# Avokadoen/tdt4230_project_raytracing

Hardware: AMD Instinct MI355X
Metric: Mray-samples/sec at 1080p/64spp/depth-8 (higher is better)
Workload: dtype f32; 1 GPU; 1920x1080, 64 spp, max_bounce 8, 64^3 octree terrain+spheres (BASELINE configs[1] scene at the metric's 64 spp); written_pixels=2027520, spp=64, passes=1, max_bounce=8, octree_max_depth=6, octree_cells=4209, scene_bytes=269868, partition=32x32 work-groups dealt round-robin over 1 rank(s)

## Files before the change

### include/tdt_rt.h

```cpp
#ifndef TDT_RT_H
#define TDT_RT_H

#include <stddef.h>
#include <stdint.h>

#ifdef __cplusplus
extern "C" {
#endif

typedef struct tdt_ctx tdt_ctx;
typedef struct tdt_compute tdt_compute;
typedef struct tdt_buffer tdt_buffer;
typedef struct tdt_image tdt_image;

enum {
  TDT_OK = 0,
  TDT_ERR_NO_DEVICE = 1,
  TDT_ERR_HIP = 2,
  TDT_ERR_INVALID_ENUM = 0x0500,
  TDT_ERR_INVALID_VALUE = 0x0501,
  TDT_ERR_INVALID_OPERATION = 0x0502,
  TDT_ERR_VARIABLE_NOT_FOUND = 3,
  TDT_ERR_INCOMPLETE = 4
};
// ... 183 lines not shown
#ifdef __cplusplus
static_assert(sizeof(tdt_mesh) == 40, "tdt_mesh is 40 bytes");
#else
_Static_assert(sizeof(tdt_mesh) == 40, "tdt_mesh is 40 bytes");
#endif
int tdt_voxelize_triangles(tdt_ctx *ctx, const tdt_mesh *mesh, int depth, int32_t *voxels_xyzm, size_t capacity, size_t *n_voxels);
int tdt_octree_edit_triangles(tdt_ctx *ctx, int op, const tdt_mesh *mesh, uint32_t *n_cells);

typedef struct tdt_fill {
  int32_t connectivity;
  int32_t material;
} tdt_fill;
#ifdef __cplusplus
static_assert(sizeof(tdt_fill) == 8, "tdt_fill is 8 bytes");
#else
_Static_assert(sizeof(tdt_fill) == 8, "tdt_fill is 8 bytes");
#endif
int tdt_octree_extract_enclosed(tdt_ctx *ctx, const tdt_fill *fill, const tdt_region *regions, size_t n_regions, int32_t *voxels_xyzm,
                                size_t capacity, size_t *n_voxels);
int tdt_octree_fill_enclosed(tdt_ctx *ctx, const tdt_fill *fill, const tdt_region *regions, size_t n_regions, uint32_t *n_cells);
int tdt_voxelize_triangles_solid(tdt_ctx *ctx, const tdt_mesh *mesh, int depth, const tdt_fill *fill, int32_t *voxels_xyzm, size_t capacity,
                                 size_t *n_voxels);
int tdt_octree_edit_triangles_solid(tdt_ctx *ctx, int op, const tdt_mesh *mesh, const tdt_fill *fill, uint32_t *n_cells);
int tdt_debug_fill_passes(const tdt_ctx *ctx);

typedef struct tdt_surface {
  int32_t merge;
  int32_t by_material;
} tdt_surface;
typedef struct tdt_quad {
  int32_t face;
  int32_t material;
  int32_t origin[3];
  int32_t size[2];
  int32_t pad;
} tdt_quad;
#ifdef __cplusplus
static_assert(sizeof(tdt_surface) == 8, "tdt_surface is 8 bytes");
static_assert(sizeof(tdt_quad) == 32, "tdt_quad is 32 bytes");
#else
_Static_assert(sizeof(tdt_surface) == 8, "tdt_surface is 8 bytes");
_Static_assert(sizeof(tdt_quad) == 32, "tdt_quad is 32 bytes");
#endif
int tdt_octree_extract_surface(tdt_ctx *ctx, const tdt_surface *opt, const tdt_region *regions, size_t n_regions, tdt_quad *quads,
                               size_t capacity, size_t *n_quads);

#define TDT_ROUND_DOMAIN_CAP (1u << 28)
typedef struct tdt_round {
  int32_t op;
  int32_t radius2;
  int32_t material;
  int32_t border;
} tdt_round;
#ifdef __cplusplus
static_assert(sizeof(tdt_round) == 16, "tdt_round is 16 bytes");
#else
_Static_assert(sizeof(tdt_round) == 16, "tdt_round is 16 bytes");
#endif
int tdt_octree_morph_round(tdt_ctx *ctx, const tdt_round *r, const tdt_region *regions, size_t n_regions, uint32_t *n_cells);
int tdt_octree_extract_morph_round(tdt_ctx *ctx, const tdt_round *r, const tdt_region *regions, size_t n_regions, int32_t *voxels_xyzm,
                                   size_t capacity, size_t *n_voxels);
int tdt_octree_distance_field(tdt_ctx *ctx, const int32_t lo[3], const int32_t hi[3], int32_t max_d2, int32_t border, int32_t *field,
                              int32_t *nearest_xyz, size_t capacity, size_t *n_voxels);

#define TDT_XFORM_ONE 65536
typedef struct tdt_xform {
  int64_t t[3];
  int32_t a[9];
  int32_t material;
  int32_t dst_lo[3], dst_hi[3];
  int32_t pad[2];
} tdt_xform;
#ifdef __cplusplus
static_assert(sizeof(tdt_xform) == 96, "tdt_xform is 96 bytes");
#else
_Static_assert(sizeof(tdt_xform) == 96, "tdt_xform is 96 bytes");
#endif
int tdt_octree_extract_transform(tdt_ctx *ctx, const tdt_xform *xf, const tdt_region *regions, size_t n_regions, int32_t *voxels_xyzm,
                                 size_t capacity, size_t *n_voxels);
int tdt_octree_transform(tdt_ctx *ctx, const tdt_xform *xf, int op, const tdt_region *regions, size_t n_regions, uint32_t *n_cells);
int tdt_debug_xform_bricks(const tdt_ctx *ctx, uint32_t out[2]);

int tdt_debug_last_variant(const tdt_ctx *ctx, int out[6]);
int tdt_debug_trace_variants(int *rows, int capacity, int *count);
int tdt_debug_stats(tdt_ctx *ctx, uint64_t *out, int n_words, int reset);
int tdt_debug_counters(tdt_ctx *ctx, uint64_t out[32]);
int tdt_debug_wave_ends(tdt_ctx *ctx, uint64_t *out, int n);
int tdt_debug_pixel_log(tdt_ctx *ctx, uint32_t *out, size_t n_u32);
int tdt_selftest(tdt_ctx *ctx, int which, uint64_t *mismatches);
int tdt_selftest_index(tdt_ctx *ctx, int32_t cell_count, float inv_cell_count, uint32_t n_cells, int shift, uint64_t *mismatches,
                       int *shape_ok);

#ifdef __cplusplus
}
#endif
#endif
```

### tdt4230_project_raytracing_amd/build.py

```python
import os
import shutil
import subprocess

_HERE = os.path.dirname(os.path.abspath(__file__))
ROOT = os.path.dirname(_HERE)
CSRC = os.path.join(_HERE, "csrc")
INCLUDE = os.path.join(ROOT, "include")

HIPCC = os.environ.get("HIPCC") or shutil.which("hipcc") or "/opt/rocm/bin/hipcc"

HIP_FLAGS = ["--offload-arch=gfx950", "-O3", "-std=c++17", "-fPIC", "-shared", "-ffp-contract=off",
             "-fhip-fp32-correctly-rounded-divide-sqrt", "-fno-fast-math", "-Wall", "-Wextra",
             "-fno-slp-vectorize"]
HOST_FLAGS = ["-O2", "-std=c++17", "-fPIC", "-shared", "-Wall", "-Wextra", "-ffp-contract=off"]


def _newer(out, srcs):
    if not os.path.exists(out):
        return True
    t = os.path.getmtime(out)
    return any(os.path.getmtime(s) > t for s in srcs)


def _run(cmd):
    r = subprocess.run(cmd, capture_output=True, text=True)
    if r.returncode != 0:
        raise RuntimeError("build failed: " + " ".join(cmd) + "\n" + r.stdout + r.stderr)
    return r.stdout + r.stderr


def build_host(force=False):
    out = os.path.join(_HERE, "libtdthost.so")
    srcs = [os.path.join(CSRC, "host_scene.cpp"), os.path.join(CSRC, "host_view.cpp"), os.path.join(CSRC, "host_mesh.cpp"),
            os.path.join(CSRC, "host_xform.cpp"), os.path.join(INCLUDE, "tdt_host.h"), os.path.join(INCLUDE, "tdt_rt.h"), os.path.abspath(__file__)]
    if force or _newer(out, srcs):
        _run(["g++"] + HOST_FLAGS + ["-I", INCLUDE] + srcs[:4] + ["-o", out, "-lz"])
    return out


DEVICE_UNITS = ("tdt_rt.hip", "tdt_multi.hip", "tdt_build.hip", "tdt_edit.hip", "tdt_query.hip", "tdt_compact.hip",
                "tdt_region.hip", "tdt_connect.hip", "tdt_morph.hip", "tdt_mesh.hip", "tdt_fill.hip", "tdt_surface.hip",
                "tdt_distance.hip", "tdt_bitvol.hip", "tdt_xform.hip")
DEVICE_HEADERS = ("trace_device.hpp", "trace_params.h", "tdt_internal.hpp", "device_scan.hpp", "region_device.hpp", "bitvol_device.hpp")


def build_device(force=False, extra_flags=(), out=None):
    out = out or os.path.join(_HERE, "libtdtrt.so")
    hdrs = [os.path.join(CSRC, f) for f in DEVICE_HEADERS] + [os.path.join(INCLUDE, "tdt_rt.h"), os.path.abspath(__file__)]
    srcs = [os.path.join(CSRC, f) for f in DEVICE_UNITS]
    if not (force or extra_flags or _newer(out, srcs + hdrs)):
        return out
    objdir = os.path.join(CSRC, "obj" + ("_" + str(abs(hash(tuple(extra_flags))) % 100000) if extra_flags else ""))
    os.makedirs(objdir, exist_ok=True)
    compile_flags = [f for f in HIP_FLAGS if f != "-shared"] + list(extra_flags)
    jobs = []
    for src in srcs:
        obj = os.path.join(objdir, os.path.basename(src) + ".o")
        if force or extra_flags or _newer(obj, [src] + hdrs):
            jobs.append((subprocess.Popen([HIPCC] + compile_flags + ["-I", INCLUDE, "-I", CSRC, "-c", src, "-o", obj],
                                          stdout=subprocess.PIPE, stderr=subprocess.STDOUT, text=True), src))
    for p, src in jobs:
        log, _ = p.communicate()
        if p.returncode != 0:
            raise RuntimeError("build failed: " + src + "\n" + log)
    objs = [os.path.join(objdir, os.path.basename(src) + ".o") for src in srcs]
    _run([HIPCC, "--offload-arch=gfx950", "-shared", "-fPIC"] + objs + ["-o", out, "-ldl"])
    return out


def build_demo(force=False):
    out = os.path.join(_HERE, "tdt_demo")
    srcs = [os.path.join(CSRC, "demo_main.cpp"), os.path.join(INCLUDE, "renderer.hpp"), os.path.join(INCLUDE, "tdt_rt.h"),
            os.path.join(INCLUDE, "tdt_host.h"), os.path.abspath(__file__)]
    if force or _newer(out, srcs):
        rocm_lib = os.path.join(os.path.dirname(os.path.dirname(os.path.realpath(HIPCC))), "lib")
        _run(["g++", "-O2", "-std=c++17", "-Wall", "-Wextra", "-I", INCLUDE, srcs[0], "-o", out, "-L", _HERE, "-ltdtrt", "-ltdthost",
              "-Wl,-rpath,$ORIGIN", "-Wl,-rpath-link," + rocm_lib])
    return out


def build_selftest(force=False):
    out = os.path.join(_HERE, "libtdtprims_selftest.so")
    src = os.path.join(CSRC, "prims_selftest.hip")
    deps = [src, os.path.join(CSRC, "device_scan.hpp"), os.path.join(CSRC, "tdt_internal.hpp"),
            os.path.join(INCLUDE, "tdt_rt.h"), os.path.abspath(__file__)]
    if force or _newer(out, deps):
        _run([HIPCC] + HIP_FLAGS + ["-I", INCLUDE, "-I", CSRC, src, "-o", out, "-L", _HERE, "-ltdtrt", "-Wl,-rpath,$ORIGIN"])
    return out


def build_all(force=False):
    return build_host(force), build_device(force), build_demo(force), build_selftest(force)
```

### tdt4230_project_raytracing_amd/csrc/tdt_rt.hip

```cpp
#include <hip/hip_runtime.h>

#include <atomic>
#include <cstdio>
#include <cstdlib>
#include <cstring>
#include <initializer_list>
#include <new>
#include <string>
#include <vector>

#include "tdt_rt.h"
#include "trace_device.hpp"
#include "trace_params.h"

#ifndef TDT_BLOCK
#define TDT_BLOCK 1024
#define TDT_BLOCKS_PER_CU 1
#endif
namespace tdt {

TDT_DEV void decode_pixel(const TraceParams &P, int k, uint32_t p, int &x, int &y, size_t &pix, bool &inside) {
  const int t = P.part_rank + k * P.part_world;
  int gx, gy;
  if (P.tiles_x_magic) { gy = (int)__umulhi((uint32_t)t, P.tiles_x_magic); gx = t - gy * P.tiles_x; }
  else { gx = t % P.tiles_x; gy = t / P.tiles_x; }
  const int tile = (int)(p >> 6), w = (int)(p & 63);
  const int lx = (tile & 3) * 8 + (w & 7), ly = (tile >> 2) * 8 + (w >> 3);
  x = gx * 32 + lx;
  y = gy * 32 + ly;
  pix = P.compact ? ((size_t)k * 1024 + (size_t)(ly * 32 + lx)) : ((size_t)y * (size_t)P.image_width + (size_t)x);
  inside = x < P.cover_w && y < P.cover_h;
}

TDT_DEV bool pixel_of_thread(const TraceParams &P, int &x, int &y, size_t &pix) {
  const int k = blockIdx.x >> 2, sub = blockIdx.x & 3;
  bool inside;
  decode_pixel(P, k, (uint32_t)(sub * 256 + threadIdx.x), x, y, pix, inside);
  return inside;
}

TDT_DEV uint32_t wave_sum(uint32_t v) {
  for (int o = 32; o > 0; o >>= 1) v += __shfl_xor(v, o, 64);
  return v;
}


enum : int { ST_DONE = -1, ST_TRAVERSE = 0, ST_HIT = 1, ST_END = 2, ST_FETCH = 3, ST_PRIMARY = 4, ST_NEWRAY = 5 };

template <bool AS_MASKS> struct HitOwed;
template <> struct HitOwed<true> {
  bool use_leaf = false, leaf_rec = false;
  TDT_DEV void set(bool later_step, bool cube_ok) { use_leaf = later_step; leaf_rec = later_step && cube_ok; }
  TDT_DEV bool leaf_site() const { return use_leaf; }
  TDT_DEV bool new_record() const { return leaf_rec; }
};
template <> struct HitOwed<false> {
  uint32_t bits = 0u;
  TDT_DEV void set(bool later_step, bool cube_ok) { bits = later_step ? (cube_ok ? 3u : 1u) : 0u; }
  TDT_DEV bool leaf_site() const { return (bits & 1u) != 0u; }
  TDT_DEV bool new_record() const { return (bits & 2u) != 0u; }
};

enum : int { STAT_TRAV_PASS = 0, STAT_TRAV_LANES, STAT_INSIDE_LANES, STAT_ALIVE_LANES, STAT_EVENT_PASS, STAT_EVENT_LANES, STAT_HIT_PASS, STAT_HIT_LANES,
             STAT_LAMB_PASS, STAT_LAMB_LANES, STAT_METAL_PASS, STAT_METAL_LANES, STAT_DIEL_PASS, STAT_DIEL_LANES, STAT_END_PASS, STAT_END_LANES,
             STAT_PIXEL_END_PASS, STAT_PIXEL_END_LANES, STAT_FETCH_PASS, STAT_FETCH_LANES, STAT_PRIMARY_PASS, STAT_PRIMARY_LANES,
             STAT_NEWRAY_PASS, STAT_NEWRAY_LANES, STAT_GATE_WAIT_LANES, STAT_DRAINED_TRAV_PASS, STAT_DRAINED_EVENT_PASS, STAT_LOOP_PASS, STAT_WAVE_TICKS, STAT_WAVES,
             STAT_T_FIRST, STAT_T_LAST, STAT_COUNT = 32 };
#ifdef TDT_STATS
TDT_DEV void stat_add(uint32_t *row, int i, unsigned long long mask) {
  const unsigned long long m = __ballot(1);
  if (mask != 0ull && (threadIdx.x & 63) == (uint32_t)__builtin_ctzll(m)) { row[i] += 1u; row[i + 1] += (uint32_t)__popcll(mask); }
}
#define TDT_ST(i, mask) stat_add(s_stat_row, (i), (mask))
#define TDT_ST1(i, v) do { const unsigned long long m_ = __ballot(1); if ((threadIdx.x & 63) == (uint32_t)__builtin_ctzll(m_)) s_stat_row[i] += (uint32_t)(v); } while (0)
#else
#define TDT_ST(i, mask) do {} while (0)
#define TDT_ST1(i, v) do {} while (0)
#endif

template <bool COUNT, int FORM, int DEPTH = 0, bool RESIDENT = false, bool SAFEV = false, bool FULL = false, bool UNIT = false, bool BRICK = false>
__global__ __launch_bounds__(TDT_BLOCK) void trace_kernel(const TraceParams P) {
  constexpr bool POW2 = FORM != FORM_LITERAL;
  constexpr bool kSlim2 = DEPTH > 0;
#ifdef TDT_THRESHOLD_EVERY
  constexpr uint32_t kThresholdEvery = kSlim2 ? TDT_THRESHOLD_EVERY : 1u;
#else
  constexpr uint32_t kThresholdEvery = kSlim2 ? 8u : 1u;
#endif
  constexpr bool kSharedRand = !BRICK;
  constexpr bool kColdArgs = BRICK;
#ifdef TDT_NO_STUCK_CUT
  constexpr bool kStuckCut = false;
#else
  constexpr bool kStuckCut = BRICK && !COUNT;
#endif
#ifdef TDT_NO_SHARED_NORM
  constexpr bool kSharedNorm = false;
#else
  constexpr bool kSharedNorm = kSlim2;
#endif
  __shared__ __attribute__((aligned(16))) uint16_t s_nodes[(BRICK ? kBrickLdsCells : kLdsCells) * 8 + 8];
  for (uint32_t i = threadIdx.x * 8u; i < P.lds_nodes; i += (uint32_t)TDT_BLOCK * 8u)
    *reinterpret_cast<uint4 *>(&s_nodes[i]) = *reinterpret_cast<const uint4 *>(&P.packed[i]);
  if (threadIdx.x < 16 && P.lds_nodes + threadIdx.x < ((P.lds_nodes + 7u) & ~7u) + 8u)
    s_nodes[P.lds_nodes + threadIdx.x] = (uint16_t)((RESIDENT && POW2) ? 0u : kPackedEscape);
  constexpr bool kPlanes = FULL && !COUNT && kFullEntryForm == kFullPlanes;
  __shared__ __attribute__((aligned(8))) float2 s_planes[kPlanes ? PlaneTable::kEntries : 1];
  if constexpr (kPlanes) build_plane_table<DEPTH, UNIT>(s_planes, P.scale, P.min_x, P.min_y, P.min_z);
  __syncthreads();
  constexpr bool TABLE = FORM == FORM_TABLE;
  static_assert(!TABLE || (SAFEV && !BRICK && !FULL), "per-cell thresholds: the resident walk, or the jump table's bands of a tree outside the LDS table");
  constexpr uint32_t kThrCells = !TABLE ? 0u : (RESIDENT ? kLdsCells : kThrTopCells);
  __shared__ __attribute__((aligned(8))) float2 s_thr[kThrCells + 1];
  __shared__ uint32_t s_band;
  if (TABLE) {
    for (uint32_t i = threadIdx.x; i <= kThrCells; i += (uint32_t)TDT_BLOCK)
      s_thr[i] = i < P.thr_cells ? reinterpret_cast<const float2 *>(P.thr)[i] : make_float2(2.0f, 2.0f);
    __syncthreads();
  }
  constexpr int GL = top_grid_levels(RESIDENT, TABLE);
  constexpr bool kUseGrid = !FULL && !BRICK && !COUNT && POW2 && SAFEV && DEPTH >= GL;
  __shared__ typename Grid<GL>::Entry s_grid[kUseGrid ? Grid<GL>::kEntries : 1];
  __shared__ int s_grid_ok;
  if (kUseGrid) build_top_grid<GL, TABLE>(s_nodes, P.lds_nodes, DEPTH, s_grid, &s_grid_ok, s_thr, P.thr_cells, P.thr_f0max, &s_band);
  __shared__ __attribute__((aligned(16))) uint32_t s_grid32[BRICK ? (1 << 15) : 4];
  if (BRICK) {
    for (uint32_t i = threadIdx.x * 4u; i < (1u << 15); i += (uint32_t)TDT_BLOCK * 4u)
      *reinterpret_cast<uint4 *>(&s_grid32[i]) = *reinterpret_cast<const uint4 *>(&P.brick_grid[i]);
    __syncthreads();
  }
  NodeSource ns;
  ns.lds = s_nodes; ns.lds_nodes = P.lds_nodes; ns.lds_cells = (P.lds_nodes + 7u) >> 3;
  ns.grid = s_grid; ns.grid_ok = kUseGrid ? (__builtin_amdgcn_readfirstlane(s_grid_ok) != 0) : false;
  ns.grid_band = FULL ? Grid<5>::kBand : (ns.grid_ok ? (TABLE && kUseGrid ? __uint_as_float((uint32_t)__builtin_amdgcn_readfirstlane((int)s_band)) : Grid<GL>::kBand) : 2.0f);
  ns.thr = s_thr; ns.thr_f0max = P.thr_f0max;
  ns.full = P.full_grid;
  if constexpr (kPlanes) ns.planes = s_planes;
  ns.grid32 = s_grid32; ns.bricks = P.bricks;
  if (BRICK) {
    uint32_t lo, hi;
    asm volatile("v_mov_b32 %0, %2\n\tv_mov_b32 %1, %3" : "=v"(lo), "=v"(hi) : "s"((uint32_t)(uintptr_t)P.bricks), "s"((uint32_t)((uintptr_t)P.bricks >> 32)));
    ns.bricks = reinterpret_cast<const void *>(((uintptr_t)hi << 32) | (uintptr_t)lo);
  }
  ns.cells = __builtin_amdgcn_make_buffer_rsrc((void *)P.cells, 0, (int)((P.cells_dwords >> 1) << 3), 0x00020000);
  typedef const __attribute__((address_space(4))) TraceParams *KArg;
  const KArg Pk = (KArg)__builtin_amdgcn_kernarg_segment_ptr();
  MatSource ms_regs;
  if (!kColdArgs) ms_regs = material_source(P);
#ifdef TDT_STATS
  __shared__ uint32_t s_stats[(TDT_BLOCK / 64) * STAT_COUNT];
  uint32_t *const s_stat_row = &s_stats[(threadIdx.x >> 6) * STAT_COUNT];
  if ((threadIdx.x & 63) < STAT_COUNT) s_stat_row[threadIdx.x & 63] = 0u;
  const unsigned long long stat_t0 = __builtin_amdgcn_s_memrealtime();
  bool stat_drained = false;
#endif
  const uint32_t total_slots = (uint32_t)P.owned_tiles * 1024u;
  if (blockIdx.x == 0 && threadIdx.x == 0 && P.queue_next) *P.queue_next = 0u;

  const float inf = __builtin_inff();
#ifdef TDT_STATS
  uint32_t stat_pix_t0 = 0u;
#endif
  unsigned long long pixel_rt0 = 0ull; bool wave_drained = false; uint32_t lane_S = 0, lane_E = 0, pass_no = 0, pixel_pass0 = 0, evpass_no = 0, pixel_evpass0 = 0;
  const unsigned long long wave_t0 = COUNT ? __builtin_amdgcn_s_memrealtime() : 0ull;
  if (COUNT && (threadIdx.x & 63) == 0) atomicCAS(&P.counters[23], 0ull, wave_t0);
  Counters cnt = {};
  uint32_t n_pixels = 0;
  constexpr int kMemo = BRICK ? kBrickMemoLevels : kMemoLevels;
  NodeMemo<kMemo> memo;
#pragma unroll
  for (int l = 0; l < kMemo; l++) { memo.key[l] = 0x3FFFFFFFu; memo.val[l] = 0u; }

  int state = ST_FETCH;
  int x = 0, y = 0; size_t pix = 0;
  uint32_t pixel_slot = 0;
  const bool exact_draw = P.plan != nullptr && __builtin_amdgcn_readfirstlane((int)P.plan[0]) != 0;
  uint32_t buf_slot = 0xFFFFFFFFu, buf_next = 0u, buf_count = 0u;
  int s = 0, loop_count = 0;
  Ray r = {0.f, 0.f, 0.f, 0.f, 0.f, 1.f};
  float ix = 0.f, iy = 0.f, iz = 0.f;
  float ar = 1.f, ag = 1.f, ab = 1.f;
  float sr = 0.f, sg = 0.f, sb = 0.f;
  float t_stride = 0.f, t_octree_max = 0.f, inv_pow_depth = 0.5f;
  int it = 0;
  HitOwed<DEPTH == 0> owed;
  uint32_t hit_index = 0;
  float leaf_box_x = 0.f, leaf_box_y = 0.f, leaf_box_z = 0.f;
  Carry pc;
  pc.root = {0.f, 0.f, 0.f, 0.f, 0.f, 0.f, false}; pc.leaf = pc.root; pc.root_t = 0.f;
  const int s_end = P.spp_begin + P.spp_count;

  uint32_t w_steps = 0, w_rays = 0, lane_work = 0;
  uint32_t ev_no = 0;
  int threshold = P.event_threshold > 0 ? P.event_threshold : 24;

  unsigned long long tacc[7] = {0, 0, 0, 0, 0, 0, 0}, tlast = COUNT ? __builtin_amdgcn_s_memtime() : 0ull;
#define TDT_TICK(i) do { if (COUNT) { const unsigned long long n_ = __builtin_amdgcn_s_memtime(); tacc[i] += n_ - tlast; tlast = n_; } } while (0)
  float vmin_x, vmin_y, vmin_z;
  if (DEPTH == 0) { vmin_x = P.min_x; vmin_y = P.min_y; vmin_z = P.min_z; }
  else asm volatile("v_mov_b32 %0, %3\n\tv_mov_b32 %1, %4\n\tv_mov_b32 %2, %5" : "=v"(vmin_x), "=v"(vmin_y), "=v"(vmin_z) : "s"(P.min_x), "s"(P.min_y), "s"(P.min_z));
  if constexpr (kPlanes) { ns.vmin_x = vmin_x; ns.vmin_y = vmin_y; ns.vmin_z = vmin_z; }
  unsigned long long k_trav = 0ull, k_event = ~0ull;
  int th_now = threshold;
  for (;;) {
    if (COUNT) pass_no++;
    TDT_ST1(STAT_LOOP_PASS, 1);
    TDT_MARK(traversal);
    {
      const bool trav = __builtin_amdgcn_inverse_ballot_w64(k_trav);
      const unsigned long long k_trav0 = k_trav;
      if (COUNT && trav) { lane_S++; cnt.trav_slots += slot64(); cnt.trav_active++; }
      const bool go = trav && (it < P.max_iter) && (t_stride < t_octree_max);
      const float adv = POW2 ? 0.0001f * (inv_pow_depth + 0.1f) : f_max(0.0001f * (inv_pow_depth + 0.1f), 0.000001f);
      const float tt = t_stride + adv;
      const float wx = tt * r.dx + r.ox, wy = tt * r.dy + r.oy, wz = tt * r.dz + r.oz;
      const float lx = UNIT ? (wx + -vmin_x) : (wx + -vmin_x) * P.inv_scale, ly = UNIT ? (wy + -vmin_y) : (wy + -vmin_y) * P.inv_scale,
                  lz = UNIT ? (wz + -vmin_z) : (wz + -vmin_z) * P.inv_scale;
      bool in_box;
      if (POW2) {
        constexpr bool kNoNegZero = UNIT && kSlim2;
        const uint32_t ux = __float_as_uint(kNoNegZero ? lx : lx + 0.0f), uy = __float_as_uint(kNoNegZero ? ly : ly + 0.0f), uz = __float_as_uint(kNoNegZero ? lz : lz + 0.0f);
        const uint32_t um = ux > uy ? ux : uy;
        in_box = (um > uz ? um : uz) < 0x3F800000u;
      } else {
        const float ex = f_fract(lx) + -lx, ey = f_fract(ly) + -ly, ez = f_fract(lz) + -lz;
        in_box = !((__builtin_fabsf(ez) + __builtin_fabsf(ey)) != -__builtin_fabsf(ex));
      }
      const bool inside = go && in_box;
      TDT_ST(STAT_TRAV_PASS, __ballot(trav)); TDT_ST1(STAT_INSIDE_LANES, __popcll(__ballot(inside))); TDT_ST1(STAT_ALIVE_LANES, __popcll(__ballot(state != ST_DONE)));
#ifdef TDT_STATS
      TDT_ST1(STAT_DRAINED_TRAV_PASS, stat_drained ? 1 : 0);
#endif
      if (inside) {
        float ugx, ugy, ugz; uint32_t value;
        if (COUNT) cnt.iterations++;
        const float ipd_in = inv_pow_depth;
        CellPlanes cp;
        bool leaf;
        if constexpr (kPlanes) leaf = tree_lookup_pow2<COUNT, kMemo, DEPTH, RESIDENT, SAFEV, FULL, BRICK, TABLE, UNIT>(P, ns, lx, ly, lz, inv_pow_depth, ugx, ugy, ugz, value, memo, cnt, &cp);
        else leaf = POW2 ? tree_lookup_pow2<COUNT, kMemo, DEPTH, RESIDENT, SAFEV, FULL, BRICK, TABLE>(P, ns, lx, ly, lz, inv_pow_depth, ugx, ugy, ugz, value, memo, cnt)
                         : tree_lookup<COUNT>(P, ns, lx, ly, lz, inv_pow_depth, ugx, ugy, ugz, value, cnt);
        TDT_MARK(traversal_b);
        float t_enter, t_exit, cs, cx = 0.f, cy = 0.f, cz = 0.f;
        if constexpr (kPlanes) {
          leaf_box_x = cp.lox; leaf_box_y = cp.loy; leaf_box_z = cp.loz; hit_index = value;
          cube_slabs_planes(r, ix, iy, iz, cp.lox, cp.loy, cp.loz, cp.hix, cp.hiy, cp.hiz, t_stride, t_octree_max, t_enter, t_exit);
          cs = UNIT ? inv_pow_depth : P.scale * inv_pow_depth;
        } else {
          if (!kSlim2) lane_work += kCostStep + (127u - (__float_as_uint(inv_pow_depth) >> 23));
          const float bx = (UNIT ? ugx : ugx * P.scale) + vmin_x, by = (UNIT ? ugy : ugy * P.scale) + vmin_y, bz = (UNIT ? ugz : ugz * P.scale) + vmin_z;
          const float cs0 = UNIT ? inv_pow_depth : P.scale * inv_pow_depth;
          const float pad = leaf ? -0.0f : -0.00001f;
          if (kSlim2) { leaf_box_x = bx + pad; leaf_box_y = by + pad; leaf_box_z = bz + pad; hit_index = value; }
          cx = kSlim2 ? leaf_box_x : bx + pad; cy = kSlim2 ? leaf_box_y : by + pad; cz = kSlim2 ? leaf_box_z : bz + pad;
          cs = leaf ? cs0 : cs0 + 0.00002f;
          cube_slabs(r, ix, iy, iz, cx, cy, cz, cs, t_stride, t_octree_max, t_enter, t_exit);
        }
        const bool cube_ok = !(t_exit < t_enter);
        if (leaf) {
          if (!kSlim2) { leaf_box_x = cx; leaf_box_y = cy; leaf_box_z = cz; hit_index = value; }
          inv_pow_depth = cs; t_stride = t_enter;
          owed.set(it > 0, cube_ok);
          state = ST_HIT;
        } else {
          const float ts_new = cube_ok ? t_exit : t_octree_max;
          if (kStuckCut) {
            const bool stuck = __float_as_uint(ts_new) == __float_as_uint(t_stride) && __float_as_uint(inv_pow_depth) == __float_as_uint(ipd_in);
            t_stride = stuck ? t_octree_max : ts_new;
          } else t_stride = ts_new;
          it++;
        }
      }
      state = (trav && !inside) ? ST_END : state;
      k_trav &= __ballot(state == ST_TRAVERSE);
      k_event = ~k_trav & (k_event | k_trav0);
    }

    TDT_TICK(0);
    TDT_MARK(gate);
    const unsigned long long m_trav = k_trav, m_event = k_event;
    if (m_trav == 0ull && m_event == 0ull) break;
    w_steps += (uint32_t)__popcll(m_trav);
    TDT_ST1(STAT_GATE_WAIT_LANES, __popcll(m_event));
    if ((int)__popcll(m_event) < th_now && m_trav != 0ull) { TDT_TICK(1); continue; }
    TDT_TICK(1);
    TDT_ST(STAT_EVENT_PASS, m_event); TDT_ST(STAT_HIT_PASS, __ballot(state == ST_HIT));
#ifdef TDT_STATS
    TDT_ST1(STAT_DRAINED_EVENT_PASS, stat_drained ? 1 : 0);
#endif

    TDT_MARK(hit_prologue);
    if (COUNT) evpass_no++;
    if (COUNT) { cnt.event_slots += slot64(); cnt.event_active += (state > ST_TRAVERSE); }
    if (kSlim2) lane_work += (state == ST_HIT || state == ST_END) ? kCostEvent + kCostRayStep * ((uint32_t)it + 1u) : ((state > ST_TRAVERSE) ? kCostEvent : 0u);
    else lane_work += (state > ST_TRAVERSE) ? kCostEvent : 0u;
    if (COUNT) lane_E += (state > ST_TRAVERSE) ? 1u : 0u;
    if (state == ST_HIT) {
      if (COUNT) { cnt.scatter_slots += slot64(); cnt.scatter_active++; }
      MatSource ms;
      if (kColdArgs) {
        KArg pk = Pk; asm volatile("" : "+s"(pk));
        ms.materials = table_rsrc(pk->materials, pk->materials_dwords); ms.albedos = table_rsrc(pk->albedos, pk->albedos_dwords);
        ms.metal = table_rsrc(pk->metal, pk->metal_dwords); ms.dielectric = table_rsrc(pk->dielectric, pk->dielectric_dwords);
      } else ms = ms_regs;
      const MatRef mat = material_fetch(ms, hit_index);
      TDT_ST(STAT_LAMB_PASS, __ballot(mat.type == 0u)); TDT_ST(STAT_METAL_PASS, __ballot(mat.type == 1u)); TDT_ST(STAT_DIEL_PASS, __ballot(mat.type == 2u));
      if (owed.new_record()) { cube_hit_record(r, t_stride, leaf_box_x, leaf_box_y, leaf_box_z, inv_pow_depth, pc.leaf); if (COUNT) cnt.leaf_records++; }
      loop_count += 1;
      const HitTmp &src = owed.leaf_site() ? pc.leaf : pc.root;
      Hit h;
      h.px = src.px; h.py = src.py; h.pz = src.pz; h.nx = src.nx; h.ny = src.ny; h.nz = src.nz; h.ff = src.ff;
      h.index = hit_index;
      Ray nr; float tr, tg, tb;
      const bool scattered = scatter<COUNT, kSharedRand, kSharedNorm>(ms, r, h, mat, nr, tr, tg, tb, cnt);
      TDT_MARK(hit_epilogue);
      if (scattered) {
        ar = ar * tr; ag = ag * tg; ab = ab * tb;
        r = nr;
        state = loop_count < P.max_bounce ? ST_NEWRAY : ST_END;
      } else {
        state = ST_END;
      }
    }
    TDT_TICK(2);
    TDT_MARK(end_of_path);
    TDT_ST(STAT_END_PASS, __ballot(state == ST_END));
    if (state == ST_END) {
      float cr, cg, cb;
      if (loop_count > 0) { cr = ar; cg = ag; cb = ab; }
      else {
        const float yp = r.dy + 1.0f;
        const float w = 1.0f + -(0.5f * yp);
        cr = w + 0.25f * yp; cg = w + 0.35f * yp; cb = 1.0f;
      }
      sr = sr + cr; sg = sg + cg; sb = sb + cb;
      s++;
      if (s < s_end) state = ST_PRIMARY;
      else {
        TDT_MARK(pixel_end);
        TDT_ST(STAT_PIXEL_END_PASS, __ballot(1));
        float4 *dst = reinterpret_cast<float4 *>(P.image) + pix;
        if (P.accumulate) {
          *dst = make_float4(sr, sg, sb, 0.f);
          if (P.carry && !P.carry_final) {
            float4 *c = reinterpret_cast<float4 *>(P.carry) + pix * 4;
            c[0] = make_float4(pc.root.nx, pc.root.ny, pc.root.nz, pc.root.px);
            c[1] = make_float4(pc.root.py, pc.root.pz, pc.root.ff ? 1.f : 0.f, pc.root_t);
            c[2] = make_float4(pc.leaf.nx, pc.leaf.ny, pc.leaf.nz, pc.leaf.px);
            c[3] = make_float4(pc.leaf.py, pc.leaf.pz, pc.leaf.ff ? 1.f : 0.f, 0.f);
          }
        } else {
          const float n = (float)P.samples_per_pixel;
          float4 o;
          o.x = f_min(f_max(__builtin_sqrtf(sr / n), 0.f), 1.f);
          o.y = f_min(f_max(__builtin_sqrtf(sg / n), 0.f), 1.f);
          o.z = f_min(f_max(__builtin_sqrtf(sb / n), 0.f), 1.f);
          o.w = 1.0f;
          *dst = o;
        }
#ifdef TDT_STATS
        if (P.stats && P.pixel_log) {
          uint32_t *L = P.pixel_log + (size_t)pixel_slot * 8;
          L[0] = lane_work; L[3] = stat_pix_t0; L[4] = (uint32_t)__builtin_amdgcn_s_memrealtime(); L[5] = blockIdx.x * 16 + (threadIdx.x >> 6); L[7] = (uint32_t)threshold;
        }
#endif
        if (COUNT && P.pixel_log) {
          uint32_t *L = P.pixel_log + (size_t)pixel_slot * 8;
          L[0] = lane_S; L[1] = lane_E; L[2] = pass_no - pixel_pass0; L[3] = (uint32_t)(pixel_rt0 - P.counters[23]);
          L[4] = (uint32_t)(__builtin_amdgcn_s_memrealtime() - P.counters[23]); L[5] = blockIdx.x * 16 + (threadIdx.x >> 6); L[6] = evpass_no - pixel_evpass0; L[7] = (uint32_t)threshold;
        }
        if (COUNT) {
          const unsigned long long d = (__builtin_amdgcn_s_memrealtime() - pixel_rt0) / 10000ull;
          atomicAdd(&P.counters[32 + 16384 + (wave_drained ? 128 : 0) + (d > 127ull ? 127ull : d)], 1ull);
        }
        if (P.slot_cost) P.slot_cost[pixel_slot] = lane_work | 1u;
        state = ST_FETCH;
      }
    }
    TDT_TICK(3);
    TDT_MARK(fetch);
    {
      bool want = state == ST_FETCH;
      unsigned long long m = __ballot(want);
      TDT_ST(STAT_FETCH_PASS, m);
      while (m != 0ull) {
        if (buf_next >= buf_count) {
          const uint32_t chunk = exact_draw ? (uint32_t)__popcll(m) : 64u;
          uint32_t base = 0;
          if ((threadIdx.x & 63) == 0) base = atomicAdd(P.queue, chunk);
          base = (uint32_t)__builtin_amdgcn_readfirstlane((int)base);
          const uint32_t bq = base + (threadIdx.x & 63u);
          buf_slot = ((threadIdx.x & 63u) < chunk && bq < total_slots) ? (P.slot_order ? P.slot_order[bq] : bq) : 0xFFFFFFFFu;
          buf_next = 0u; buf_count = chunk;
          if (COUNT && base + chunk > total_slots) wave_drained = true;
#ifdef TDT_STATS
          if (base + chunk > total_slots && !stat_drained) { stat_drained = true; if (P.stats && (threadIdx.x & 63) == 0) atomicMin(&P.stats[STAT_COUNT], __builtin_amdgcn_s_memrealtime()); }
#endif
        }
        const uint32_t rank = (uint32_t)__popcll(m & ((1ull << (threadIdx.x & 63)) - 1ull));
        const uint32_t avail = buf_count - buf_next;
        const uint32_t got = (uint32_t)__shfl((int)buf_slot, (int)((buf_next + rank) & 63u), 64);
        const bool served = want && rank < avail;
        buf_next += (uint32_t)__popcll(m) < avail ? (uint32_t)__popcll(m) : avail;
        m = __ballot(want && !served);
        if (served) {
          want = false;
          const uint32_t q = got;
          if (q == 0xFFFFFFFFu) { state = ST_DONE; if (COUNT) atomicMin(&P.counters[22], __builtin_amdgcn_s_memrealtime()); }
          else {
#ifdef TDT_STATS
            stat_pix_t0 = (uint32_t)__builtin_amdgcn_s_memrealtime();
#endif
            if (COUNT) { pixel_rt0 = __builtin_amdgcn_s_memrealtime(); lane_S = 0; lane_E = 0; pixel_pass0 = pass_no; pixel_evpass0 = evpass_no; }
            bool inside;
            pixel_slot = q;
            decode_pixel(P, (int)(pixel_slot >> 10), pixel_slot & 1023u, x, y, pix, inside);
            lane_work = 0u;
            if (inside) {
              n_pixels++;
              sr = 0.f; sg = 0.f; sb = 0.f; s = P.spp_begin;
              pc.root = {0.f, 0.f, 0.f, 0.f, 0.f, 0.f, false}; pc.leaf = pc.root; pc.root_t = 0.f;
              if (P.accumulate && P.spp_begin != 0) {
                const float4 acc = *(reinterpret_cast<const float4 *>(P.image) + pix);
                sr = acc.x; sg = acc.y; sb = acc.z;
                if (P.carry) {
                  const float4 *c = reinterpret_cast<const float4 *>(P.carry) + pix * 4;
                  const float4 c0 = c[0], c1 = c[1], c2 = c[2], c3 = c[3];
                  pc.root = {c0.x, c0.y, c0.z, c0.w, c1.x, c1.y, c1.z != 0.f}; pc.root_t = c1.w;
                  pc.leaf = {c2.x, c2.y, c2.z, c2.w, c3.x, c3.y, c3.z != 0.f};
                }
              }
              if (s < s_end) state = ST_PRIMARY;
              else if (!P.accumulate) {
                const float n = (float)P.samples_per_pixel;
                const float v0 = f_min(f_max(__builtin_sqrtf(0.f / n), 0.f), 1.f);
                *(reinterpret_cast<float4 *>(P.image) + pix) = make_float4(v0, v0, v0, 1.0f);
              }
            }
          }
        }
      }
    }
    TDT_TICK(4);
    TDT_MARK(primary);
    TDT_ST(STAT_PRIMARY_PASS, __ballot(state == ST_PRIMARY));
    if (state == ST_PRIMARY) {
      r = primary_ray(P, x, y, s);
      loop_count = 0; ar = 1.f; ag = 1.f; ab = 1.f;
      state = ST_NEWRAY;
    }
    TDT_MARK(threshold);
    w_rays += (uint32_t)__popcll(__ballot(state == ST_NEWRAY));
    if (P.event_threshold <= 0 && (ev_no++ & (kThresholdEvery - 1u)) == 0u) {
      if (w_rays > kEventWindow) { w_steps >>= 1; w_rays >>= 1; }
      const float est = 64.0f * __builtin_amdgcn_rcpf(0.5f + __builtin_amdgcn_sqrtf(P.event_k * (float)w_steps * __builtin_amdgcn_rcpf((float)w_rays + 1.0f)));
      const int th = (int)__builtin_fminf(est, P.event_clamp);
      threshold = w_rays < 256u ? 24 : (th < 2 ? 2 : th);
    }
    TDT_TICK(5);
    TDT_MARK(newray);
    TDT_ST(STAT_NEWRAY_PASS, __ballot(state == ST_NEWRAY));
    if (state == ST_NEWRAY) {
      if (!(loop_count < P.max_bounce)) state = ST_END;
      else {
        if (COUNT) cnt.octree_hit_calls++;
        q_rcp3(r.dx, r.dy, r.dz, ix, iy, iz);
        const float lx = (P.min_x + -r.ox) * ix, ly = (P.min_y + -r.oy) * iy, lz = (P.min_z + -r.oz) * iz;
        const float ux = ((P.min_x + P.scale) + -r.ox) * ix, uy = ((P.min_y + P.scale) + -r.oy) * iy,
                    uz = ((P.min_z + P.scale) + -r.oz) * iz;
        const float mnx = hw_min(lx, ux), mny = hw_min(ly, uy), mnz = hw_min(lz, uz);
        const float mxx = hw_max(lx, ux), mxy = hw_max(ly, uy), mxz = hw_max(lz, uz);
        const float t_enter = hw_max(hw_max(hw_max(mnx, 0.0003f), mny), mnz);
        const float t_exit = hw_min(hw_min(hw_min(mxx, inf), mxy), mxz);
        t_octree_max = inf;
        if (t_exit >= t_enter) {
          cube_hit_record(r, t_enter, P.min_x, P.min_y, P.min_z, P.scale, pc.root);
          pc.root_t = t_enter;
          t_octree_max = t_exit;
        }
        t_stride = pc.root_t;
        inv_pow_depth = 0.5f;
        it = 0;
        state = ST_TRAVERSE;
      }
    }
    TDT_TICK(6);
    k_trav = __ballot(state == ST_TRAVERSE); k_event = __ballot(state > ST_TRAVERSE);
    { const int n_alive = __popcll(k_trav | k_event); th_now = n_alive == 64 ? threshold : ((threshold * n_alive) >> 6) + 1; }
    TDT_MARK(loop_tail);
  }
  TDT_MARK(after_loop);
#undef TDT_TICK
#ifdef TDT_STATS
  if (P.stats) {
    const unsigned long long stat_t1 = __builtin_amdgcn_s_memrealtime();
    const uint32_t lane = threadIdx.x & 63u;
    if (lane < (uint32_t)STAT_WAVE_TICKS) { const uint32_t v = s_stat_row[lane]; if (v) atomicAdd(&P.stats[lane], (unsigned long long)v); }
    if (lane == 0) { atomicAdd(&P.stats[STAT_WAVE_TICKS], stat_t1 - stat_t0); atomicAdd(&P.stats[STAT_WAVES], 1ull);
                     atomicMin(&P.stats[STAT_T_FIRST], stat_t0); atomicMax(&P.stats[STAT_T_LAST], stat_t1);
                     const uint32_t w = blockIdx.x * (TDT_BLOCK / 64) + (threadIdx.x >> 6);
                     if (w < 8192u) P.stats[STAT_COUNT + 1 + w] = stat_t1; }
  }
#endif

  if (COUNT) {
    if ((threadIdx.x & 63) == 0) {
      const unsigned long long t_end = __builtin_amdgcn_s_memrealtime();
      atomicMin(&P.counters[18], wave_t0); atomicMax(&P.counters[19], t_end);
      atomicAdd(&P.counters[20], t_end - wave_t0); atomicAdd(&P.counters[21], 1ull);
      P.counters[32 + blockIdx.x * (TDT_BLOCK / 64) + (threadIdx.x >> 6)] = t_end;
    }
    if ((threadIdx.x & 63) == 0) for (int i = 0; i < 7; i++) atomicAdd(&P.counters[24 + i], tacc[i]);
    uint32_t v[18] = {n_pixels, cnt.octree_hit_calls, cnt.iterations, cnt.node_loads,
                      cnt.lambertian, cnt.metal, cnt.dielectric, cnt.unknown,
                      cnt.trav_slots, cnt.trav_active, cnt.level_slots, cnt.level_active, cnt.event_slots, cnt.event_active,
                      cnt.scatter_slots, cnt.scatter_active, cnt.memo_miss, cnt.leaf_records};
    for (int i = 0; i < 18; i++) {
      uint32_t tot = wave_sum(v[i]);
      if ((threadIdx.x & 63) == 0 && tot) atomicAdd(&P.counters[i], (unsigned long long)tot);
    }
  }
}

__global__ __launch_bounds__(256) void resolve_kernel(const TraceParams P) {
  int x, y; size_t pix;
  if (!pixel_of_thread(P, x, y, pix)) return;
  float4 *dst = reinterpret_cast<float4 *>(P.image) + pix;
  float4 a = *dst;
  if (P.carry_final && a.w != 0.f) return;
  const float n = (float)P.total_spp;
  float4 o;
  o.x = f_min(f_max(__builtin_sqrtf(a.x / n), 0.f), 1.f);
  o.y = f_min(f_max(__builtin_sqrtf(a.y / n), 0.f), 1.f);
  o.z = f_min(f_max(__builtin_sqrtf(a.z / n), 0.f), 1.f);
  o.w = 1.0f;
  *dst = o;
}

__global__ __launch_bounds__(256) void miss_prepass_kernel(const TraceParams P, uint8_t *__restrict__ done) {
  int x, y; size_t pix;
  const bool covered = pixel_of_thread(P, x, y, pix);
  const size_t slot = (size_t)(blockIdx.x >> 2) * 1024u + (size_t)((blockIdx.x & 3) * 256 + threadIdx.x);
  bool all_miss = covered;
  float sr = 0.f, sg = 0.f, sb = 0.f;
  const float inf = __builtin_inff();
  for (int s = 0; s < P.samples_per_pixel && __ballot(all_miss) != 0ull; s++) {
    const Ray r = primary_ray(P, x, y, s);
    float ix, iy, iz;
    q_rcp3(r.dx, r.dy, r.dz, ix, iy, iz);
    const float lx = (P.min_x + -r.ox) * ix, ly = (P.min_y + -r.oy) * iy, lz = (P.min_z + -r.oz) * iz;
    const float ux = ((P.min_x + P.scale) + -r.ox) * ix, uy = ((P.min_y + P.scale) + -r.oy) * iy, uz = ((P.min_z + P.scale) + -r.oz) * iz;
    const float mnx = hw_min(lx, ux), mny = hw_min(ly, uy), mnz = hw_min(lz, uz);
    const float mxx = hw_max(lx, ux), mxy = hw_max(ly, uy), mxz = hw_max(lz, uz);
    const float t_enter = hw_max(hw_max(hw_max(mnx, 0.0003f), mny), mnz);
    const float t_exit = hw_min(hw_min(hw_min(mxx, inf), mxy), mxz);
    const bool root_hit = t_exit >= t_enter;
    const float adv = f_max(0.0001f * (0.5f + 0.1f), 0.000001f);
    const float tt = 0.f + adv;
    const float wx = tt * r.dx + r.ox, wy = tt * r.dy + r.oy, wz = tt * r.dz + r.oz;
    const float px = (wx + -P.min_x) * P.inv_scale, py = (wy + -P.min_y) * P.inv_scale, pz = (wz + -P.min_z) * P.inv_scale;
    const float ex = f_fract(px) + -px, ey = f_fract(py) + -py, ez = f_fract(pz) + -pz;
    const bool in_box = !((__builtin_fabsf(ez) + __builtin_fabsf(ey)) != -__builtin_fabsf(ex));
    const bool steps_in = (0 < P.max_iter) && (0.f < inf) && in_box;
    if (root_hit || steps_in) all_miss = false;
    const float yp = r.dy + 1.0f;
    const float w = 1.0f + -(0.5f * yp);
    sr = sr + (w + 0.25f * yp); sg = sg + (w + 0.35f * yp); sb = sb + 1.0f;
  }
  if (covered && all_miss) {
    const float n = (float)P.samples_per_pixel;
    float4 o;
    o.x = f_min(f_max(__builtin_sqrtf(sr / n), 0.f), 1.f);
    o.y = f_min(f_max(__builtin_sqrtf(sg / n), 0.f), 1.f);
    o.z = f_min(f_max(__builtin_sqrtf(sb / n), 0.f), 1.f);
    o.w = 1.0f;
    *(reinterpret_cast<float4 *>(P.image) + pix) = o;
  }
  done[slot] = (!covered || all_miss) ? 1u : 0u;
}

constexpr uint32_t kFilterChunk = 4096;
TDT_DEV uint32_t filter_rank(bool live, uint32_t *s_wave, uint32_t &block_total) {
  const unsigned long long m = __ballot(live);
  const uint32_t lane = threadIdx.x & 63u, wave = threadIdx.x >> 6;
  if (lane == 0) s_wave[wave] = (uint32_t)__popcll(m);
  __syncthreads();
  uint32_t before = 0, total = 0;
  for (uint32_t w = 0; w < 16u; w++) { const uint32_t c = s_wave[w]; before += w < wave ? c : 0u; total += c; }
  __syncthreads();
  block_total = total;
  return before + (uint32_t)__popcll(m & ((1ull << lane) - 1ull));
}
__global__ __launch_bounds__(1024) void filter_count_kernel(const uint32_t *__restrict__ order, const uint8_t *__restrict__ done, uint32_t n, uint32_t *__restrict__ counts) {
// ... 479 lines not shown
  const float4 c = image[(size_t)y * w + x];
  auto u8 = [](float v) -> uint32_t {
    const float t = !(v > 0.0f) ? 0.0f : (v > 1.0f ? 1.0f : v);
    return (uint32_t)__builtin_rintf(t * 255.0f);
  };
  out[(size_t)(top_down ? h - 1 - y : y) * w + x] = u8(c.x) | (u8(c.y) << 8) | (u8(c.z) << 16) | (u8(c.w) << 24);
}

__global__ __launch_bounds__(256) void assemble_kernel(const float4 *__restrict__ tiles, float4 *__restrict__ image,
                                                       int image_width, int cover_w, int cover_h, int tiles_x,
                                                       int world, int tiles_per_rank) {
  const int x = blockIdx.x * 64 + (threadIdx.x & 63);
  const int y = blockIdx.y * 4 + (threadIdx.x >> 6);
  if (x >= cover_w || y >= cover_h) return;
  const int t = (y >> 5) * tiles_x + (x >> 5);
  const int rank = t % world, k = t / world;
  const size_t src = ((size_t)rank * tiles_per_rank + k) * 1024 + (size_t)((y & 31) * 32 + (x & 31));
  image[(size_t)y * image_width + x] = tiles[src];
}

}

#include "tdt_internal.hpp"

namespace {
thread_local std::string g_create_err;
}

namespace tdt {
int fail(tdt_ctx *ctx, int code, const std::string &msg) {
  if (ctx) ctx->err = msg; else g_create_err = msg;
  return code;
}
int hip_fail(tdt_ctx *ctx, hipError_t e, const char *what) {
  return fail(ctx, TDT_ERR_HIP, std::string(what) + ": " + hipGetErrorString(e));
}
}
using tdt::fail; using tdt::hip_fail; using tdt::erase_from; using tdt::Cover; using tdt::Tiles; using tdt::cover_of; using tdt::tiles_of;

Cover tdt::cover_of(const tdt_compute *c, int width, int height) {
  Cover k;
  k.groups_x = width / 32 < 1 ? 1 : width / 32;
  k.groups_y = height / 32 < 1 ? 1 : height / 32;
  long cw = (long)k.groups_x * 32, ch = (long)k.groups_y * 32;
  k.cover_w = (int)(cw < c->image_width ? cw : c->image_width);
  k.cover_h = (int)(ch < c->image_height ? ch : c->image_height);
  if (k.cover_w < 0) k.cover_w = 0;
  if (k.cover_h < 0) k.cover_h = 0;
  return k;
}
Tiles tdt::tiles_of(const tdt_compute *c, const Cover &k) {
  Tiles t;
  t.tiles_x = (k.cover_w + 31) / 32; t.tiles_y = (k.cover_h + 31) / 32;
  t.total = t.tiles_x * t.tiles_y;
  t.owned = t.total > c->part_rank ? (t.total - c->part_rank + c->part_world - 1) / c->part_world : 0;
  return t;
}
namespace {
int64_t owned_pixels(const tdt_compute *c, const Cover &k) {
  Tiles t = tiles_of(c, k);
  int64_t n = 0;
  for (int i = 0; i < t.owned; i++) {
    int id = c->part_rank + i * c->part_world;
    int gx = id % t.tiles_x, gy = id / t.tiles_x;
    int w = k.cover_w - gx * 32, h = k.cover_h - gy * 32;
    n += (int64_t)(w > 32 ? 32 : w) * (h > 32 ? 32 : h);
  }
  return n;
}

void make_sig(const tdt_ctx *ctx, const tdt_compute *c, const Cover &k, const tdt_image *img, CostSig *sig) {
  std::memset(sig, 0, sizeof *sig);
  std::memcpy(sig->cam_i, &c->image_width, sizeof sig->cam_i);
  std::memcpy(sig->cam_f, c->horizontal, sizeof sig->cam_f);
  sig->part[0] = c->part_rank; sig->part[1] = c->part_world;
  std::memcpy(sig->octree_f, ctx->ssbo[TDT_SLOT_OCTREE_FLOATS]->shadow, sizeof sig->octree_f);
  std::memcpy(sig->octree_i, ctx->ssbo[TDT_SLOT_OCTREE_INTS]->shadow, sizeof sig->octree_i);
  sig->cover[0] = k.cover_w; sig->cover[1] = k.cover_h; sig->image[0] = img->w; sig->image[1] = img->h;
  for (int sl = 0; sl < kNumSlots; sl++)
    if (ctx->ssbo[sl]) { sig->slot[sl].buffer = ctx->ssbo[sl]; sig->slot[sl].version = ctx->ssbo[sl]->version; }
}

using TraceFn = void (*)(const TraceParams);
struct TraceVariant { int form, depth; bool resident, full, brick, unit; TraceFn fn; };
#define TDT_V1(FORM, D, R, F, B, U) {tdt::FORM, D, R, F, B, U, tdt::trace_kernel<false, tdt::FORM, D, R, true, F, U, B>}
#define TDT_V(FORM, D, R, F, B) TDT_V1(FORM, D, R, F, B, false), TDT_V1(FORM, D, R, F, B, true)
const TraceVariant kTraceVariants[] = {
  TDT_V(FORM_POW2, 6, false, false, true), TDT_V(FORM_POW2, 7, false, false, true), TDT_V(FORM_POW2, 8, false, false, true),
  TDT_V(FORM_POW2, 9, false, false, true), TDT_V(FORM_POW2, 10, false, false, true),
  TDT_V(FORM_POW2, 6, false, false, false), TDT_V(FORM_POW2, 7, false, false, false), TDT_V(FORM_POW2, 8, false, false, false),
  TDT_V(FORM_POW2, 9, false, false, false), TDT_V(FORM_POW2, 10, false, false, false),
  TDT_V(FORM_POW2, 5, true, true, false), TDT_V(FORM_POW2, 6, true, true, false),
  TDT_V(FORM_POW2, 3, true, false, false), TDT_V(FORM_POW2, 4, true, false, false), TDT_V(FORM_POW2, 5, true, false, false),
  TDT_V(FORM_POW2, 6, true, false, false), TDT_V(FORM_POW2, 7, true, false, false), TDT_V(FORM_POW2, 8, true, false, false),
  TDT_V(FORM_POW2, 9, true, false, false), TDT_V(FORM_POW2, 10, true, false, false),
  TDT_V(FORM_TABLE, 3, true, false, false), TDT_V(FORM_TABLE, 4, true, false, false), TDT_V(FORM_TABLE, 5, true, false, false),
  TDT_V(FORM_TABLE, 6, true, false, false), TDT_V(FORM_TABLE, 7, true, false, false), TDT_V(FORM_TABLE, 8, true, false, false),
  TDT_V(FORM_TABLE, 9, true, false, false), TDT_V(FORM_TABLE, 10, true, false, false),
  TDT_V(FORM_TABLE, 6, false, false, false), TDT_V(FORM_TABLE, 7, false, false, false), TDT_V(FORM_TABLE, 8, false, false, false),
  TDT_V(FORM_TABLE, 9, false, false, false), TDT_V(FORM_TABLE, 10, false, false, false),
};
#undef TDT_V
#undef TDT_V1
TraceFn find_variant(int form, int depth, bool resident, bool full, bool brick, bool unit) {
  for (const TraceVariant &v : kTraceVariants)
    if (v.form == form && v.depth == depth && v.resident == resident && v.full == full && v.brick == brick && v.unit == unit) return v.fn;
  return nullptr;
}

}

int tdt::octree_uniforms(tdt_ctx *ctx, TraceParams &P) {
  if (ctx->ssbo[TDT_SLOT_OCTREE_FLOATS]->bytes < 28 || ctx->ssbo[TDT_SLOT_OCTREE_INTS]->bytes < 12)
    return fail(ctx, TDT_ERR_INVALID_VALUE, "octree uniform buffers are too small (need 28 / 12 bytes)");
  float of[7]; int32_t oi[3];
  std::memcpy(of, ctx->ssbo[TDT_SLOT_OCTREE_FLOATS]->shadow, sizeof of);
  std::memcpy(oi, ctx->ssbo[TDT_SLOT_OCTREE_INTS]->shadow, sizeof oi);
  P.min_x = of[0]; P.min_y = of[1]; P.min_z = of[2]; P.scale = of[4]; P.inv_scale = of[5]; P.inv_cell_count = of[6];
  P.max_depth = oi[0]; P.max_iter = oi[1]; P.cell_count = oi[2];
  return TDT_OK;
}

namespace {
bool env_set(const char *name) { return getenv(name) != nullptr; }
bool env_one(const char *name) { const char *v = getenv(name); return v && v[0] == '1'; }
float env_float(const char *name, float otherwise) { const char *v = getenv(name); return v ? (float)atof(v) : otherwise; }
int env_int(const char *name, int lo, int hi, int otherwise) {
  const char *v = getenv(name);
  return v && atoi(v) >= lo && atoi(v) <= hi ? atoi(v) : otherwise;
}
constexpr int kAnyLo = -2147483647 - 1, kAnyHi = 2147483647;
}

struct tdt::TraceState {
  tdt::DeviceScratch mem;
  struct Switches {
    bool no_cost_order = env_one("TDT_NO_COST_ORDER");
    int force_smooth = env_int("TDT_ORDER_SMOOTH", kAnyLo, kAnyHi, -1);
    bool no_cost_accum = env_set("TDT_NO_COST_ACCUM");
    bool no_two_phase = env_set("TDT_NO_TWO_PHASE");
    bool no_prepass = env_set("TDT_NO_PREPASS");
    bool no_order_reuse = env_set("TDT_NO_ORDER_REUSE");
    bool no_full = env_set("TDT_NO_FULL_GRID");
    bool no_table_form = env_set("TDT_NO_TABLE_FORM");
    bool no_bricks = env_set("TDT_NO_BRICKS");
    float max_share = env_float("TDT_MAX_SHARE", 1.0f);
    float order_blend = env_float("TDT_ORDER_BLEND", 0.5f);
    int two_phase_min_spp = env_int("TDT_TWO_PHASE_MIN_SPP", 2, kAnyHi, 16);
    int probe_div = env_int("TDT_PROBE_DIV", 2, 64, 16);
    bool force_generic = env_one("TDT_FORCE_GENERIC");
    bool no_specialise = env_one("TDT_NO_SPECIALISE");
    int event_threshold = env_int("TDT_EVENT_THRESHOLD", kAnyLo, kAnyHi, 0);
    float event_k = env_float("TDT_EVENT_K", 0.0f);
    int event_clamp = env_int("TDT_EVENT_CLAMP", 2, 64, 40);
  } env;
  struct Queue {
    unsigned int *heads = nullptr; unsigned parity = 0;
  } queue;
  struct CostOrder {
    uint32_t *slot_cost = nullptr, *slot_acc = nullptr, *slot_order = nullptr;
    uint32_t *hist = nullptr; unsigned parity = 0;
    uint32_t tile_capacity = 0, cost_tiles = 0;
    uint32_t cost_dispatches = 0;
    uint32_t acc_samples = 0, last_launch_samples = 0;
    int cost_range[2] = {0, 0}; bool order_exact = false;
    CostSig cost_sig = {};
  } order;
  struct MissPrepass {
    uint8_t *slot_done = nullptr; uint32_t *slot_live = nullptr, *filter_counts = nullptr; uint32_t capacity = 0;
  } miss;
  struct TableKey {
    const tdt_buffer *buffer = nullptr; unsigned long long version = 0; int depth = 0;
    bool operator==(const TableKey &o) const { return buffer == o.buffer && version == o.version && depth == o.depth; }
  };
  struct ThresholdKey {
    int32_t cell_count = 0; uint32_t ic_bits = 0, n = 0;
    bool operator==(const ThresholdKey &o) const { return cell_count == o.cell_count && ic_bits == o.ic_bits && n == o.n; }
  };
  struct Tables {
    uint16_t *packed = nullptr; TableKey packed_key;
    uint32_t *scan = nullptr;
    uint32_t max_parent_value = 0xFFFFFFFFu, max_any_value = 0xFFFFFFFFu, live_nodes = 0xFFFFFFFFu;
    float *thr = nullptr; ThresholdKey thr_key; float thr_f0max = 0.0f; bool thr_ok = false;
    FullGridEntry *full_grid = nullptr; TableKey full_key; bool full_ok = false;
    uint32_t *brick_grid = nullptr; uint16_t *bricks = nullptr; size_t bricks_bytes = 0; TableKey brick_key; bool brick_ok = false;
  } tables;
  float *frame_carry = nullptr; size_t frame_carry_bytes = 0;
  bool phase_timing = false; hipEvent_t phase_ev[4] = {}; int phase_n = 0;
  uint32_t *present = nullptr; size_t present_bytes = 0;
  uint32_t *pixel_log = nullptr; size_t pixel_log_u32 = 0;
  unsigned long long *stats = nullptr;
  int last_variant[6] = {};

  ~TraceState() { if (phase_timing) for (auto &e : phase_ev) (void)hipEventDestroy(e); }
  template <class T> hipError_t alloc(T *&p, size_t n) { p = mem.get<T>(n); return p ? hipSuccess : hipErrorOutOfMemory; }
  struct Array {
    void **p; size_t bytes;
    template <class T> Array(T *&ptr, size_t count) : p(reinterpret_cast<void **>(&ptr)), bytes(count * sizeof(T)) {}
  };
  template <class C> hipError_t grow(C &capacity, C need, std::initializer_list<Array> arrays) {
    if (capacity >= need) return hipSuccess;
    capacity = 0;
    for (const Array &a : arrays) { mem.drop(*a.p); *a.p = nullptr; }
    for (const Array &a : arrays)
      if (!(*a.p = mem.get<unsigned char>(a.bytes))) {
        for (const Array &b : arrays) { mem.drop(*b.p); *b.p = nullptr; }
        return hipErrorOutOfMemory;
      }
    capacity = need;
    return hipSuccess;
  }
};

namespace {
using tdt::TraceState;

struct LaunchRequest {
  enum Kind { kRender = 0, kAccumulate = 1, kResolve = 2, kMissPrepass = 3 } kind = kRender;
  int spp_begin = 0, spp_count = 0, total_spp = 0;
  void *carry = nullptr; bool carry_final = false;
  bool probe = false;
  bool prepass_ran = false;
  unsigned long long *counts_out = nullptr;
};

int bind_params(const tdt_compute *c, int width, int height, const LaunchRequest &rq, TraceParams &P, Cover &k, Tiles &t) {
  tdt_ctx *ctx = c->ctx;
  const TraceState::Switches &env = ctx->trace->env;
  static const int required[] = {TDT_SLOT_CELLS, TDT_SLOT_MATERIALS, TDT_SLOT_ALBEDOS, TDT_SLOT_METAL,
                                 TDT_SLOT_DIELECTRIC, TDT_SLOT_OCTREE_FLOATS, TDT_SLOT_OCTREE_INTS};
  for (int s : required)
    if (!ctx->ssbo[s]) return fail(ctx, TDT_ERR_INCOMPLETE, "no buffer bound to shader-storage slot " + std::to_string(s));
  if (!ctx->image0) return fail(ctx, TDT_ERR_INCOMPLETE, "no image bound to unit 0");
  const tdt_image *img = ctx->image0;

  std::memset(&P, 0, sizeof P);
  if (int rc = tdt::octree_uniforms(ctx, P)) return rc;
  P.image_width = c->image_width; P.image_height = c->image_height;
  for (int i = 0; i < 3; i++) {
    P.hor[i] = c->horizontal[i]; P.ver[i] = c->vertical[i]; P.llc[i] = c->lower_left_corner[i]; P.org[i] = c->origin[i];
  }
  P.samples_per_pixel = c->samples_per_pixel; P.max_bounce = c->max_bounce;
  auto dwords = [](const tdt_buffer *b) { size_t d = b->bytes >> 2; return (uint32_t)(d > 0xFFFFFFFFull ? 0xFFFFFFFFull : d); };
  P.cells = (const uint32_t *)ctx->ssbo[TDT_SLOT_CELLS]->dev; P.cells_dwords = dwords(ctx->ssbo[TDT_SLOT_CELLS]);
  P.materials = (const uint32_t *)ctx->ssbo[TDT_SLOT_MATERIALS]->dev; P.materials_dwords = dwords(ctx->ssbo[TDT_SLOT_MATERIALS]);
  P.albedos = (const uint32_t *)ctx->ssbo[TDT_SLOT_ALBEDOS]->dev; P.albedos_dwords = dwords(ctx->ssbo[TDT_SLOT_ALBEDOS]);
  P.metal = (const uint32_t *)ctx->ssbo[TDT_SLOT_METAL]->dev; P.metal_dwords = dwords(ctx->ssbo[TDT_SLOT_METAL]);
  P.dielectric = (const uint32_t *)ctx->ssbo[TDT_SLOT_DIELECTRIC]->dev; P.dielectric_dwords = dwords(ctx->ssbo[TDT_SLOT_DIELECTRIC]);
  P.image = img->dev; P.carry = (float *)rq.carry;
  P.carry_final = (rq.kind == LaunchRequest::kResolve ? rq.prepass_ran : rq.carry_final) ? 1 : 0;
  k = cover_of(c, width, height);
  t = tiles_of(c, k);
  P.cover_w = k.cover_w; P.cover_h = k.cover_h;
  P.tiles_x = t.tiles_x > 0 ? t.tiles_x : 1; P.owned_tiles = t.owned;
  P.tiles_x_magic = ((unsigned long long)(t.total > 0 ? t.total : 1) * (unsigned long long)P.tiles_x < (1ull << 32) && P.tiles_x > 1)
                        ? (uint32_t)((1ull << 32) / (unsigned long long)P.tiles_x) + 1u : 0u;
  P.part_rank = c->part_rank; P.part_world = c->part_world;
  if (img->w == c->image_width && img->h == c->image_height) P.compact = 0;
  else if (img->w == 32 && img->h >= 32 * t.owned && (img->h % 32) == 0) P.compact = 1;
  else return fail(ctx, TDT_ERR_INVALID_OPERATION,
                   "bound image is neither camera.image_width x image_height nor a 32 x 32*tiles tile buffer");
  P.spp_begin = rq.spp_begin; P.spp_count = rq.spp_count; P.mode = rq.kind; P.total_spp = rq.total_spp;
  P.accumulate = rq.kind == LaunchRequest::kAccumulate ? 1 : 0;
  P.event_threshold = env.event_threshold;
  P.event_clamp = (float)env.event_clamp;
  {
    const float mib = (float)ctx->ssbo[TDT_SLOT_CELLS]->bytes / 1048576.0f;
    const float r = 0.07f * mib;
    P.event_k = env.event_k > 0.0f ? env.event_k : (r < 0.10f ? 0.10f : (r > 0.35f ? 0.35f : r));
    { static const char *ks = getenv("TDT_EVENT_K_SCALE"); if (ks && atof(ks) > 0.0) P.event_k *= (float)atof(ks); }
  }
  TDT_HIP(ctx, hipSetDevice(ctx->device));
  if (ctx->ssbo[TDT_SLOT_CELLS]->bytes > 0xFFFFFFF8ull)
    return fail(ctx, TDT_ERR_INVALID_VALUE, "cells buffer larger than 4 GiB is not addressable by the shader's 32-bit offsets");
  return TDT_OK;
// ... 1 lines not shown

int launch_miss_prepass(tdt_ctx *ctx, TraceState &S, int owned, const TraceParams &P) {
  if (owned <= 0) return TDT_OK;
  const size_t n = (size_t)owned * 1024;
  TDT_HIP(ctx, S.grow(S.miss.capacity, (uint32_t)owned, {{S.miss.slot_done, n}, {S.miss.slot_live, n},
                                                         {S.miss.filter_counts, (n + tdt::kFilterChunk - 1) / tdt::kFilterChunk + 1}}));
  hipLaunchKernelGGL(tdt::miss_prepass_kernel, dim3((unsigned)owned * 4u), dim3(256), 0, ctx->stream, P, S.miss.slot_done);
  TDT_HIP(ctx, hipGetLastError());
  return TDT_OK;
}

int launch_resolve(tdt_ctx *ctx, int owned, const TraceParams &P) {
  if (owned <= 0) return TDT_OK;
  hipLaunchKernelGGL(tdt::resolve_kernel, dim3((unsigned)owned * 4u, 1, 1), dim3(256, 1, 1), 0, ctx->stream, P);
  TDT_HIP(ctx, hipGetLastError());
  return TDT_OK;
}

int begin_instrumented(tdt_ctx *ctx, TraceState &S, const LaunchRequest &rq, int owned, TraceParams &P) {
  bool logged = rq.counts_out != nullptr;
#ifdef TDT_STATS
  P.stats = !rq.counts_out && !(rq.probe && getenv("TDT_STATS_SKIP_PROBE")) ? S.stats : nullptr;
  logged = logged || P.stats;
#endif
  if (rq.counts_out) {
    if (!ctx->counters) TDT_HIP(ctx, hipMalloc((void **)&ctx->counters, (32 + 16384 + 256) * sizeof(unsigned long long)));
    TDT_HIP(ctx, hipMemsetAsync(ctx->counters, 0, 32 * sizeof(unsigned long long), ctx->stream));
    TDT_HIP(ctx, hipMemsetAsync(ctx->counters + 18, 0xFF, sizeof(unsigned long long), ctx->stream));
    TDT_HIP(ctx, hipMemsetAsync(ctx->counters + 22, 0xFF, sizeof(unsigned long long), ctx->stream));
    TDT_HIP(ctx, hipMemsetAsync(ctx->counters + 32 + 16384, 0, 256 * sizeof(unsigned long long), ctx->stream));
    P.counters = ctx->counters;
  }
  if (logged && getenv("TDT_PIXEL_LOG")) {
    const size_t need = (size_t)owned * 1024 * 8;
    TDT_HIP(ctx, S.grow(S.pixel_log_u32, need, {{S.pixel_log, need}}));
    TDT_HIP(ctx, hipMemsetAsync(S.pixel_log, 0, need * 4, ctx->stream));
    P.pixel_log = S.pixel_log;
  }
  return TDT_OK;
}

int bind_queue(tdt_ctx *ctx, TraceState::Queue &Q, tdt::DeviceScratch &mem, TraceParams &P) {
  if (!Q.heads) {
    unsigned int *heads = mem.get<unsigned int>(2);
    if (!heads) return hip_fail(ctx, hipErrorOutOfMemory, "pixel-queue heads");
    const hipError_t e = hipMemsetAsync(heads, 0, 2 * sizeof(unsigned int), ctx->stream);
    if (e != hipSuccess) { mem.drop(heads); return hip_fail(ctx, e, "pixel-queue heads"); }
    Q.heads = heads; Q.parity = 0;
  }
  P.queue = Q.heads + Q.parity; P.queue_next = Q.heads + (Q.parity ^ 1u);
  return TDT_OK;
}

int refresh_packed(tdt_ctx *ctx, TraceState &S, TraceParams &P) {
  TraceState::Tables &T = S.tables;
  const tdt_buffer *cb = ctx->ssbo[TDT_SLOT_CELLS];
  const uint32_t buf_nodes = P.cells_dwords >> 1;
  if (!T.packed) TDT_HIP(ctx, S.alloc(T.packed, (size_t)tdt::kLdsCells * 8));
  P.lds_nodes = buf_nodes < tdt::kLdsCells * 8u ? (buf_nodes & ~7u) : tdt::kLdsCells * 8u;
  const TraceState::TableKey key{cb, cb->version, 0};
  if (!(T.packed_key == key)) {
    if (!T.scan) TDT_HIP(ctx, S.alloc(T.scan, 4));
    TDT_HIP(ctx, hipMemsetAsync(T.scan, 0, 4 * sizeof(uint32_t), ctx->stream));
    if (P.lds_nodes)
      hipLaunchKernelGGL(tdt::pack_cells_kernel, dim3((P.lds_nodes + 255) / 256), dim3(256), 0, ctx->stream,
                         P.cells, P.cells_dwords, T.packed, P.lds_nodes);
    if (buf_nodes) {
      unsigned nb = (buf_nodes + 255) / 256; if (nb > 4096) nb = 4096;
      hipLaunchKernelGGL(tdt::scan_cells_kernel, dim3(nb), dim3(256), 0, ctx->stream, P.cells, buf_nodes, T.scan);
    }
    TDT_HIP(ctx, hipGetLastError());
    uint32_t res[3] = {0, 0, 0};
    TDT_HIP(ctx, hipMemcpyAsync(res, T.scan, sizeof res, hipMemcpyDeviceToHost, ctx->stream));
    TDT_HIP(ctx, hipStreamSynchronize(ctx->stream));
    T.max_parent_value = res[0]; T.max_any_value = res[1]; T.live_nodes = res[2];
    T.packed_key = key;
  }
  P.packed = T.packed;
  return TDT_OK;
}

struct HandOut { const uint32_t *slot_order = nullptr, *plan = nullptr; uint32_t *slot_cost = nullptr; };

int plan_order(tdt_ctx *ctx, TraceState &S, const CostSig &sig, const LaunchRequest &rq, int owned, HandOut &out) {
  TraceState::CostOrder &O = S.order;
  const TraceState::Switches &env = S.env;
  const size_t n = (size_t)owned * 1024;
  if (O.tile_capacity < (uint32_t)owned) { O.cost_tiles = 0; O.order_exact = false; }
  TDT_HIP(ctx, S.grow(O.tile_capacity, (uint32_t)owned, {{O.slot_cost, n}, {O.slot_order, n}, {O.slot_acc, n}}));
  if (!O.hist) {
    TDT_HIP(ctx, S.alloc(O.hist, 2048 + 4 + 512));
    TDT_HIP(ctx, hipMemsetAsync(O.hist, 0, (2048 + 4 + 512) * sizeof(uint32_t), ctx->stream));
    O.parity = 0;
  }
  out.slot_cost = O.slot_cost;
  const bool same_sig = std::memcmp(&sig, &O.cost_sig, sizeof sig) == 0;
  const bool same_launch = O.cost_tiles == (uint32_t)owned && same_sig &&
                           O.cost_range[0] == rq.spp_begin && O.cost_range[1] == rq.spp_count && env.force_smooth < 0;
  if (same_launch && O.order_exact && !env.no_order_reuse) {
    out.slot_order = O.slot_order; out.plan = O.hist + 2048; out.slot_cost = nullptr;
  } else if (O.cost_tiles == (uint32_t)owned) {
    if (O.order_exact) {
      TDT_HIP(ctx, hipMemcpyAsync(O.slot_cost, O.slot_acc, n * sizeof(uint32_t), hipMemcpyDeviceToDevice, ctx->stream));
      O.order_exact = false;
    }
    const int smooth = env.force_smooth >= 0 ? env.force_smooth : (same_sig ? 0 : 1);
    const bool keep_costs = !smooth && !env.no_cost_accum && O.cost_dispatches < 256;
    O.cost_dispatches = keep_costs ? O.cost_dispatches + 1 : 0;
    O.acc_samples = (keep_costs ? O.acc_samples : 0u) + O.last_launch_samples;
    const float blend = (!smooth && O.acc_samples < 16u) ? env.order_blend : 0.0f;
    if (smooth) O.acc_samples = 0;
    const uint32_t n_slots = (uint32_t)owned * 1024u, n_chunks = (n_slots + tdt::kOrderChunk - 1) / tdt::kOrderChunk;
    const uint32_t og = tdt::kOrderBits;
    uint32_t *hist = O.hist + 1024u * O.parity, *hist_next = O.hist + 1024u * (O.parity ^ 1u), *plan = O.hist + 2048;
    const uint32_t lanes = (uint32_t)ctx->num_cus * TDT_BLOCKS_PER_CU * TDT_BLOCK;
    hipLaunchKernelGGL(tdt::order_hist_kernel, dim3(n_chunks), dim3(1024), 0, ctx->stream, O.slot_cost, O.slot_acc, n_slots, hist, og, smooth, keep_costs ? 1 : 0, blend);
    hipLaunchKernelGGL(tdt::order_plan_kernel, dim3(1), dim3(512), 0, ctx->stream, hist, og, lanes, env.max_share, plan, smooth, hist_next, plan + 4);
    hipLaunchKernelGGL(tdt::order_scatter_kernel, dim3(n_chunks), dim3(1024), 0, ctx->stream, O.slot_cost, O.slot_acc, n_slots,
                       plan + 4, hist + 512, O.slot_order, og, smooth, blend);
    const hipError_t e = hipGetLastError();
    if (e != hipSuccess) {
      (void)hipMemsetAsync(O.hist, 0, (2048 + 4 + 512) * sizeof(uint32_t), ctx->stream);
      O.cost_tiles = 0; O.order_exact = false; O.parity = 0;
      return hip_fail(ctx, e, "cost-order sort");
    }
    O.parity ^= 1u;
    out.slot_order = O.slot_order; out.plan = plan;
    O.order_exact = same_launch && !smooth && blend == 0.0f;
  } else {
    TDT_HIP(ctx, hipMemsetAsync(O.slot_cost, 0, n * sizeof(uint32_t), ctx->stream));
    TDT_HIP(ctx, hipMemsetAsync(O.slot_acc, 0, n * sizeof(uint32_t), ctx->stream));
    O.cost_dispatches = 0; O.acc_samples = 0; O.order_exact = false;
  }
  if (out.slot_cost) {
    O.last_launch_samples = (uint32_t)(rq.spp_count > 0 ? rq.spp_count : 0);
    O.cost_sig = sig; O.cost_range[0] = rq.spp_begin; O.cost_range[1] = rq.spp_count;
    O.cost_tiles = (uint32_t)owned;
  }
  return TDT_OK;
}

int filter_done(tdt_ctx *ctx, const TraceState::MissPrepass &M, int owned, const uint32_t *&slot_order) {
  const uint32_t n_slots = (uint32_t)owned * 1024u, n_chunks = (n_slots + tdt::kFilterChunk - 1) / tdt::kFilterChunk;
  hipLaunchKernelGGL(tdt::filter_count_kernel, dim3(n_chunks), dim3(1024), 0, ctx->stream, slot_order, M.slot_done, n_slots, M.filter_counts);
  hipLaunchKernelGGL(tdt::filter_write_kernel, dim3(n_chunks), dim3(1024), 0, ctx->stream, slot_order, M.slot_done, n_slots, M.filter_counts, M.slot_live);
  TDT_HIP(ctx, hipGetLastError());
  slot_order = M.slot_live;
  return TDT_OK;
}

struct TreeForm { bool depth_ok, pow2, safev, resident, table_form = false, full = false, brick = false; };

TreeForm classify_tree(const TraceState &S, TraceParams &P) {
  const TraceState::Tables &T = S.tables;
  TreeForm f;
  const uint32_t cc = (uint32_t)P.cell_count;
  f.depth_ok = P.max_depth >= 0 && P.max_depth <= 30;
  f.pow2 = !S.env.force_generic && P.cell_count > 0 && (cc & (cc - 1)) == 0 && cc <= (1u << 22) &&
           P.inv_cell_count == 1.0f / (float)cc && f.depth_ok;
  f.safev = T.max_parent_value < (1u << 22);
  f.resident = (P.cells_dwords >> 1) > 0 && T.live_nodes <= P.lds_nodes && T.max_any_value <= tdt::kPackedMaxValue;
  if (f.resident && !S.env.no_specialise) P.lds_nodes = (T.live_nodes + 7u) & ~7u;
  return f;
}

int prepare_thresholds(tdt_ctx *ctx, TraceState &S, TreeForm &f, TraceParams &P) {
  TraceState::Tables &T = S.tables;
  if (f.pow2 || S.env.force_generic || S.env.no_specialise || S.env.no_table_form || !f.depth_ok || P.cell_count <= 0 || P.lds_nodes == 0) return TDT_OK;
  const uint32_t lds_cells = (P.lds_nodes + 7u) >> 3;
  const uint32_t n_thr = f.resident ? lds_cells : (lds_cells < tdt::kThrTopCells ? lds_cells : tdt::kThrTopCells);
  TraceState::ThresholdKey key{P.cell_count, 0, n_thr};
  std::memcpy(&key.ic_bits, &P.inv_cell_count, 4);
  if (!(T.thr_key == key)) {
    if (!T.thr) TDT_HIP(ctx, S.alloc(T.thr, ((size_t)tdt::kLdsCells + 1) * 2));
    uint32_t *aux = reinterpret_cast<uint32_t *>(T.thr + (size_t)tdt::kLdsCells * 2);
    TDT_HIP(ctx, hipMemsetAsync(aux, 0, 2 * sizeof(uint32_t), ctx->stream));
    hipLaunchKernelGGL(tdt::build_thresholds_kernel, dim3((n_thr + 255u) / 256u), dim3(256), 0, ctx->stream, P.inv_cell_count, P.cell_count, n_thr,
                       reinterpret_cast<float2 *>(T.thr), aux, (float4 *)nullptr);
    TDT_HIP(ctx, hipGetLastError());
    uint32_t res[2] = {1, 0};
    TDT_HIP(ctx, hipMemcpyAsync(res, aux, sizeof res, hipMemcpyDeviceToHost, ctx->stream));
    TDT_HIP(ctx, hipStreamSynchronize(ctx->stream));
    T.thr_key = key; T.thr_ok = res[0] == 0;
    std::memcpy(&T.thr_f0max, &res[1], 4);
  }
  f.table_form = T.thr_ok && (!f.resident || T.max_parent_value < n_thr);
  P.thr = T.thr; P.thr_cells = n_thr; P.thr_f0max = T.thr_f0max;
  return TDT_OK;
}

int prepare_full_grid(tdt_ctx *ctx, TraceState &S, TreeForm &f, TraceParams &P) {
  TraceState::Tables &T = S.tables;
  if (!f.pow2 || !f.safev || !f.resident || S.env.no_specialise || S.env.no_full || (P.max_depth != 5 && P.max_depth != 6)) return TDT_OK;
  const tdt_buffer *cb = ctx->ssbo[TDT_SLOT_CELLS];
  const TraceState::TableKey key{cb, cb->version, P.max_depth};
  if (!(T.full_key == key)) {
    const size_t entries = (size_t)1 << (3 * P.max_depth);
    if (!T.full_grid) TDT_HIP(ctx, S.alloc(T.full_grid, ((size_t)1 << 18) + 2));
    uint32_t *bad = reinterpret_cast<uint32_t *>(T.full_grid + ((size_t)1 << 18));
    TDT_HIP(ctx, hipMemsetAsync(bad, 0, sizeof(uint32_t), ctx->stream));
    hipLaunchKernelGGL(tdt::build_full_grid_kernel<tdt::kFullEntryForm>, dim3((unsigned)((entries + 255) / 256)), dim3(256), 0, ctx->stream, P.cells, P.cells_dwords, P.max_depth, T.full_grid, bad);
    TDT_HIP(ctx, hipGetLastError());
    uint32_t flag = 1;
    TDT_HIP(ctx, hipMemcpyAsync(&flag, bad, sizeof flag, hipMemcpyDeviceToHost, ctx->stream));
    TDT_HIP(ctx, hipStreamSynchronize(ctx->stream));
    T.full_key = key; T.full_ok = flag == 0;
  }
  f.full = T.full_ok;
  P.full_grid = T.full_grid;
  return TDT_OK;
}

int prepare_bricks(tdt_ctx *ctx, TraceState &S, TreeForm &f, TraceParams &P) {
  TraceState::Tables &T = S.tables;
  if (!f.pow2 || !f.safev || f.resident || S.env.no_specialise || S.env.no_bricks || P.max_depth < 6 || P.max_depth > 10) return TDT_OK;
  const tdt_buffer *cb = ctx->ssbo[TDT_SLOT_CELLS];
  const TraceState::TableKey key{cb, cb->version, P.max_depth};
  if (!(T.brick_key == key)) {
    const bool has_bricks = tdt::brick_levels(P.max_depth) != 0u;
    const size_t need = has_bricks ? ((size_t)1 << 15) * tdt::brick_entries(P.max_depth) * sizeof(uint16_t) : 0;
    if (!T.brick_grid) TDT_HIP(ctx, S.alloc(T.brick_grid, ((size_t)1 << 15) + 1));
    if (S.grow(T.bricks_bytes, need, {{T.bricks, need / sizeof(uint16_t)}}) != hipSuccess) {
      (void)hipGetLastError();
      S.env.no_bricks = true;
      return TDT_OK;
    }
    uint32_t *bad = T.brick_grid + ((size_t)1 << 15);
    TDT_HIP(ctx, hipMemsetAsync(bad, 0, sizeof(uint32_t), ctx->stream));
    switch (tdt::brick_levels(P.max_depth)) {
#define TDT_BUILD_BRICKS(B) case B: hipLaunchKernelGGL(tdt::build_bricks_kernel<B>, dim3(1u << 15), dim3(256), 0, ctx->stream, P.cells, P.cells_dwords, T.brick_grid, T.bricks, bad); break
      TDT_BUILD_BRICKS(1); TDT_BUILD_BRICKS(2); TDT_BUILD_BRICKS(3); TDT_BUILD_BRICKS(4);
      default: TDT_BUILD_BRICKS(0);
#undef TDT_BUILD_BRICKS
    }
    TDT_HIP(ctx, hipGetLastError());
    uint32_t flag = 1;
    TDT_HIP(ctx, hipMemcpyAsync(&flag, bad, sizeof flag, hipMemcpyDeviceToHost, ctx->stream));
    TDT_HIP(ctx, hipStreamSynchronize(ctx->stream));
    T.brick_key = key; T.brick_ok = flag == 0;
  }
  f.brick = T.brick_ok;
  if (f.brick) {
    P.brick_grid = T.brick_grid; P.bricks = T.bricks;
    if (P.lds_nodes > tdt::kBrickLdsCells * 8u) P.lds_nodes = tdt::kBrickLdsCells * 8u;
  }
  return TDT_OK;
}

int launch_trace(tdt_ctx *ctx, TraceState &S, const LaunchRequest &rq, const TreeForm &f, int owned, const TraceParams &P) {
  unsigned nblk = (unsigned)(((long)owned * 1024 + 1023) / 1024);
  if (nblk > (unsigned)ctx->num_cus * TDT_BLOCKS_PER_CU) nblk = (unsigned)ctx->num_cus * TDT_BLOCKS_PER_CU;
  const dim3 grid(nblk, 1, 1), block(TDT_BLOCK, 1, 1);
  bool launched = false;
  if (!rq.counts_out && (f.pow2 || f.table_form) && f.safev && !S.env.no_specialise) {
    const bool unit = P.scale == 1.0f && P.inv_scale == 1.0f && P.min_x != 0.0f && P.min_y != 0.0f && P.min_z != 0.0f && !rq.probe;
    const int form = f.pow2 ? tdt::FORM_POW2 : tdt::FORM_TABLE;
    TraceFn fn = nullptr;
    if (f.brick) fn = find_variant(form, P.max_depth, false, false, true, unit);
    if (!fn && f.full) fn = find_variant(form, P.max_depth, true, true, false, unit);
    if (!fn) fn = find_variant(form, P.max_depth, f.resident, false, false, unit);
    if (fn) {
      hipLaunchKernelGGL(fn, grid, block, 0, ctx->stream, P); launched = true;
      const int v[6] = {form, P.max_depth, (f.brick || !f.resident) ? 0 : 1, (!f.brick && f.full) ? 1 : 0, f.brick ? 1 : 0, unit ? 1 : 0};
      std::memcpy(S.last_variant, v, sizeof v);
    }
  }
  if (!launched) { const int v[6] = {f.pow2 ? tdt::FORM_POW2 : tdt::FORM_LITERAL, 0, 0, 0, 0, 0}; std::memcpy(S.last_variant, v, sizeof v); }
#define TDT_LAUNCH(C) do { if (f.pow2) hipLaunchKernelGGL((tdt::trace_kernel<C, tdt::FORM_POW2>), grid, block, 0, ctx->stream, P); \
                           else hipLaunchKernelGGL((tdt::trace_kernel<C, tdt::FORM_LITERAL>), grid, block, 0, ctx->stream, P); } while (0)
  if (!launched && rq.counts_out && getenv("TDT_COUNT_SPECIALISED") && f.pow2 && f.safev && f.resident && P.max_depth == 6) {
    hipLaunchKernelGGL((tdt::trace_kernel<true, tdt::FORM_POW2, 6, true, true>), grid, block, 0, ctx->stream, P); launched = true;
  }
  if (launched) {}
  else if (!rq.counts_out) TDT_LAUNCH(false);
  else TDT_LAUNCH(true);
#undef TDT_LAUNCH
  TDT_HIP(ctx, hipGetLastError());
  S.queue.parity ^= 1u;
  return TDT_OK;
}

int launch(tdt_compute *c, int width, int height, int depth, const LaunchRequest &rq) {
  (void)depth;
  tdt_ctx *ctx = c->ctx;
  TraceState &S = *ctx->trace;
  TraceParams P; Cover k; Tiles t;
  if (int rc = bind_params(c, width, height, rq, P, k, t)) return rc;
  if (rq.kind == LaunchRequest::kMissPrepass) return launch_miss_prepass(ctx, S, t.owned, P);
  if (rq.kind == LaunchRequest::kResolve) return launch_resolve(ctx, t.owned, P);
  if (int rc = begin_instrumented(ctx, S, rq, t.owned, P)) return rc;
  if (t.owned > 0) {
    if (int rc = bind_queue(ctx, S.queue, S.mem, P)) return rc;
    if (int rc = refresh_packed(ctx, S, P)) return rc;
    if (!S.env.no_cost_order) {
      CostSig sig; HandOut h;
      make_sig(ctx, c, k, ctx->image0, &sig);
      if (int rc = plan_order(ctx, S, sig, rq, t.owned, h)) return rc;
      P.slot_order = h.slot_order; P.plan = h.plan; P.slot_cost = h.slot_cost;
    }
    if (rq.prepass_ran && !rq.counts_out)
      if (int rc = filter_done(ctx, S.miss, t.owned, P.slot_order)) return rc;
    TreeForm f = classify_tree(S, P);
    if (!rq.counts_out) {
      if (int rc = prepare_thresholds(ctx, S, f, P)) return rc;
      if (int rc = prepare_full_grid(ctx, S, f, P)) return rc;
      if (int rc = prepare_bricks(ctx, S, f, P)) return rc;
    }
    if (int rc = launch_trace(ctx, S, rq, f, t.owned, P)) return rc;
  }
  if (rq.counts_out) {
    TDT_HIP(ctx, hipMemcpyAsync(rq.counts_out, ctx->counters, 8 * sizeof(unsigned long long), hipMemcpyDeviceToHost, ctx->stream));
    TDT_HIP(ctx, hipStreamSynchronize(ctx->stream));
  }
  return TDT_OK;
}

}

static unsigned long long next_buffer_version() {
  static std::atomic<unsigned long long> next_version{1};
  return next_version.fetch_add(1);
}

int tdt::adopt_device_buffer(tdt_ctx *ctx, void *dev, size_t bytes, tdt_buffer **out) {
  tdt_buffer *b = new (std::nothrow) tdt_buffer();
  if (!b) return fail(ctx, TDT_ERR_HIP, "out of host memory");
  b->ctx = ctx; b->bytes = bytes; b->dev = dev; b->version = next_buffer_version();
  const size_t head = bytes < sizeof b->shadow ? bytes : sizeof b->shadow;
  hipError_t e = hipSetDevice(ctx->device);
  if (e == hipSuccess && head) e = hipMemcpyAsync(b->shadow, dev, head, hipMemcpyDeviceToHost, ctx->stream);
  if (e == hipSuccess) e = hipStreamSynchronize(ctx->stream);
  if (e != hipSuccess) { delete b; return hip_fail(ctx, e, "adopt_device_buffer"); }
  ctx->buffers.push_back(b);
  *out = b;
  return TDT_OK;
}

extern "C" {

int tdt_ctx_create(int device_id, void *stream, tdt_ctx **out) {
  if (!out) return fail(nullptr, TDT_ERR_INVALID_VALUE, "null out pointer");
  *out = nullptr;
  int n = 0;
  hipError_t e = hipGetDeviceCount(&n);
  if (e != hipSuccess || n <= 0)
    return fail(nullptr, TDT_ERR_NO_DEVICE, std::string("no HIP device: ") + (e != hipSuccess ? hipGetErrorString(e) : "device count is 0"));
  if (device_id < 0 || device_id >= n) return fail(nullptr, TDT_ERR_INVALID_VALUE, "device id out of range");
  e = hipSetDevice(device_id);
  if (e != hipSuccess) return fail(nullptr, TDT_ERR_NO_DEVICE, std::string("hipSetDevice: ") + hipGetErrorString(e));
  tdt_ctx *ctx = new (std::nothrow) tdt_ctx();
  if (!ctx) return fail(nullptr, TDT_ERR_HIP, "out of host memory");
  ctx->device = device_id;
  ctx->trace = new (std::nothrow) tdt::TraceState();
  if (!ctx->trace) { delete ctx; return fail(nullptr, TDT_ERR_HIP, "out of host memory"); }
  { hipDeviceProp_t prop; ctx->num_cus = (hipGetDeviceProperties(&prop, device_id) == hipSuccess && prop.multiProcessorCount > 0) ? prop.multiProcessorCount : 256; }
  if (stream) { ctx->stream = (hipStream_t)stream; ctx->own_stream = false; }
  else {
    e = hipStreamCreateWithFlags(&ctx->stream, hipStreamNonBlocking);
    if (e != hipSuccess) { delete ctx->trace; delete ctx; return fail(nullptr, TDT_ERR_NO_DEVICE, std::string("hipStreamCreate: ") + hipGetErrorString(e)); }
    ctx->own_stream = true;
  }
  *out = ctx;
  return TDT_OK;
}

void tdt_ctx_destroy(tdt_ctx *ctx) {
  if (!ctx) return;
  if (ctx->multi) { tdt::multi_destroy(ctx); return; }
  (void)hipSetDevice(ctx->device);
  (void)hipStreamSynchronize(ctx->stream);
  for (tdt_compute *c : ctx->computes) delete c;
  for (tdt_buffer *b : ctx->buffers) { (void)hipFree(b->dev); delete b; }
  for (tdt_image *i : ctx->images) { if (i->owned) (void)hipFree(i->dev); delete i; }
  if (ctx->counters) (void)hipFree(ctx->counters);
  delete ctx->trace;
  tdt::edit_scratch_destroy(ctx);
  tdt::query_scratch_destroy(ctx);
  if (ctx->own_stream) (void)hipStreamDestroy(ctx->stream);
  delete ctx;
}

int tdt_finish(tdt_ctx *ctx) {
  if (!ctx) return TDT_ERR_INVALID_VALUE;
  if (ctx->multi) return tdt::multi_finish(ctx);
  TDT_HIP(ctx, hipSetDevice(ctx->device));
  TDT_HIP(ctx, hipStreamSynchronize(ctx->stream));
  return TDT_OK;
}

const char *tdt_last_error(const tdt_ctx *ctx) { return ctx ? ctx->err.c_str() : g_create_err.c_str(); }

// ... 343 lines not shown
int tdt_dispatch_resolve(tdt_compute *c, int width, int height, int depth, int total_spp) {
  if (!c) return TDT_ERR_INVALID_VALUE;
  if (c->kind != TDT_PROGRAM_RAYTRACER) return fail(c->ctx, TDT_ERR_INVALID_OPERATION, "not the raytracer program");
  if (c->ctx->multi) return tdt::multi_dispatch_resolve(c, width, height, depth, total_spp);
  LaunchRequest rq;
  rq.kind = LaunchRequest::kResolve; rq.total_spp = total_spp;
  return launch(c, width, height, depth, rq);
}

int64_t tdt_covered_pixels(const tdt_compute *c, int width, int height, int depth) {
  (void)depth;
  if (!c) return 0;
  return owned_pixels(c, cover_of(c, width, height));
}

int tdt_owned_tiles(const tdt_compute *c, int width, int height, int depth, int *tiles_x, int *tiles_total) {
  (void)depth;
  if (!c) return 0;
  Cover k = cover_of(c, width, height);
  Tiles t = tiles_of(c, k);
  if (tiles_x) *tiles_x = t.tiles_x;
  if (tiles_total) *tiles_total = t.total;
  return t.owned;
}

int tdt_dispatch_counted(tdt_compute *c, int width, int height, int depth, uint64_t counts[8]) {
  if (!c || !counts) return TDT_ERR_INVALID_VALUE;
  if (c->ctx->multi) return tdt::multi_dispatch_counted(c, width, height, depth, counts);
  if (c->kind != TDT_PROGRAM_RAYTRACER) return fail(c->ctx, TDT_ERR_INVALID_OPERATION, "not the raytracer program");
  static_assert(sizeof(unsigned long long) == sizeof(uint64_t), "");
  LaunchRequest rq;
  rq.spp_count = rq.total_spp = c->samples_per_pixel; rq.counts_out = reinterpret_cast<unsigned long long *>(counts);
  return launch(c, width, height, depth, rq);
}

int tdt_dispatch_counted_range(tdt_compute *c, int width, int height, int depth, int spp_begin, int spp_count, void *carry,
                               uint64_t counts[8]) {
  if (!c || !counts) return TDT_ERR_INVALID_VALUE;
  if (c->ctx->multi) return fail(c->ctx, TDT_ERR_INVALID_OPERATION, "progressive passes are a single-device feature (per-device carry memory)");
  if (c->kind != TDT_PROGRAM_RAYTRACER) return fail(c->ctx, TDT_ERR_INVALID_OPERATION, "not the raytracer program");
  if (spp_begin < 0 || spp_count < 0) return fail(c->ctx, TDT_ERR_INVALID_VALUE, "negative sample range");
  if (carry && ((uintptr_t)carry & 15) != 0) return fail(c->ctx, TDT_ERR_INVALID_VALUE, "carry memory must be 16-byte aligned");
  LaunchRequest rq;
  rq.kind = LaunchRequest::kAccumulate; rq.spp_begin = spp_begin; rq.spp_count = spp_count; rq.carry = carry;
  rq.counts_out = reinterpret_cast<unsigned long long *>(counts);
  return launch(c, width, height, depth, rq);
}

int tdt_forget_costs(tdt_ctx *ctx) {
  if (!ctx) return TDT_ERR_INVALID_VALUE;
  if (ctx->multi) return tdt::multi_forget_costs(ctx);
  tdt::TraceState::CostOrder &O = ctx->trace->order;
  O.cost_tiles = 0; O.cost_dispatches = 0; O.order_exact = false;
  return TDT_OK;
}

int tdt_debug_phase_timing(tdt_ctx *ctx, int enable, float ms[3]) {
  if (!ctx) return TDT_ERR_INVALID_VALUE;
  TDT_HIP(ctx, hipSetDevice(ctx->device));
  if (ms) ms[0] = ms[1] = ms[2] = 0.f;
  if (!ctx->trace) return TDT_OK;
  tdt::TraceState &S = *ctx->trace;
  if (ms && S.phase_timing && S.phase_n >= 2) {
    TDT_HIP(ctx, hipEventSynchronize(S.phase_ev[S.phase_n - 1]));
    for (int i = 0; i + 1 < S.phase_n; i++) TDT_HIP(ctx, hipEventElapsedTime(&ms[S.phase_n == 2 ? 1 : i], S.phase_ev[i], S.phase_ev[i + 1]));
  }
  if (enable && !S.phase_timing) {
    for (auto &e : S.phase_ev) TDT_HIP(ctx, hipEventCreate(&e));
    S.phase_timing = true; S.phase_n = 0;
  } else if (!enable && S.phase_timing) {
    for (auto &e : S.phase_ev) (void)hipEventDestroy(e);
    S.phase_timing = false; S.phase_n = 0;
  }
  return TDT_OK;
}

int tdt_debug_last_variant(const tdt_ctx *ctx, int out[6]) {
  if (!ctx || !out) return TDT_ERR_INVALID_VALUE;
  if (ctx->multi) ctx = tdt::multi_first_member(const_cast<tdt_ctx *>(ctx));
  std::memcpy(out, ctx->trace->last_variant, 6 * sizeof(int));
  return TDT_OK;
}

int tdt_debug_trace_variants(int *rows, int capacity, int *count) {
  if (!count || capacity < 0 || (capacity > 0 && !rows)) return TDT_ERR_INVALID_VALUE;
  int n = 0;
  for (const TraceVariant &v : kTraceVariants) {
    if (n < capacity) {
      const int r[6] = {v.form, v.depth, v.resident ? 1 : 0, v.full ? 1 : 0, v.brick ? 1 : 0, v.unit ? 1 : 0};
      std::memcpy(rows + 6 * n, r, sizeof r);
    }
    n++;
  }
  *count = n;
  return TDT_OK;
}

int tdt_debug_stats(tdt_ctx *ctx, uint64_t *out, int n_words, int reset) {
  if (!ctx) return TDT_ERR_INVALID_VALUE;
  if (ctx->multi) ctx = tdt::multi_first_member(ctx);
#ifdef TDT_STATS
  TDT_HIP(ctx, hipSetDevice(ctx->device));
  unsigned long long *&stats = ctx->trace->stats;
  const bool fresh = stats == nullptr;
  constexpr size_t kStatWords = tdt::STAT_COUNT + 1 + 8192;
  if (fresh) TDT_HIP(ctx, ctx->trace->alloc(stats, kStatWords));
  TDT_HIP(ctx, hipStreamSynchronize(ctx->stream));
  const size_t n_out = n_words > 0 ? ((size_t)n_words < kStatWords ? (size_t)n_words : kStatWords) : (size_t)tdt::STAT_COUNT;
  if (out && !fresh) TDT_HIP(ctx, hipMemcpy(out, stats, n_out * sizeof(uint64_t), hipMemcpyDeviceToHost));
  else if (out) std::memset(out, 0, n_out * sizeof(uint64_t));
  if (reset || fresh) {
    std::vector<unsigned long long> init(kStatWords, 0ull);
    init[tdt::STAT_T_FIRST] = ~0ull; init[tdt::STAT_COUNT] = ~0ull;
    TDT_HIP(ctx, hipMemcpy(stats, init.data(), kStatWords * sizeof(unsigned long long), hipMemcpyHostToDevice));
  }
  return TDT_OK;
#else
  (void)out; (void)n_words; (void)reset;
  return fail(ctx, TDT_ERR_INVALID_OPERATION, "pass statistics need a -DTDT_STATS build of the library (tools/loss_budget.py)");
#endif
}

int tdt_debug_counters(tdt_ctx *ctx, uint64_t out[32]) {
  if (!ctx || !out || !ctx->counters) return TDT_ERR_INVALID_VALUE;
  TDT_HIP(ctx, hipSetDevice(ctx->device));
  TDT_HIP(ctx, hipMemcpy(out, ctx->counters, 32 * sizeof(uint64_t), hipMemcpyDeviceToHost));
  return TDT_OK;
}
int tdt_debug_pixel_log(tdt_ctx *ctx, uint32_t *out, size_t n_u32) {
  if (!ctx || !out || !ctx->trace || !ctx->trace->pixel_log || n_u32 > ctx->trace->pixel_log_u32) return TDT_ERR_INVALID_VALUE;
  TDT_HIP(ctx, hipSetDevice(ctx->device));
  TDT_HIP(ctx, hipMemcpy(out, ctx->trace->pixel_log, n_u32 * 4, hipMemcpyDeviceToHost));
  return TDT_OK;
}
int tdt_debug_wave_ends(tdt_ctx *ctx, uint64_t *out, int n) {
  if (!ctx || !out || !ctx->counters || n < 0 || n > 16384 + 256) return TDT_ERR_INVALID_VALUE;
  TDT_HIP(ctx, hipSetDevice(ctx->device));
  TDT_HIP(ctx, hipMemcpy(out, ctx->counters + 32, (size_t)n * sizeof(uint64_t), hipMemcpyDeviceToHost));
  return TDT_OK;
}

static int selftest_full_grid(tdt_ctx *front, int which, uint64_t *mismatches) {
  tdt_ctx *ctx = front->multi ? tdt::multi_first_member(front) : front;
  TDT_HIP(front, hipSetDevice(ctx->device));
  TraceParams P;
  std::memset(&P, 0, sizeof P);
  const tdt_buffer *cb = ctx->ssbo[TDT_SLOT_CELLS];
  if (!cb) return tdt::fail(front, TDT_ERR_INCOMPLETE, "tdt_selftest 17: no cells buffer bound");
  if (int rc = tdt::octree_uniforms(ctx, P)) return rc;
  if (P.max_depth != 5 && P.max_depth != 6) return tdt::fail(front, TDT_ERR_INVALID_OPERATION, "tdt_selftest 17: max_depth must be 5 or 6");
  if (cb->bytes > 0xFFFFFFF8ull) return tdt::fail(front, TDT_ERR_INVALID_OPERATION, "tdt_selftest 17: cells buffer too large");
  const uint32_t *cells = (const uint32_t *)cb->dev;
  const uint32_t cells_dwords = (uint32_t)(cb->bytes >> 2), buf_nodes = cells_dwords >> 1;
  const uint32_t staged = buf_nodes < tdt::kLdsCells * 8u ? (buf_nodes & ~7u) : tdt::kLdsCells * 8u;
  const size_t entries = (size_t)1 << (3 * P.max_depth);
  tdt::DeviceScratch mem;
  FullGridEntry *grid = which == 17 ? mem.get<FullGridEntry>(entries) : nullptr;
  FullGridEntry64 *grid_planes = which == 18 ? mem.get<FullGridEntry64>(entries) : nullptr;
  uint16_t *grid16 = mem.get<uint16_t>(entries), *packed = mem.get<uint16_t>((size_t)tdt::kLdsCells * 8);
  unsigned long long *words = mem.get<unsigned long long>(4);
  if ((!grid && !grid_planes) || !grid16 || !packed || !words) return tdt::hip_fail(front, hipErrorOutOfMemory, "tdt_selftest 17");
  uint32_t *bad = reinterpret_cast<uint32_t *>(words + 1), *scan = reinterpret_cast<uint32_t *>(words + 2);
  TDT_HIP(front, hipMemsetAsync(words, 0, 4 * sizeof(unsigned long long), ctx->stream));
  if (staged) hipLaunchKernelGGL(tdt::pack_cells_kernel, dim3((staged + 255) / 256), dim3(256), 0, ctx->stream, cells, cells_dwords, packed, staged);
  if (buf_nodes) {
    unsigned nb = (buf_nodes + 255) / 256; if (nb > 4096) nb = 4096;
    hipLaunchKernelGGL(tdt::scan_cells_kernel, dim3(nb), dim3(256), 0, ctx->stream, cells, buf_nodes, scan);
  }
  const dim3 blocks((unsigned)((entries + 255) / 256));
  if (which == 17) hipLaunchKernelGGL(tdt::build_full_grid_kernel<tdt::kFullEntryForm>, blocks, dim3(256), 0, ctx->stream, cells, cells_dwords, P.max_depth, grid, bad);
// ... 81 lines not shown
```

### tdt4230_project_raytracing_amd/csrc/trace_device.hpp

```cpp
#pragma once
#include <hip/hip_runtime.h>
#include <stdint.h>

#include "trace_params.h"

namespace tdt {

#define TDT_DEV __device__ __forceinline__
#ifdef TDT_MARKERS
#define TDT_MARK(name) asm volatile("; TDT_MARK " #name)
#else
#define TDT_MARK(name) do {} while (0)
#endif

enum : int { FORM_LITERAL = 0, FORM_POW2 = 1, FORM_TABLE = 2 };

TDT_DEV float f_fract(float x) { return x - __builtin_floorf(x); }
TDT_DEV float f_fract_nonneg(float x) { return __builtin_amdgcn_fractf(x); }
TDT_DEV float f_rcp(float x) { return 1.0f / x; }
TDT_DEV float f_rsq(float x) { return 1.0f / __builtin_sqrtf(x); }

TDT_DEV bool exp_in_window(float x) {
  return ((__float_as_uint(x) & 0x7FFFFFFFu) - 0x0D800000u) < 0x65000000u;
}
// ... 49 lines not shown
TDT_DEV float hw_min(float a, float b) { return __builtin_fminf(a, b); }
TDT_DEV float hw_max(float a, float b) { return __builtin_fmaxf(a, b); }
TDT_DEV float b2f(bool b) { return b ? 1.0f : 0.0f; }
TDT_DEV int32_t f2i(float f) {
  return (f > -2147483904.0f && f < 2147483648.0f) ? (int32_t)f : (int32_t)0x80000000;
}

TDT_DEV void sincos_poly(float a, float &s_out, float &c_out) {
  float x = __builtin_fabsf(a);
  int32_t j = f2i(x * 1.27323954473516f);
  j = (j + 1) & ~1;
  float y = (float)j;
  x = __builtin_fmaf(y, -0.78515625f, x);
  x = __builtin_fmaf(y, -2.4187564849853515625e-4f, x);
  x = __builtin_fmaf(y, -3.77489497744594108e-8f, x);
  float z = x * x;
  float c = 2.443315711809948e-5f;
  c = __builtin_fmaf(c, z, -1.388731625493765e-3f);
  c = __builtin_fmaf(c, z, 4.166664568298827e-2f);
  c = c * z;
  c = c * z;
  c = __builtin_fmaf(-0.5f, z, c);
  c = c + 1.0f;
  float s = -1.9515295891e-4f;
  s = __builtin_fmaf(s, z, 8.3321608736e-3f);
  s = __builtin_fmaf(s, z, -1.6666654611e-1f);
  s = s * z;
  s = __builtin_fmaf(s, x, x);
  float rs = ((j & 2) == 0) ? s : c;
  bool neg_s = (((j & 4) != 0) != ((__float_as_uint(a) >> 31) != 0));
  s_out = neg_s ? -rs : rs;
  int32_t k = j - 2;
  float rc = ((k & 2) == 0) ? s : c;
  c_out = (((~k) & 4) != 0) ? -rc : rc;
}
TDT_DEV float sin_poly(float a) { float s, c; sincos_poly(a, s, c); return s; }

TDT_DEV float pow_poly(float x, float yy) {
  uint32_t u = __float_as_uint(x);
  float e = (float)((int32_t)((u >> 23) & 0xff) - 127);
  float m = __uint_as_float((u & 0x007fffffu) | 0x3f800000u);
  float t = pow_t(m);
  float z = t * t;
  float z2 = z * z;
  float even = __builtin_fmaf(z2, __builtin_fmaf(z2, 0.406718052498846252698f, 0.577440339438736392009f), 2.88539009343309178325f);
  float odd = __builtin_fmaf(z2, 0.403343858251329912514f, 0.961791550404184197881f);
  float p = __builtin_fmaf(odd, z, even);
  float l2 = __builtin_fmaf(t, p, e);
  float w = l2 * yy;
  w = f_min(f_max(w, -126.99999f), 128.0f);
  float i = __builtin_floorf(w);
  float f = w - i;
  float f2 = f * f;
  float ev = __builtin_fmaf(f2, __builtin_fmaf(f2, 0.00898934009049466391101f, 0.240153617044375388211f), 1.0f);
  float od = __builtin_fmaf(f2, __builtin_fmaf(f2, 0.00187757667519147912699f, 0.0558263180532956664775f), 0.693153073200168932794f);
  float q = __builtin_fmaf(od, f, ev);
  int32_t ii = f2i(i);
  return __uint_as_float((uint32_t)(ii + 127) << 23) * q;
}

TDT_DEV uint32_t ld_dw(const uint32_t *buf, uint32_t dwords, uint32_t byte_off) {
  uint32_t i = byte_off >> 2;
  return (i < dwords) ? buf[i] : 0u;
}

#ifndef TDT_LDS_CELLS
#define TDT_LDS_CELLS 5120
#endif
constexpr uint32_t kLdsCells = TDT_LDS_CELLS;
constexpr uint32_t kPackedEscape = 0xFFFFu;
constexpr uint32_t kPackedMaxValue = 0x3FFEu;

struct NodeSource {
  const uint16_t *lds;
  uint32_t lds_nodes;
  uint32_t lds_cells;
  const void *grid;
  bool grid_ok; float grid_band;
  const FullGridEntry *full;
  const float2 *planes; float vmin_x, vmin_y, vmin_z;
  const uint32_t *grid32; const void *bricks;
  const float2 *thr; float thr_f0max;
  __amdgpu_buffer_rsrc_t cells;
};

TDT_DEV uint32_t fetch_node(const NodeSource &ns, uint32_t idx, uint32_t &code) {
  idx &= 0x1FFFFFFFu;
  {
    const uint32_t n = ns.lds[idx < ns.lds_nodes ? idx : ns.lds_nodes];
    if (n != kPackedEscape) { code = n & 3u; return n >> 2; }
  }
  const auto n2 = __builtin_amdgcn_raw_buffer_load_b64(ns.cells, (int)(idx << 3), 0, 0);
  const uint32_t node_type = (uint32_t)n2[1];
  code = (node_type == 0u) ? 0u : (node_type == 2u ? 2u : 1u);
  return (uint32_t)n2[0];
}

struct Counters {
  uint32_t octree_hit_calls, iterations, node_loads, lambertian, metal, dielectric, unknown;
  uint32_t trav_slots, trav_active, level_slots, level_active, event_slots, event_active,
           scatter_slots, scatter_active, memo_miss, leaf_records;
};
TDT_DEV uint32_t slot64() {
  const unsigned long long m = __ballot(1);
  return ((threadIdx.x & 63) == (uint32_t)__builtin_ctzll(m)) ? 64u : 0u;
}

struct Ray { float ox, oy, oz, dx, dy, dz; };
struct HitTmp { float nx, ny, nz, px, py, pz; bool ff; };
struct Carry { HitTmp root; float root_t; HitTmp leaf; };
struct Hit { float px, py, pz, nx, ny, nz; bool ff; uint32_t index; };

TDT_DEV void cube_normal_literal(const Ray &r, float nx, float ny, float nz, HitTmp &h) {
  float ax = __builtin_fabsf(nx), ay = __builtin_fabsf(ny), az = __builtin_fabsf(nz);
  nx = nx * b2f(ax >= f_max(ay, az));
  ny = ny * b2f(f_max(ax, az) < ay);
  nz = nz * b2f(f_max(ax, ay) < az);
  float rs = q_rsq((nz * nz + ny * ny) + nx * nx);
  nx = nx * rs; ny = ny * rs; nz = nz * rs;
  bool ff = (r.dz * nz + r.dy * ny) < -(r.dx * nx);
  float flip = -2.0f * b2f(!ff) + 1.0f;
  nx = nx * flip; ny = ny * flip; nz = nz * flip;
  rs = q_rsq((nz * nz + ny * ny) + nx * nx);
  h.nx = nx * rs; h.ny = ny * rs; h.nz = nz * rs;
  h.ff = ff;
}
TDT_DEV bool cube_normal_fast_ok(float nx, float ny, float nz, bool &sx, bool &sy, bool &sz) {
  const float ax = __builtin_fabsf(nx), ay = __builtin_fabsf(ny), az = __builtin_fabsf(nz);
  sx = ax >= hw_max(ay, az); sy = hw_max(ax, az) < ay; sz = hw_max(ax, ay) < az;
  const float sum = (ax + ay) + az;
  return (sx || sy || sz) && (__float_as_uint(sum) - 0x27000000u) < (0x58000000u - 0x27000000u);
}
TDT_DEV void cube_normal_fast(const Ray &r, float nx, float ny, float nz, bool sx, bool sy, bool sz, HitTmp &h) {
  const uint32_t ex = (__float_as_uint(nx) & 0x80000000u) | (sx ? 0x3F800000u : 0u);
  const uint32_t ey = (__float_as_uint(ny) & 0x80000000u) | (sy ? 0x3F800000u : 0u);
  const uint32_t ez = (__float_as_uint(nz) & 0x80000000u) | (sz ? 0x3F800000u : 0u);
  const bool ff = (r.dz * __uint_as_float(ez) + r.dy * __uint_as_float(ey)) < -(r.dx * __uint_as_float(ex));
  const uint32_t fl = ff ? 0u : 0x80000000u;
  h.nx = __uint_as_float(ex ^ fl); h.ny = __uint_as_float(ey ^ fl); h.nz = __uint_as_float(ez ^ fl);
  h.ff = ff;
}
TDT_DEV void cube_hit_record(const Ray &r, float t, float cx, float cy, float cz, float size, HitTmp &h) {
  float px = t * r.dx + r.ox, py = t * r.dy + r.oy, pz = t * r.dz + r.oz;
  float radius = size * 0.5f;
  float nx = px + -(cx + radius), ny = py + -(cy + radius), nz = pz + -(cz + radius);
  h.px = px; h.py = py; h.pz = pz;
#ifdef TDT_LITERAL_NORMAL
  cube_normal_literal(r, nx, ny, nz, h);
#else
  bool sx, sy, sz;
  const bool ok = cube_normal_fast_ok(nx, ny, nz, sx, sy, sz);
  if (__builtin_expect(__ballot(!ok) != 0ull, 0)) cube_normal_literal(r, nx, ny, nz, h);
  else cube_normal_fast(r, nx, ny, nz, sx, sy, sz, h);
#endif
}

TDT_DEV void cube_slabs(const Ray &r, float ix, float iy, float iz, float cx, float cy, float cz, float size,
                        float t_min, float t_max, float &t_enter, float &t_exit) {
  float lx = (cx + -r.ox) * ix, ly = (cy + -r.oy) * iy, lz = (cz + -r.oz) * iz;
  float ux = ((cx + size) + -r.ox) * ix, uy = ((cy + size) + -r.oy) * iy, uz = ((cz + size) + -r.oz) * iz;
  float mnx = hw_min(lx, ux), mny = hw_min(ly, uy), mnz = hw_min(lz, uz);
  float mxx = hw_max(lx, ux), mxy = hw_max(ly, uy), mxz = hw_max(lz, uz);
  float e1, e3, x1, x3;
  asm("v_max_f32 %0, %1, %2" : "=v"(e1) : "v"(t_min), "v"(mnx));
  asm("v_max3_f32 %0, %1, %2, %3" : "=v"(e3) : "v"(e1), "v"(mny), "v"(mnz));
  asm("v_min_f32 %0, %1, %2" : "=v"(x1) : "v"(t_max), "v"(mxx));
  asm("v_min3_f32 %0, %1, %2, %3" : "=v"(x3) : "v"(x1), "v"(mxy), "v"(mxz));
  t_enter = e3; t_exit = x3;
}
TDT_DEV void cube_slabs_planes(const Ray &r, float ix, float iy, float iz, float cx, float cy, float cz, float hx, float hy, float hz,
                               float t_min, float t_max, float &t_enter, float &t_exit) {
  float lx = (cx + -r.ox) * ix, ly = (cy + -r.oy) * iy, lz = (cz + -r.oz) * iz;
  float ux = (hx + -r.ox) * ix, uy = (hy + -r.oy) * iy, uz = (hz + -r.oz) * iz;
  float mnx = hw_min(lx, ux), mny = hw_min(ly, uy), mnz = hw_min(lz, uz);
  float mxx = hw_max(lx, ux), mxy = hw_max(ly, uy), mxz = hw_max(lz, uz);
  float e1, e3, x1, x3;
  asm("v_max_f32 %0, %1, %2" : "=v"(e1) : "v"(t_min), "v"(mnx));
  asm("v_max3_f32 %0, %1, %2, %3" : "=v"(e3) : "v"(e1), "v"(mny), "v"(mnz));
  asm("v_min_f32 %0, %1, %2" : "=v"(x1) : "v"(t_max), "v"(mxx));
  asm("v_min3_f32 %0, %1, %2, %3" : "=v"(x3) : "v"(x1), "v"(mxy), "v"(mxz));
  t_enter = e3; t_exit = x3;
}

template <bool COUNT>
TDT_DEV bool tree_lookup(const TraceParams &P, const NodeSource &ns, float cx, float cy, float cz, float &inv_pow_depth,
                         float &gx, float &gy, float &gz, uint32_t &value, Counters &cnt) {
  float ipd = 1.0f, ux = 0.0f, uy = 0.0f, uz = 0.0f;
  uint32_t node_value = 0;
  bool is_leaf = false;
  const float two_cc = (float)(int32_t)((uint32_t)P.cell_count << 1);
  const float fdepth = (float)P.max_depth;
  for (float i = 0.0f; i < fdepth; i = i + 1.0f) {
    ipd = ipd * 0.5f;
    float fx = f_fract(cx), fy = f_fract(cy), fz = f_fract(cz);
    float rx = __builtin_rintf((((float)node_value + fx) * P.inv_cell_count) * two_cc + -0.5f);
    float ry = __builtin_rintf(fy * 2.0f + -0.5f);
    float rz = __builtin_rintf(fz * 2.0f + -0.5f);
    int32_t ix = f2i(rx), iy = f2i(ry), iz = f2i(rz);
    float tx = __builtin_truncf(rx), ty = __builtin_truncf(ry), tz = __builtin_truncf(rz);
    float bx = tx + -(2.0f * __builtin_floorf(tx / 2.0f));
    float by = ty + -(2.0f * __builtin_floorf(ty / 2.0f));
    float bz = tz + -(2.0f * __builtin_floorf(tz / 2.0f));
    ux = ux + bx * ipd; uy = uy + by * ipd; uz = uz + bz * ipd;
    uint32_t idx = (((uint32_t)ix << 1) + (uint32_t)iy);
    idx = (idx << 1) + (uint32_t)iz;
    uint32_t node_type;
    node_value = fetch_node(ns, idx, node_type);
    if (COUNT) cnt.node_loads++;
    if (node_type == 0u || node_type == 2u) { is_leaf = (node_type == 2u); break; }
    cx = cx * 2.0f; cy = cy * 2.0f; cz = cz * 2.0f;
  }
  inv_pow_depth = ipd; gx = ux; gy = uy; gz = uz; value = node_value;
  return is_leaf;
}

TDT_DEV int32_t x_index_literal(uint32_t v, float f, float inv_cell_count, float two_cc) {
  return f2i(__builtin_rintf((((float)v + f) * inv_cell_count) * two_cc + -0.5f));
}
TDT_DEV float x_threshold_need(float2 F, float f0max) {
  const float d1 = __builtin_fabsf(F.x - 0.5f), d2 = F.y <= 1.0f ? 1.0f - F.y : 0.0f;
  const float d = d1 > d2 ? d1 : d2;
  return d > f0max ? d : f0max;
}
TDT_DEV float4 x_thresholds(uint32_t v, float inv_cell_count, int32_t cell_count, uint32_t *bad) {
  const float two_cc = (float)(int32_t)((uint32_t)cell_count << 1);
  const int32_t base = (int32_t)(2u * v);
  const uint32_t kOne = 0x3F800000u;
  const int32_t g0 = x_index_literal(v, 0.0f, inv_cell_count, two_cc), g1 = x_index_literal(v, __uint_as_float(kOne - 1u), inv_cell_count, two_cc);
  if (v >= (1u << 22) || cell_count <= 0 || g0 < base - 1 || g0 > base || g1 < base + 1 || g1 > base + 2 || (v == 0u && g0 != 0)) {
    atomicOr(bad, 1u);
    return make_float4(2.0f, 2.0f, 0.0f, 0.0f);
  }
  auto first = [&](int32_t target) {
    uint32_t lo = 0u, hi = kOne;
    while (lo < hi) {
      const uint32_t mid = (lo + hi) >> 1;
      if (x_index_literal(v, __uint_as_float(mid), inv_cell_count, two_cc) >= target) hi = mid; else lo = mid + 1u;
    }
    return lo == kOne ? 2.0f : __uint_as_float(lo);
  };
  return make_float4(first(base + 1), first(base + 2), first(base), 0.0f);
}
template <int CL>
struct NodeMemo { uint32_t key[CL]; uint32_t val[CL]; };
constexpr int kNoProbeFrom = 6;
TDT_DEV uint32_t grid_v_bound(int level) { return level < 3 ? 128u : (level == 3 ? 1024u : 8192u); }
template <int GL> struct Grid;
template <> struct Grid<4> {
  static constexpr int kLevels = 4;
  static constexpr uint32_t kEntries = 1u << 12;
  static constexpr float kBand = 0x1.0p-12f;
  typedef uint32_t Entry;
  static TDT_DEV bool encode(uint32_t v, uint32_t m, uint32_t code, Entry &e) { e = (v << 5) | (m << 2) | code; return true; }
  static TDT_DEV void decode(uint32_t g, uint32_t &v, uint32_t &m, uint32_t &code) { code = g & 3u; m = (g >> 2) & 7u; v = g >> 5; }
};
template <> struct Grid<5> {
  static constexpr int kLevels = 5;
  static constexpr uint32_t kEntries = 1u << 15;
  static constexpr float kBand = 0x1.0p-11f;
  typedef uint16_t Entry;
  static TDT_DEV bool encode(uint32_t v, uint32_t m, uint32_t code, Entry &e) {
    if (code == 1u) { e = (Entry)((v << 2) | 1u); return v <= kPackedMaxValue && m == 5u; }
    e = (Entry)((v << 5) | (m << 2) | code);
    return v < 2048u;
  }
  static TDT_DEV void decode(uint32_t g, uint32_t &v, uint32_t &m, uint32_t &code) {
    code = g & 3u;
    const bool parent = code == 1u;
    m = parent ? 5u : (g >> 2) & 7u;
    v = parent ? g >> 2 : g >> 5;
  }
};
template <int GL, bool TABLE = false>
TDT_DEV void build_top_grid(const uint16_t *lds, uint32_t lds_nodes, int depth, typename Grid<GL>::Entry *grid, int *grid_ok,
                            const float2 *thr = nullptr, uint32_t thr_cells = 0u, float f0max = 0.0f, uint32_t *band_bits = nullptr) {
  constexpr int kGridLevels = GL;
  if (threadIdx.x == 0) { *grid_ok = depth >= kGridLevels ? 1 : 0; if (TABLE) *band_bits = 0u; }
  __syncthreads();
  if (depth >= kGridLevels) {
    for (uint32_t e = threadIdx.x; e < Grid<GL>::kEntries; e += blockDim.x) {
      const uint32_t xg = e >> (2 * kGridLevels), yg = (e >> kGridLevels) & ((1u << kGridLevels) - 1u), zg = e & ((1u << kGridLevels) - 1u);
      uint32_t v = 0, code = 1u, m = 0;
      bool ok = true;
      float need = 0.0f;
      for (int l = 1; l <= kGridLevels && code == 1u; l++) {
        const int sh = kGridLevels - l;
        if (TABLE) {
          if (v >= thr_cells) { ok = false; break; }
          const float n = x_threshold_need(thr[v], f0max) * (float)(2 << sh);
          need = n > need ? n : need;
        }
        const uint32_t idx = ((2u * v + ((xg >> sh) & 1u)) << 2) + (((yg >> sh) & 1u) << 1) + ((zg >> sh) & 1u);
        const uint32_t n = lds[idx < lds_nodes ? idx : lds_nodes];
        if (n == kPackedEscape) { ok = false; break; }
        v = n >> 2; code = n & 3u; m = (uint32_t)l;
        if (!TABLE && code == 1u && l < kGridLevels && v >= grid_v_bound(l)) ok = false;
      }
      if (code == 1u && m < (uint32_t)kGridLevels) ok = false;
      if (!Grid<GL>::encode(v, m, code, grid[e])) ok = false;
      if (!ok) atomicAnd(grid_ok, 0);
      if (TABLE) atomicMax(band_bits, __float_as_uint(need));
    }
  }
  __syncthreads();
}

constexpr uint32_t kCostStep = 3, kCostEvent = 64, kCostRayStep = 7;
constexpr uint32_t kEventWindow = 1024;
constexpr int kMemoLevels = 9;
constexpr int kBrickMemoLevels = 3;
__host__ __device__ constexpr int top_grid_levels(bool resident, bool table) { return (resident || table) ? 4 : 5; }
constexpr uint32_t kThrTopCells = 1024u;
constexpr int kMemoFirst = 3;

__host__ __device__ constexpr uint32_t brick_levels(int depth) { return depth >= 6 && depth <= 9 ? (uint32_t)(depth - 5) : 0u; }
__host__ __device__ constexpr uint32_t brick_entries(int depth) { uint32_t n = 1u; for (uint32_t j = 0; j < brick_levels(depth); j++) n *= 12u; return n; }
constexpr uint32_t kBrickLdsCells = 1024u;
TDT_DEV int brick_band_exp(int l, uint32_t v) { return (v == 0u ? -40 : (31 - (int)__builtin_clz(v)) + 5 - l - 23); }
TDT_DEV float brick_q(uint32_t e, float f) { const float V = __uint_as_float((127u + e) << 23); return (V + f) - V; }
constexpr int kFullEntryBits = TDT_FULL_ENTRY_BITS;
constexpr int kFullPlanes = 65;
constexpr int kFullEntryForm = TDT_FULL_ENTRY_PLANES ? kFullPlanes : kFullEntryBits;
template <int BITS> struct FullEntry;
template <> struct FullEntry<16> { typedef uint16_t Type; };
template <> struct FullEntry<32> { typedef uint32_t Type; };
template <> struct FullEntry<64> { typedef FullGridEntry64 Type; };
template <> struct FullEntry<kFullPlanes> { typedef FullGridEntry64 Type; };
// ... 7 lines not shown
    f = j >= kCells ? 1u : 0u; const uint32_t c = j - f * kCells + 2u;
    m = 31u - (uint32_t)__builtin_clz(c); k = c - (1u << m);
  }
};
template <bool UNIT>
TDT_DEV float2 slab_planes(float ug, float ipd, bool leaf, float scale, float vmin) {
  const float b = (UNIT ? ug : ug * scale) + vmin;
  const float lo = b + (leaf ? -0.0f : -0.00001f);
  const float cs0 = UNIT ? ipd : scale * ipd;
  const float cs = leaf ? cs0 : cs0 + 0.00002f;
  return make_float2(lo, lo + cs);
}
template <int DEPTH, bool UNIT>
TDT_DEV void build_plane_table(float2 *t, float scale, float min_x, float min_y, float min_z) {
  static_assert(DEPTH >= 1 && DEPTH <= 6, "PlaneTable::kCells");
  for (uint32_t i = threadIdx.x; i < PlaneTable::kEntries; i += blockDim.x) {
    uint32_t a, f, m, k;
    PlaneTable::cell(i, a, f, m, k);
    if (m > (uint32_t)DEPTH) continue;
    const float ipd = __uint_as_float((127u - m) << 23);
    t[i] = slab_planes<UNIT>((float)k * ipd, ipd, f != 0u, scale, a == 0u ? min_x : (a == 1u ? min_y : min_z));
  }
}
struct CellPlanes { float lox, loy, loz, hix, hiy, hiz; };
template <int BITS>
TDT_DEV bool full_entry_encode(uint32_t meta16, int depth, uint32_t xg, uint32_t yg, uint32_t zg, typename FullEntry<BITS>::Type &e) {
  if constexpr (BITS == 16) { e = (uint16_t)meta16; return true; }
  else if constexpr (BITS == kFullPlanes) {
    const uint32_t sh = (meta16 >> 2) & 7u, m = (uint32_t)depth - sh, f = (meta16 & 3u) == 2u ? 1u : 0u;
    if (depth > 6 || m < 1u) { e.w0 = meta16; e.w1 = 0u; return false; }
    e.w0 = (PlaneTable::index(0u, f, m, xg >> sh) << 19) | meta16;
    e.w1 = (PlaneTable::index(1u, f, m, yg >> sh) << 19) | (PlaneTable::index(2u, f, m, zg >> sh) << 3);
    return true;
  } else {
    const uint32_t sh = (meta16 >> 2) & 7u;
    const float ipd = __uint_as_float(((127u - (uint32_t)depth) << 23) + (sh << 23));
    const uint32_t cx = __float_as_uint((float)(xg >> sh) * ipd), cy = __float_as_uint((float)(yg >> sh) * ipd), cz = __float_as_uint((float)(zg >> sh) * ipd);
    if constexpr (BITS == 32) { e = (cx & 0xFFFF0000u) | meta16; return (cx & 0xFFFFu) == 0u; }
    else { e.w0 = (cx & 0xFFFF0000u) | meta16; e.w1 = (cy & 0xFFFF0000u) | (cz >> 16); return ((cx | cy | cz) & 0xFFFFu) == 0u; }
  }
}
template <int BITS, int DEPTH>
TDT_DEV bool full_entry_decode(const typename FullEntry<BITS>::Type &g, uint32_t xg, uint32_t Yi, uint32_t Zi, float &gx, float &gy, float &gz, float &ipd, uint32_t &value) {
  uint32_t meta;
  if constexpr (BITS == 64 || BITS == kFullPlanes) meta = g.w0; else meta = g;
  const uint32_t sh = (meta >> 2) & 7u;
  ipd = __uint_as_float(((127u - (uint32_t)DEPTH) << 23) + (sh << 23));
  if constexpr (BITS == kFullPlanes) {
    const uint32_t off[3] = {g.w0 >> 16, g.w1 >> 16, g.w1 & 0xFFFFu};
    float c[3];
    for (uint32_t a = 0; a < 3u; a++) {
      uint32_t ta, tf, tm, tk;
      PlaneTable::cell(off[a] >> 3, ta, tf, tm, tk);
      const bool ok = (off[a] & 7u) == 0u && (off[a] >> 3) < PlaneTable::kEntries && ta == a && tm == (uint32_t)DEPTH - sh && tf == ((meta & 3u) == 2u ? 1u : 0u);
      c[a] = ok ? (float)tk * ipd : __builtin_nanf("");
    }
    gx = c[0]; gy = c[1]; gz = c[2];
    value = (meta >> 5) & 0x7FFu;
  } else
  if constexpr (BITS == 16) {
    gx = (float)(xg >> sh) * ipd; gy = (float)(Yi >> sh) * ipd; gz = (float)(Zi >> sh) * ipd;
    value = meta >> 5;
  } else if constexpr (BITS == 32) {
    gx = __uint_as_float(meta & 0xFFFF0000u); gy = (float)(Yi >> sh) * ipd; gz = (float)(Zi >> sh) * ipd;
    value = (meta >> 5) & 0x7FFu;
  } else {
    gx = __uint_as_float(meta & 0xFFFF0000u); gy = __uint_as_float(g.w1 & 0xFFFF0000u); gz = __uint_as_float(g.w1 << 16);
    value = (meta >> 5) & 0x7FFu;
  }
  return (meta & 3u) == 2u;
}
template <int DEPTH>
TDT_DEV bool full_entry_planes(const FullGridEntry64 &g, const float2 *planes, CellPlanes &cp, float &ipd, uint32_t &value) {
  const char *base = reinterpret_cast<const char *>(planes);
  const float2 px = *reinterpret_cast<const float2 *>(base + (g.w0 >> 16));
  const float2 py = *reinterpret_cast<const float2 *>(base + (g.w1 >> 16));
  const float2 pz = *reinterpret_cast<const float2 *>(base + (g.w1 & 0xFFFFu));
  cp.lox = px.x; cp.hix = px.y; cp.loy = py.x; cp.hiy = py.y; cp.loz = pz.x; cp.hiz = pz.y;
  const uint32_t sh = (g.w0 >> 2) & 7u;
  ipd = __uint_as_float(((127u - (uint32_t)DEPTH) << 23) + (sh << 23));
  value = (g.w0 >> 5) & 0x7FFu;
  return (g.w0 & 3u) == 2u;
}
template <bool COUNT, int CL, int DEPTH, bool RESIDENT, bool SAFEV, bool FULL = false, bool BRICK = false, bool TABLE = false, bool UNIT = false>
TDT_DEV bool tree_lookup_pow2(const TraceParams &P, const NodeSource &ns, float fx, float fy, float fz, float &inv_pow_depth,
                              float &gx, float &gy, float &gz, uint32_t &value, NodeMemo<CL> &memo, Counters &cnt, CellPlanes *cp = nullptr) {
  static_assert(!TABLE || (SAFEV && !BRICK && !FULL), "per-cell thresholds: the resident walk, or (trees outside the LDS table) the jump table's bands only");
  constexpr bool PLANES = FULL && !COUNT && kFullEntryForm == kFullPlanes;
  const int depth = DEPTH > 0 ? DEPTH : P.max_depth;
  const float scale_d = __uint_as_float((uint32_t)(127 + depth) << 23);
  const float Yf = fy * scale_d, Zf = fz * scale_d;
  const float Yfl = __builtin_floorf(Yf), Zfl = __builtin_floorf(Zf);
  uint32_t Yi = (uint32_t)Yfl, Zi = (uint32_t)Zfl;
  if (__builtin_expect(__ballot((Yf == Yfl) | (Zf == Zfl)) != 0ull, 0)) {
    Yi = (Yf == Yfl) ? (Yi & (Yi - 1u)) : Yi;
    Zi = (Zf == Zfl) ? (Zi & (Zi - 1u)) : Zi;
  }
  uint32_t qx = 1u, v = 0, code = 1u;
  const float fx0 = fx;
  bool jumped = false;
  constexpr int kTableLevels = top_grid_levels(RESIDENT, TABLE);
  constexpr int kGridLevels = FULL ? DEPTH : kTableLevels;
  if constexpr (FULL && !COUNT) {
    const float tg = fx0 * (float)(1 << DEPTH);
    const bool safe = __builtin_fabsf(tg - __builtin_rintf(tg)) > ns.grid_band;
    if (__builtin_expect(__ballot(!safe) == 0ull, 1)) {
      const uint32_t xg = (uint32_t)tg;
      const FullGridEntry g = ns.full[(xg << (2 * DEPTH)) | (Yi << DEPTH) | Zi];
      if constexpr (PLANES) return full_entry_planes<DEPTH>(g, ns.planes, *cp, inv_pow_depth, value);
      else return full_entry_decode<kFullEntryBits, DEPTH>(g, xg, Yi, Zi, gx, gy, gz, inv_pow_depth, value);
    }
  } else if constexpr (BRICK && !COUNT) {
    static_assert(!BRICK || (DEPTH >= 6 && DEPTH <= 10 && !RESIDENT && SAFEV), "the 32-bit table: trees of depth 6-10 outside the LDS table");
    constexpr int BL = (int)brick_levels(DEPTH);
    const float tg = fx0 * 32.0f;
    const uint32_t xg = (uint32_t)tg;
    const uint32_t e = (xg << 10) | ((Yi >> (DEPTH - 5)) << 5) | (Zi >> (DEPTH - 5));
    const uint32_t g = ns.grid32[e];
    const float band = __uint_as_float((116u - (g >> 29)) << 23);
    if constexpr (BL == 0) {
      if (__builtin_expect(__ballot(!(__builtin_fabsf(tg - __builtin_rintf(tg)) > band)) == 0ull, 1)) {
        code = g & 3u;
        const bool parent = code == 1u;
        const uint32_t mg = parent ? 5u : (g >> 2) & 15u;
        v = parent ? (g >> 2) & 0x3FFFFFu : (g >> 6) & 0x7FFFFFu;
        qx = (1u << mg) | (xg >> (5u - mg));
        fx = f_fract_nonneg(tg);
        jumped = true;
      }
    } else
    if (__builtin_expect((__ballot(!(__builtin_fabsf(tg - __builtin_rintf(tg)) > band)) | __ballot((g & 0x7Fu) == 0x7Du)) == 0ull, 1)) {
      uint32_t ent = g & 0x1FFFFFFFu, xd = xg << BL;
      if ((g & 3u) == 1u) {
        uint32_t ci = 0u, xlow = 0u;
#pragma unroll
        for (int j = 0; j < BL; j++) {
          const float f = j == 0 ? f_fract_nonneg(tg) : f_fract_nonneg(fx0 * (float)(32 << j));
          const float q = brick_q((g >> (2 + 5 * j)) & 31u, f);
          const uint32_t a = q > 0.5f ? 1u : 0u, b = q == 1.0f ? 1u : 0u;
          ci = ci * 3u + a + b;
          xlow = (xlow << 1) | (a & ~b);
        }
        constexpr uint32_t kCombos = BL == 1 ? 3u : (BL == 2 ? 9u : (BL == 3 ? 27u : 81u)), kMask = (1u << BL) - 1u;
        const uint32_t bi = ((__umul24(e, kCombos) + ci) << (2 * BL)) | ((Yi & kMask) << BL) | (Zi & kMask);
        ent = static_cast<const uint16_t *>(ns.bricks)[bi];
        xd |= xlow;
      }
      const uint32_t sh = (ent >> 2) & 15u;
      const float ipd = __uint_as_float(((127u - (uint32_t)DEPTH) << 23) + (sh << 23));
      gx = (float)(xd >> sh) * ipd; gy = (float)(Yi >> sh) * ipd; gz = (float)(Zi >> sh) * ipd;
      inv_pow_depth = ipd;
      value = ent >> 6;
      return (ent & 3u) == 2u;
    }
  } else if constexpr (!COUNT && DEPTH >= kTableLevels) {
    const float tg = fx0 * (float)(1 << kGridLevels);
    const bool safe = __builtin_fabsf(tg - __builtin_rintf(tg)) > ns.grid_band;
    if (__builtin_expect(__ballot(!safe) == 0ull, 1)) {
      const uint32_t xg = (uint32_t)tg;
      const uint32_t g = static_cast<const typename Grid<kTableLevels>::Entry *>(ns.grid)[(xg << (2 * kGridLevels)) | ((Yi >> (depth - kGridLevels)) << kGridLevels) | (Zi >> (depth - kGridLevels))];
      uint32_t mg;
      Grid<kTableLevels>::decode(g, v, mg, code);
      qx = (1u << mg) | (xg >> ((uint32_t)kGridLevels - mg));
      fx = f_fract_nonneg(tg);
      jumped = true;
    }
  }
  auto level = [&](int l, uint32_t *mkey, uint32_t *mval) {
    const int sh = depth - l;
    const float fv = (float)v;
    if (COUNT) { cnt.level_slots += slot64(); cnt.level_active++; cnt.node_loads++; }
    if (RESIDENT && SAFEV) {
      const uint32_t cell = v < ns.lds_cells ? v : ns.lds_cells;
      const uint4 c = *reinterpret_cast<const uint4 *>(ns.lds + (cell << 3));
      bool a, b, low = false;
      if constexpr (TABLE) { const float2 F = ns.thr[cell]; a = fx >= F.x; b = fx >= F.y; low = fx < ns.thr_f0max; }
      else { const float q = (fv + fx) - fv; a = q > 0.5f; b = (q == 1.0f); }
      uint32_t bitx = (a && !b) ? 1u : 0u;
      const uint32_t yb = (Yi >> sh) & 1u, zb = (Zi >> sh) & 1u;
      const uint32_t lo = a ? c.z : c.x, hi = a ? c.w : c.y;
      uint32_t n = ((yb ? hi : lo) >> (zb << 4)) & 0xFFFFu;
      if (__builtin_expect(__ballot(b || low) != 0ull, 0)) {
        if (b || low) {
          uint32_t ix = 2u * v + 2u;
          if constexpr (TABLE) if (low) {
            ix = (uint32_t)x_index_literal(v, fx, P.inv_cell_count, (float)(int32_t)((uint32_t)P.cell_count << 1));
            bitx = ix & 1u;
          }
          const uint32_t idx = ((ix << 2) + (yb << 1) + zb) & 0x1FFFFFFFu;
          n = ns.lds[idx < ns.lds_nodes ? idx : ns.lds_nodes];
        }
      }
      qx = qx + qx + bitx;
      v = n >> 2; code = n & 3u;
      fx = f_fract_nonneg(fx0 * __uint_as_float((uint32_t)(127 + l) << 23));
      return;
    }
    uint32_t ix; uint32_t bitx;
    if constexpr (TABLE) {
      const float two_cc = (float)(int32_t)((uint32_t)P.cell_count << 1);
      const float rx = __builtin_rintf(((fv + fx) * P.inv_cell_count) * two_cc + -0.5f);
      ix = (uint32_t)f2i(rx);
      const float tx = __builtin_truncf(rx);
      bitx = ((tx + -(2.0f * __builtin_floorf(tx / 2.0f))) != 0.0f) ? 1u : 0u;
    } else
    if (SAFEV || __builtin_expect(__ballot(v >= (1u << 22)) == 0ull, 1)) {
      const float q = (fv + fx) - fv;
      const bool a = q > 0.5f, b = (q == 1.0f);
      ix = (v + v + (uint32_t)a) + (uint32_t)b;
      bitx = (a && !b) ? 1u : 0u;
    } else {
      const float two_cc = (float)(int32_t)((uint32_t)P.cell_count << 1);
      const float rx = __builtin_rintf(((fv + fx) * P.inv_cell_count) * two_cc + -0.5f);
      ix = (uint32_t)f2i(rx);
      const float tx = __builtin_truncf(rx);
      bitx = ((tx + -(2.0f * __builtin_floorf(tx / 2.0f))) != 0.0f) ? 1u : 0u;
      if (v < (1u << 22)) {
        const float q = (fv + fx) - fv;
        const uint32_t a = q > 0.5f ? 1u : 0u, b = (q == 1.0f) ? 1u : 0u;
        ix = 2u * v + a + b; bitx = a & ~b;
      }
    }
    qx = qx + qx + bitx;
    const uint32_t idx = ((ix << 2) + (((Yi >> sh) & 1u) << 1) + ((Zi >> sh) & 1u)) & 0x1FFFFFFFu;
    bool resident = false;
    if (RESIDENT || l < kNoProbeFrom) {
      const uint32_t li = idx < ns.lds_nodes ? idx : ns.lds_nodes;
      const uint32_t n = ns.lds[li];
      resident = RESIDENT || (n != kPackedEscape);
      v = n >> 2; code = n & 3u;
    }
    if (!resident) {
      if (mkey && (*mkey & 0x1FFFFFFFu) == idx) {
        v = *mval; code = *mkey >> 30;
      } else {
        if (COUNT) cnt.memo_miss++;
        const auto n2 = __builtin_amdgcn_raw_buffer_load_b64(ns.cells, (int)(idx << 3), 0, 0);
        const uint32_t node_type = (uint32_t)n2[1];
        code = (node_type == 0u) ? 0u : (node_type == 2u ? 2u : 1u);
        v = (uint32_t)n2[0];
        if (mkey) { *mkey = idx | (code << 30); *mval = v; }
      }
    }
    fx = f_fract_nonneg(fx0 * __uint_as_float((uint32_t)(127 + l) << 23));
  };
  constexpr int kFirstAfterJump = (kGridLevels > kMemoFirst ? kGridLevels : kMemoFirst) + 1;
  TDT_MARK(walk);
  if (!jumped) {
#pragma unroll
    for (int l = 1; l <= kMemoFirst; l++) {
      if (code == 1u && l <= depth) level(l, nullptr, nullptr);
    }
#pragma unroll
    for (int l = kMemoFirst + 1; l < kFirstAfterJump; l++) {
      if (code == 1u && l <= depth) {
        if (l - kMemoFirst - 1 < CL) level(l, &memo.key[l - kMemoFirst - 1 < CL ? l - kMemoFirst - 1 : 0], &memo.val[l - kMemoFirst - 1 < CL ? l - kMemoFirst - 1 : 0]);
        else level(l, nullptr, nullptr);
      }
    }
  }
#pragma unroll
  for (int l = kFirstAfterJump; l <= kMemoFirst + CL; l++) {
    if (code == 1u && l <= depth) level(l, &memo.key[l - kMemoFirst - 1], &memo.val[l - kMemoFirst - 1]);
  }
  for (int l = (kMemoFirst + CL + 1 > kFirstAfterJump ? kMemoFirst + CL + 1 : kFirstAfterJump); code == 1u && l <= depth; l++) level(l, nullptr, nullptr);
  const int m = 31 - __builtin_clz(qx);
  qx ^= 1u << m;
  const float ipd = __uint_as_float((uint32_t)(127 - m) << 23);
  const int sh = depth - m;
  if constexpr (PLANES) {
    const bool leaf = code == 2u;
    const float2 px = slab_planes<UNIT>((float)qx * ipd, ipd, leaf, P.scale, ns.vmin_x), py = slab_planes<UNIT>((float)(Yi >> sh) * ipd, ipd, leaf, P.scale, ns.vmin_y),
                 pz = slab_planes<UNIT>((float)(Zi >> sh) * ipd, ipd, leaf, P.scale, ns.vmin_z);
    cp->lox = px.x; cp->hix = px.y; cp->loy = py.x; cp->hiy = py.y; cp->loz = pz.x; cp->hiz = pz.y;
    inv_pow_depth = ipd; value = v;
    return leaf;
  }
  gx = (float)qx * ipd; gy = (float)(Yi >> sh) * ipd; gz = (float)(Zi >> sh) * ipd;
  if (DEPTH > 0) {
    inv_pow_depth = ipd;
  } else {
    inv_pow_depth = (m == 0) ? 1.0f : ipd;
    if (m == 0) { gx = 0.f; gy = 0.f; gz = 0.f; }
  }
  value = v;
  return code == 2u;
}

TDT_DEV float rand2(float cx, float cy) {
  return f_fract(sin_poly(cy * 78.233f + cx * 12.9898f) * 43758.5453f);
}

struct MatSource { __amdgpu_buffer_rsrc_t materials, albedos, metal, dielectric; };
TDT_DEV __amdgpu_buffer_rsrc_t table_rsrc(const uint32_t *p, uint32_t dwords) {
  return __builtin_amdgcn_make_buffer_rsrc((void *)p, 0, (int)(dwords < (1u << 30) ? dwords << 2 : 0xFFFFFFFFu), 0x00020000);
}
TDT_DEV MatSource material_source(const TraceParams &P) {
  MatSource ms;
  ms.materials = table_rsrc(P.materials, P.materials_dwords); ms.albedos = table_rsrc(P.albedos, P.albedos_dwords);
  ms.metal = table_rsrc(P.metal, P.metal_dwords); ms.dielectric = table_rsrc(P.dielectric, P.dielectric_dwords);
  return ms;
}
TDT_DEV uint32_t ld_buf(__amdgpu_buffer_rsrc_t rs, uint32_t byte_off) { return (uint32_t)__builtin_amdgcn_raw_buffer_load_b32(rs, (int)byte_off, 0, 0); }
struct MatRef { uint32_t type, attribute, albedo; };
TDT_DEV MatRef material_fetch(const MatSource &ms, uint32_t index) {
  const uint32_t mo = index * 12u;
  MatRef m;
  m.type = ld_buf(ms.materials, mo);
  m.attribute = ld_buf(ms.materials, mo + 4u);
// ... 158 lines not shown
```

### tdt4230_project_raytracing_amd/rt.py

```python
import ctypes
import os

import numpy as np

_HERE = os.path.dirname(os.path.abspath(__file__))
LIB_PATH = os.environ.get("TDT_LIB") or os.path.join(_HERE, "libtdtrt.so")

OK, ERR_NO_DEVICE, ERR_HIP, ERR_VARIABLE_NOT_FOUND, ERR_INCOMPLETE = 0, 1, 2, 3, 4
ERR_INVALID_ENUM, ERR_INVALID_VALUE, ERR_INVALID_OPERATION = 0x0500, 0x0501, 0x0502
PROGRAM_RAYTRACER, PROGRAM_OCTREE_UPDATE = 0, 1
SHADER_STORAGE_BUFFER, ATOMIC_COUNTER_BUFFER = 0x90D2, 0x92C0

RAY_MISS, RAY_HIT, RAY_ITER_LIMIT = 0, 1, 2
RAY_HIT_DTYPE = np.dtype([("status", "<i4"), ("material", "<u4"), ("t", "<f4"), ("iterations", "<i4"),
                          ("point", "<f4", (3,)), ("normal", "<f4", (3,)), ("front_face", "<i4"), ("fresh_record", "<i4"),
                          ("cell_min", "<f4", (3,)), ("cell_size", "<f4")])
assert RAY_HIT_DTYPE.itemsize == 64


def hits_from_bytes(b):
    if hasattr(b, "detach"):
        b = b.detach().cpu().numpy()
    return np.ascontiguousarray(b, np.uint8).reshape(-1, 64).view(RAY_HIT_DTYPE).reshape(-1)

# ... 118 lines not shown

assert ctypes.sizeof(Xform) == 96


def _exact_ints(a, dtype, name):
    src = np.asarray(a)
    if src.size and src.dtype.kind not in "iu":
        raise ValueError(f"{name} must be integers, not {src.dtype}")
    out = np.ascontiguousarray(src.astype(dtype))
    if src.size and not np.array_equal(out.astype(object), src.astype(object)):
        raise ValueError(f"{name} holds values outside {np.dtype(dtype).name}")
    return out


def _mesh(vertices, triangles, materials, material):
    v = _exact_ints(vertices, np.int32, "vertices")
    t = _exact_ints(triangles, np.uint32, "triangles")
    if v.ndim != 2 or v.shape[1] != 3 or t.ndim != 2 or t.shape[1] != 3:
        raise ValueError("vertices and triangles must be (n, 3) arrays")
    m = None
    if materials is not None:
        m = _exact_ints(materials, np.int32, "materials").reshape(-1)
        if len(m) != len(t):
            raise ValueError(f"{len(m)} materials for {len(t)} triangles")
    if isinstance(material, bool) or int(material) != material or not -2**31 <= int(material) <= 2**31 - 1:
        raise ValueError(f"material must be an int32, not {material!r}")
    mesh = Mesh(v.ctypes.data if len(v) else None, t.ctypes.data if len(t) else None, m.ctypes.data if m is not None and len(m) else None,
                len(v), len(t), int(material), 0)
    return mesh, (v, t, m)


_P, _I, _U, _F, _S = ctypes.c_void_p, ctypes.c_int, ctypes.c_uint, ctypes.c_float, ctypes.c_size_t
_PP = ctypes.POINTER(ctypes.c_void_p)
SYMBOLS = [
    ("tdt_ctx_create", _I, [_I, _P, _PP]),
    ("tdt_ctx_create_multi", _I, [_I, ctypes.POINTER(ctypes.c_int), _PP]),
    ("tdt_ctx_device_count", _I, [_P]),
    ("tdt_ctx_destroy", None, [_P]),
    ("tdt_finish", _I, [_P]),
    ("tdt_last_error", ctypes.c_char_p, [_P]),
    ("tdt_strerror", ctypes.c_char_p, [_I]),
    ("tdt_compute_create", _I, [_P, _I, _PP]),
    ("tdt_compute_destroy", None, [_P]),
    ("tdt_compute_group_size", _I, [_P, ctypes.POINTER(ctypes.c_int)]),
    ("tdt_set_i32", _I, [_P, ctypes.c_char_p, ctypes.c_int32]),
    ("tdt_set_f32", _I, [_P, ctypes.c_char_p, _F]),
    ("tdt_set_vec3f", _I, [_P, ctypes.c_char_p, _F, _F, _F]),
    ("tdt_set_vec3i", _I, [_P, ctypes.c_char_p, ctypes.c_int32, ctypes.c_int32, ctypes.c_int32]),
    ("tdt_buffer_create", _I, [_P, _P, _S, _PP]),
    ("tdt_buffer_destroy", None, [_P]),
    ("tdt_bind_buffer_base", _I, [_P, _I, _U, _P]),
    ("tdt_buffer_sub_data", _I, [_P, _S, _S, _P]),
    ("tdt_buffer_read", _I, [_P, _S, _S, _P]),
    ("tdt_image_create_rgba32f", _I, [_P, _I, _I, _PP]),
    ("tdt_image_wrap_device", _I, [_P, _P, _I, _I, _PP]),
    ("tdt_image_destroy", None, [_P]),
    ("tdt_bind_image", _I, [_P, _U, _P]),
    ("tdt_image_width", _I, [_P]),
    ("tdt_image_height", _I, [_P]),
    ("tdt_image_device_ptr", _P, [_P]),
    ("tdt_image_read", _I, [_P, _P]),
    ("tdt_image_read_rgba8", _I, [_P, _I, _P]),
    ("tdt_dispatch_compute", _I, [_P, _I, _I, _I]),
    ("tdt_set_partition", _I, [_P, _I, _I]),
    ("tdt_dispatch_accumulate", _I, [_P, _I, _I, _I, _I, _I, _P]),
    ("tdt_dispatch_resolve", _I, [_P, _I, _I, _I, _I]),
    ("tdt_covered_pixels", ctypes.c_int64, [_P, _I, _I, _I]),
    ("tdt_owned_tiles", _I, [_P, _I, _I, _I, ctypes.POINTER(ctypes.c_int), ctypes.POINTER(ctypes.c_int)]),
    ("tdt_assemble_tiles", _I, [_P, _P, _I, _I, _P, _I, _I, _I]),
    ("tdt_dispatch_counted", _I, [_P, _I, _I, _I, ctypes.POINTER(ctypes.c_uint64)]),
    ("tdt_dispatch_counted_range", _I, [_P, _I, _I, _I, _I, _I, _P, ctypes.POINTER(ctypes.c_uint64)]),
    ("tdt_forget_costs", _I, [_P]),
    ("tdt_debug_phase_timing", _I, [_P, _I, ctypes.POINTER(ctypes.c_float)]),
    ("tdt_debug_multi_timing", _I, [_P, ctypes.POINTER(ctypes.c_float), ctypes.POINTER(ctypes.c_float), ctypes.POINTER(ctypes.c_float)]),
    ("tdt_debug_multi_transport", ctypes.c_char_p, [_P]),
    ("tdt_debug_multi_rccl_ranks", _I, [_P]),
    ("tdt_debug_multi_fail", _I, [_P, _I]),
    ("tdt_octree_build_cells", _I, [_P, _P, _S, _I, _PP, ctypes.POINTER(ctypes.c_uint32)]),
    ("tdt_octree_build_from_points", _I, [_P, _P, _S, ctypes.POINTER(ctypes.c_int32), _P, _P, _S, _I, _I, _PP,
                                          ctypes.POINTER(ctypes.c_int32), ctypes.POINTER(ctypes.c_int32)]),
    ("tdt_debug_edit_mode", _I, [_P, _I]),
    ("tdt_debug_last_edit_path", _I, [_P]),
    ("tdt_debug_last_variant", _I, [_P, ctypes.POINTER(ctypes.c_int)]),
    ("tdt_debug_trace_variants", _I, [ctypes.POINTER(ctypes.c_int), _I, ctypes.POINTER(ctypes.c_int)]),
    ("tdt_debug_counters", _I, [_P, ctypes.POINTER(ctypes.c_uint64)]),
    ("tdt_debug_stats", _I, [_P, ctypes.POINTER(ctypes.c_uint64), _I, _I]),
    ("tdt_debug_wave_ends", _I, [_P, ctypes.POINTER(ctypes.c_uint64), _I]),
    ("tdt_debug_pixel_log", _I, [_P, ctypes.c_void_p, ctypes.c_size_t]),
    ("tdt_raycast", _I, [_P, _P, _S, _P]),
    ("tdt_raycast_device", _I, [_P, _P, _S, _P]),
    ("tdt_pick_pixels", _I, [_P, _P, _S, _I, _P, _P]),
    ("tdt_octree_census", _I, [_P, ctypes.POINTER(ctypes.c_int64)]),
    ("tdt_octree_extract", _I, [_P, _P, _S, ctypes.POINTER(ctypes.c_size_t)]),
    ("tdt_octree_compact", _I, [_P, ctypes.POINTER(ctypes.c_uint32)]),
    ("tdt_octree_edit_region", _I, [_P, _I, _P, _S, ctypes.c_int32, ctypes.POINTER(ctypes.c_uint32)]),
    ("tdt_octree_edit_voxels", _I, [_P, _I, _P, _S, ctypes.POINTER(ctypes.c_uint32)]),
    ("tdt_octree_extract_region", _I, [_P, _P, _S, _P, _S, ctypes.POINTER(ctypes.c_size_t)]),
    ("tdt_octree_components", _I, [_P, _I, _I, _P, _S, ctypes.POINTER(ctypes.c_size_t), _P, _S, ctypes.POINTER(ctypes.c_size_t)]),
    ("tdt_octree_edit_connected", _I, [_P, _I, ctypes.POINTER(Select), _P, _S, _P, _S, ctypes.c_int32, ctypes.POINTER(ctypes.c_uint32)]),
    ("tdt_octree_extract_connected", _I, [_P, ctypes.POINTER(Select), _P, _S, _P, _S, _P, _S, ctypes.POINTER(ctypes.c_size_t)]),
    ("tdt_octree_morph", _I, [_P, ctypes.POINTER(Morph), _P, _S, ctypes.POINTER(ctypes.c_uint32)]),
    ("tdt_octree_extract_morph", _I, [_P, ctypes.POINTER(Morph), _P, _S, _P, _S, ctypes.POINTER(ctypes.c_size_t)]),
    ("tdt_voxelize_triangles", _I, [_P, ctypes.POINTER(Mesh), _I, _P, _S, ctypes.POINTER(ctypes.c_size_t)]),
    ("tdt_octree_edit_triangles", _I, [_P, _I, ctypes.POINTER(Mesh), ctypes.POINTER(ctypes.c_uint32)]),
    ("tdt_octree_extract_enclosed", _I, [_P, ctypes.POINTER(Fill), _P, _S, _P, _S, ctypes.POINTER(ctypes.c_size_t)]),
    ("tdt_octree_fill_enclosed", _I, [_P, ctypes.POINTER(Fill), _P, _S, ctypes.POINTER(ctypes.c_uint32)]),
    ("tdt_voxelize_triangles_solid", _I, [_P, ctypes.POINTER(Mesh), _I, ctypes.POINTER(Fill), _P, _S, ctypes.POINTER(ctypes.c_size_t)]),
    ("tdt_octree_edit_triangles_solid", _I, [_P, _I, ctypes.POINTER(Mesh), ctypes.POINTER(Fill), ctypes.POINTER(ctypes.c_uint32)]),
    ("tdt_debug_fill_passes", _I, [_P]),
    ("tdt_octree_extract_surface", _I, [_P, ctypes.POINTER(Surface), _P, _S, _P, _S, ctypes.POINTER(ctypes.c_size_t)]),
    ("tdt_octree_morph_round", _I, [_P, ctypes.POINTER(Round), _P, _S, ctypes.POINTER(ctypes.c_uint32)]),
    ("tdt_octree_extract_morph_round", _I, [_P, ctypes.POINTER(Round), _P, _S, _P, _S, ctypes.POINTER(ctypes.c_size_t)]),
    ("tdt_octree_distance_field", _I, [_P, ctypes.POINTER(ctypes.c_int32), ctypes.POINTER(ctypes.c_int32), ctypes.c_int32, ctypes.c_int32,
                                       _P, _P, _S, ctypes.POINTER(ctypes.c_size_t)]),
    ("tdt_octree_extract_transform", _I, [_P, ctypes.POINTER(Xform), _P, _S, _P, _S, ctypes.POINTER(ctypes.c_size_t)]),
    ("tdt_octree_transform", _I, [_P, ctypes.POINTER(Xform), _I, _P, _S, ctypes.POINTER(ctypes.c_uint32)]),
    ("tdt_debug_xform_bricks", _I, [_P, ctypes.POINTER(ctypes.c_uint32)]),
    ("tdt_selftest", _I, [_P, _I, ctypes.POINTER(ctypes.c_uint64)]),
    ("tdt_selftest_index", _I, [_P, ctypes.c_int32, _F, ctypes.c_uint32, _I, ctypes.POINTER(ctypes.c_uint64), ctypes.POINTER(ctypes.c_int)]),
]

_lib = None


def lib():
    global _lib
    if _lib is None:
        if not os.path.exists(LIB_PATH):
            raise RuntimeError(f"{LIB_PATH} is missing — build it with `python -c 'import __graft_entry__ as g; g.build()'`; "
                               "the trace has no CPU fallback")
        try:
            import torch
        except ImportError:
            pass
        L = ctypes.CDLL(LIB_PATH)
        for name, res, args in SYMBOLS:
            try:
                f = getattr(L, name)
            except AttributeError:
                if os.environ.get("TDT_LIB"):
                    continue
                raise
            f.restype = res
            f.argtypes = args
        _lib = L
    return _lib


class TdtError(RuntimeError):

    def __init__(self, code, message):
        super().__init__(f"[{code:#x}] {message}")
        self.code = code


class Context:

    def __init__(self, device=0, stream=None, devices=None):
        h = ctypes.c_void_p()
        if devices is not None:
            ids = (ctypes.c_int * len(devices))(*[int(d) for d in devices])
            rc = lib().tdt_ctx_create_multi(len(devices), ids, ctypes.byref(h))
            device = devices[0] if len(devices) else 0
        else:
            rc = lib().tdt_ctx_create(int(device), ctypes.c_void_p(stream) if stream else None, ctypes.byref(h))
        if rc != OK:
# ... 292 lines not shown
            self.check(lib().tdt_octree_extract_morph_round(self.h, ctypes.byref(r), arr, k, out.ctypes.data, n.value, ctypes.byref(n)))
        return out

    def octree_distance_field(self, lo, hi, max_d2, border=0, nearest=False):
        box3 = []
        for name, c in (("lo", lo), ("hi", hi)):
            c = list(c)
            if len(c) != 3:
                raise ValueError(f"{name} must hold three coordinates")
            box3.append((ctypes.c_int32 * 3)(*[self._int32(name, v) for v in c]))
        max_d2, border = self._int32("max_d2", max_d2), self._int32("border", border, allow_bool=True)
        n = ctypes.c_size_t(0)
        self.check(lib().tdt_octree_distance_field(self.h, box3[0], box3[1], max_d2, border, None, None, 0, ctypes.byref(n)))
        ex, ey, ez = (int(box3[1][a]) - int(box3[0][a]) + 1 for a in range(3))
        field = np.zeros((ez, ey, ex), np.int32)
        near = np.zeros((ez, ey, ex, 3), np.int32) if nearest else None
        assert field.size == n.value
        self.check(lib().tdt_octree_distance_field(self.h, box3[0], box3[1], max_d2, border, field.ctypes.data,
                                                   near.ctypes.data if nearest else None, field.size, ctypes.byref(n)))
        return (field, near) if nearest else field

    @classmethod
    def _xform(cls, xf):
        if isinstance(xf, Xform):
            get = lambda k, d: getattr(xf, k)
        elif isinstance(xf, dict):
            get = lambda k, d: xf.get(k, d)
        else:
            raise ValueError(f"xf must be an rt.Xform or a dict, not {type(xf).__name__}")

        def ints(name, v, count, bits):
            v = list(v)
            if len(v) != count:
                raise ValueError(f"{name} must hold {count} entries")
            for e in v:
                if isinstance(e, (bool, np.bool_)) or int(e) != e or not -2 ** (bits - 1) <= int(e) <= 2 ** (bits - 1) - 1:
                    raise ValueError(f"{name} must hold int{bits} values, not {e!r}")
            return [int(e) for e in v]
        material = get("material", -1)
        out = Xform()
        out.t[:] = ints("t", get("t", (0, 0, 0)), 3, 64)
        out.a[:] = ints("a", get("a", (XFORM_ONE, 0, 0, 0, XFORM_ONE, 0, 0, 0, XFORM_ONE)), 9, 32)
        out.material = cls._int32("material", -1 if material is None else material)
        out.dst_lo[:] = ints("dst_lo", get("dst_lo", (0, 0, 0)), 3, 32)
        out.dst_hi[:] = ints("dst_hi", get("dst_hi", (2 ** 31 - 1,) * 3), 3, 32)
        out.pad[:] = ints("pad", get("pad", (0, 0)), 2, 32)
        return out

    def octree_transform(self, xf, op=REGION_SET, regions=None):
        x = self._xform(xf)
        op = self._int32("op", op)
        arr, k = _touch_regions(regions)
        n = ctypes.c_uint32(0)
        self._check_edit(lib().tdt_octree_transform(self.h, ctypes.byref(x), op, arr, k, ctypes.byref(n)), n)
        return int(n.value)

    def octree_extract_transform(self, xf, regions=None):
        x = self._xform(xf)
        arr, k = _touch_regions(regions)
        n = ctypes.c_size_t(0)
        self.check(lib().tdt_octree_extract_transform(self.h, ctypes.byref(x), arr, k, None, 0, ctypes.byref(n)))
        out = np.zeros((n.value, 4), np.int32)
        if n.value:
            self.check(lib().tdt_octree_extract_transform(self.h, ctypes.byref(x), arr, k, out.ctypes.data, n.value, ctypes.byref(n)))
        return out

    def xform_bricks(self):
        out = (ctypes.c_uint32 * 2)()
        self.check(lib().tdt_debug_xform_bricks(self.h, out))
        return int(out[0]), int(out[1])

    def fill_passes(self):
        return int(lib().tdt_debug_fill_passes(self.h))

    def bind_buffer_base(self, target, slot, vbo):
        self.check(lib().tdt_bind_buffer_base(self.h, target, slot, vbo.h if vbo is not None else None))

    def selftest(self, which):
        n = ctypes.c_uint64(0)
        self.check(lib().tdt_selftest(self.h, which, ctypes.byref(n)))
        return n.value

    def last_variant(self):
        v = (ctypes.c_int * 6)()
        self.check(lib().tdt_debug_last_variant(self.h, v))
        return dict(zip(("form", "depth", "resident", "full", "brick", "unit"), [int(x) for x in v]))

    STAT_NAMES = ("trav_pass", "trav_lanes", "inside_lanes", "alive_lanes", "event_pass", "event_lanes", "hit_pass", "hit_lanes", "lamb_pass", "lamb_lanes",
                  "metal_pass", "metal_lanes", "diel_pass", "diel_lanes", "end_pass", "end_lanes", "pixel_end_pass", "pixel_end_lanes", "fetch_pass", "fetch_lanes",
                  "primary_pass", "primary_lanes", "newray_pass", "newray_lanes", "gate_wait_lanes", "drained_trav_pass", "drained_event_pass", "loop_pass",
                  "wave_ticks", "waves", "t_first", "t_last")

    def stats(self, reset=True):
        n = 32 + 1 + 8192
        v = (ctypes.c_uint64 * n)()
        self.check(lib().tdt_debug_stats(self.h, v, n, 1 if reset else 0))
        d = dict(zip(self.STAT_NAMES, [int(x) for x in v[:32]]))
        d["t_queue_dry"] = int(v[32])
        d["wave_ends"] = [int(x) for x in v[33:33 + min(int(v[29]), 8192)]]
        return d

    def selftest_index(self, cell_count, inv_cell_count, n_cells, shift=0):
        n, ok = ctypes.c_uint64(0), ctypes.c_int(0)
        self.check(lib().tdt_selftest_index(self.h, int(cell_count), float(inv_cell_count), int(n_cells), int(shift), ctypes.byref(n), ctypes.byref(ok)))
        return n.value, bool(ok.value)

    def close(self):
        if self.h:
            lib().tdt_ctx_destroy(self.h)
            self.h = None

    def __enter__(self):
        return self

    def __exit__(self, *a):
        self.close()


class VertexBufferObject:

    def __init__(self, ctx, data):
        a = np.ascontiguousarray(data)
        h = ctypes.c_void_p()
        ctx.check(lib().tdt_buffer_create(ctx.h, a.ctypes.data if a.size else None, a.nbytes, ctypes.byref(h)))
        self.ctx, self.h, self.nbytes = ctx, h, a.nbytes

    @classmethod
    def _adopt(cls, ctx, h, nbytes):
        b = cls.__new__(cls)
        b.ctx, b.h, b.nbytes = ctx, h, nbytes
        return b

    def sub_data(self, offset, data):
        a = np.ascontiguousarray(data)
        self.ctx.check(lib().tdt_buffer_sub_data(self.h, offset, a.nbytes, a.ctypes.data))

    def read(self, dtype=np.uint32):
        out = np.empty(self.nbytes // np.dtype(dtype).itemsize, dtype)
        self.ctx.check(lib().tdt_buffer_read(self.h, 0, out.nbytes, out.ctypes.data))
        return out


class Texture:

    def __init__(self, ctx, h, width, height):
        self.ctx, self.h, self._w, self._h = ctx, h, width, height

    @classmethod
    def new_2d(cls, ctx, width, height, bind=True):
        h = ctypes.c_void_p()
        ctx.check(lib().tdt_image_create_rgba32f(ctx.h, width, height, ctypes.byref(h)))
        t = cls(ctx, h, width, height)
        if bind:
            t.bind()
        return t

    @classmethod
    def wrap_device(cls, ctx, device_ptr, width, height, bind=True):
        h = ctypes.c_void_p()
        ctx.check(lib().tdt_image_wrap_device(ctx.h, ctypes.c_void_p(device_ptr), width, height, ctypes.byref(h)))
        t = cls(ctx, h, width, height)
        if bind:
            t.bind()
        return t

    def bind(self):
        self.ctx.check(lib().tdt_bind_image(self.ctx.h, 0, self.h))

    def width(self):
        return self._w

    def height(self):
        return self._h

    def depth(self):
        return 1

    def read(self):
        img = np.empty((self._h, self._w, 4), np.float32)
        self.ctx.check(lib().tdt_image_read(self.h, img.ctypes.data))
        return img

# ... 206 lines not shown
```

Measured before the change: 7688 Mray-samples/s.

## Add five-waves-per-SIMD trace variant spilling cold per-lane state to LDS

Adds a templated trace-kernel build (PER_CU>1, total 1280 threads per CU) for whole-depth plane-form trees. It drops the LDS node copy and memo, walks the tree from global memory, and parks rarely-used per-lane state (root/leaf hit records, sample sums, pixel coords, work counter) in shared memory so each lane holds fewer registers and more waves fit per SIMD. The cost-order planner now receives the chosen build's thread count. It trades extra LDS traffic and global node fetches for higher occupancy to hide latency. Stats counters for fallback lanes and a geometry debug query are also added.

```diff
diff --git a/include/tdt_rt.h b/include/tdt_rt.h
--- a/include/tdt_rt.h
+++ b/include/tdt_rt.h
@@ -289,6 +289,7 @@
 int tdt_debug_xform_bricks(const tdt_ctx *ctx, uint32_t out[2]);
 
 int tdt_debug_last_variant(const tdt_ctx *ctx, int out[6]);
+int tdt_debug_last_geometry(const tdt_ctx *ctx, int out[2]);
 int tdt_debug_trace_variants(int *rows, int capacity, int *count);
 int tdt_debug_stats(tdt_ctx *ctx, uint64_t *out, int n_words, int reset);
 int tdt_debug_counters(tdt_ctx *ctx, uint64_t out[32]);
diff --git a/tdt4230_project_raytracing_amd/build.py b/tdt4230_project_raytracing_amd/build.py
--- a/tdt4230_project_raytracing_amd/build.py
+++ b/tdt4230_project_raytracing_amd/build.py
@@ -68,6 +68,17 @@
     return out
 
 
+STATS_LIB = os.path.join(_HERE, "libtdtrt_stats.so")
+
+
+def build_stats(force=False):
+    hdrs = [os.path.join(CSRC, f) for f in DEVICE_HEADERS] + [os.path.join(INCLUDE, "tdt_rt.h"), os.path.abspath(__file__)]
+    srcs = [os.path.join(CSRC, f) for f in DEVICE_UNITS]
+    if force or _newer(STATS_LIB, srcs + hdrs):
+        build_device(extra_flags=("-DTDT_STATS",), out=STATS_LIB)
+    return STATS_LIB
+
+
 def build_demo(force=False):
     out = os.path.join(_HERE, "tdt_demo")
     srcs = [os.path.join(CSRC, "demo_main.cpp"), os.path.join(INCLUDE, "renderer.hpp"), os.path.join(INCLUDE, "tdt_rt.h"),
@@ -90,4 +101,9 @@
 
 
 def build_all(force=False):
-    return build_host(force), build_device(force), build_demo(force), build_selftest(force)
+    from concurrent.futures import ThreadPoolExecutor
+    with ThreadPoolExecutor(2) as pool:
+        stats = pool.submit(build_stats, force)
+        host_lib, device_lib = build_host(force), build_device(force)
+        stats_lib = stats.result()
+    return host_lib, device_lib, build_demo(force), build_selftest(force), stats_lib
diff --git a/tdt4230_project_raytracing_amd/csrc/tdt_rt.hip b/tdt4230_project_raytracing_amd/csrc/tdt_rt.hip
--- a/tdt4230_project_raytracing_amd/csrc/tdt_rt.hip
+++ b/tdt4230_project_raytracing_amd/csrc/tdt_rt.hip
@@ -15,7 +15,6 @@
 
 #ifndef TDT_BLOCK
 #define TDT_BLOCK 1024
-#define TDT_BLOCKS_PER_CU 1
 #endif
 namespace tdt {
 
@@ -61,11 +60,28 @@
   TDT_DEV bool new_record() const { return (bits & 2u) != 0u; }
 };
 
+enum : int { COLD_ROOT = 0, COLD_ROOT_T = 7, COLD_LEAF = 8,
+             COLD_SUM = 15, COLD_WORK = 18, COLD_X = 19, COLD_Y = 20,
+             COLD_WORDS = 21 };
+template <int BLOCK> struct ColdSlots {
+  uint32_t *lane;
+  TDT_DEV uint32_t u(int w) const { return lane[w * BLOCK]; }
+  TDT_DEV float f(int w) const { return __uint_as_float(lane[w * BLOCK]); }
+  TDT_DEV void u(int w, uint32_t v) const { lane[w * BLOCK] = v; }
+  TDT_DEV void f(int w, float v) const { lane[w * BLOCK] = __float_as_uint(v); }
+  TDT_DEV void put(int w, const HitTmp &h) const {
+    f(w, h.nx); f(w + 1, h.ny); f(w + 2, h.nz); f(w + 3, h.px); f(w + 4, h.py); f(w + 5, h.pz); u(w + 6, h.ff ? 1u : 0u);
+  }
+  TDT_DEV HitTmp get(int w) const { return {f(w), f(w + 1), f(w + 2), f(w + 3), f(w + 4), f(w + 5), u(w + 6) != 0u}; }
+};
+
 enum : int { STAT_TRAV_PASS = 0, STAT_TRAV_LANES, STAT_INSIDE_LANES, STAT_ALIVE_LANES, STAT_EVENT_PASS, STAT_EVENT_LANES, STAT_HIT_PASS, STAT_HIT_LANES,
              STAT_LAMB_PASS, STAT_LAMB_LANES, STAT_METAL_PASS, STAT_METAL_LANES, STAT_DIEL_PASS, STAT_DIEL_LANES, STAT_END_PASS, STAT_END_LANES,
              STAT_PIXEL_END_PASS, STAT_PIXEL_END_LANES, STAT_FETCH_PASS, STAT_FETCH_LANES, STAT_PRIMARY_PASS, STAT_PRIMARY_LANES,
              STAT_NEWRAY_PASS, STAT_NEWRAY_LANES, STAT_GATE_WAIT_LANES, STAT_DRAINED_TRAV_PASS, STAT_DRAINED_EVENT_PASS, STAT_LOOP_PASS, STAT_WAVE_TICKS, STAT_WAVES,
-             STAT_T_FIRST, STAT_T_LAST, STAT_COUNT = 32 };
+             STAT_T_FIRST, STAT_T_LAST,
+             STAT_FALLBACK_PASS = 32, STAT_FALLBACK_LANES,
+             STAT_COUNT = 34 };
 #ifdef TDT_STATS
 TDT_DEV void stat_add(uint32_t *row, int i, unsigned long long mask) {
   const unsigned long long m = __ballot(1);
@@ -78,8 +94,9 @@
 #define TDT_ST1(i, v) do {} while (0)
 #endif
 
-template <bool COUNT, int FORM, int DEPTH = 0, bool RESIDENT = false, bool SAFEV = false, bool FULL = false, bool UNIT = false, bool BRICK = false>
-__global__ __launch_bounds__(TDT_BLOCK) void trace_kernel(const TraceParams P) {
+template <bool COUNT, int FORM, int DEPTH = 0, bool RESIDENT = false, bool SAFEV = false, bool FULL = false, bool UNIT = false, bool BRICK = false,
+          int BLOCK = TDT_BLOCK, int PER_CU = 1>
+__global__ __attribute__((amdgpu_flat_work_group_size(1, BLOCK), amdgpu_waves_per_eu((BLOCK * PER_CU + 255) / 256))) void trace_kernel(const TraceParams P) {
   constexpr bool POW2 = FORM != FORM_LITERAL;
   constexpr bool kSlim2 = DEPTH > 0;
 #ifdef TDT_THRESHOLD_EVERY
@@ -99,11 +116,19 @@
 #else
   constexpr bool kSharedNorm = kSlim2;
 #endif
-  __shared__ __attribute__((aligned(16))) uint16_t s_nodes[(BRICK ? kBrickLdsCells : kLdsCells) * 8 + 8];
-  for (uint32_t i = threadIdx.x * 8u; i < P.lds_nodes; i += (uint32_t)TDT_BLOCK * 8u)
-    *reinterpret_cast<uint4 *>(&s_nodes[i]) = *reinterpret_cast<const uint4 *>(&P.packed[i]);
-  if (threadIdx.x < 16 && P.lds_nodes + threadIdx.x < ((P.lds_nodes + 7u) & ~7u) + 8u)
-    s_nodes[P.lds_nodes + threadIdx.x] = (uint16_t)((RESIDENT && POW2) ? 0u : kPackedEscape);
+  constexpr bool kCold = PER_CU > 1;
+  static_assert(!kCold || (FULL && !COUNT && !BRICK && RESIDENT && SAFEV && DEPTH > 0 && kFullEntryForm == kFullPlanes && BLOCK * PER_CU == 1280),
+                "five waves per SIMD: the whole-depth plane-form builds");
+  __shared__ __attribute__((aligned(16))) uint16_t s_nodes[(kCold ? 0u : (BRICK ? kBrickLdsCells : kLdsCells)) * 8 + 8];
+  if constexpr (!kCold) {
+    for (uint32_t i = threadIdx.x * 8u; i < P.lds_nodes; i += (uint32_t)BLOCK * 8u)
+      *reinterpret_cast<uint4 *>(&s_nodes[i]) = *reinterpret_cast<const uint4 *>(&P.packed[i]);
+    if (threadIdx.x < 16 && P.lds_nodes + threadIdx.x < ((P.lds_nodes + 7u) & ~7u) + 8u)
+      s_nodes[P.lds_nodes + threadIdx.x] = (uint16_t)((RESIDENT && POW2) ? 0u : kPackedEscape);
+  }
+  __shared__ uint32_t s_cold[kCold ? COLD_WORDS * BLOCK : 1];
+  const ColdSlots<BLOCK> cold = {&s_cold[kCold ? threadIdx.x : 0]};
+  if constexpr (kCold) cold.u(COLD_WORK, 0u);
   constexpr bool kPlanes = FULL && !COUNT && kFullEntryForm == kFullPlanes;
   __shared__ __attribute__((aligned(8))) float2 s_planes[kPlanes ? PlaneTable::kEntries : 1];
   if constexpr (kPlanes) build_plane_table<DEPTH, UNIT>(s_planes, P.scale, P.min_x, P.min_y, P.min_z);
@@ -114,7 +139,7 @@
   __shared__ __attribute__((aligned(8))) float2 s_thr[kThrCells + 1];
   __shared__ uint32_t s_band;
   if (TABLE) {
-    for (uint32_t i = threadIdx.x; i <= kThrCells; i += (uint32_t)TDT_BLOCK)
+    for (uint32_t i = threadIdx.x; i <= kThrCells; i += (uint32_t)BLOCK)
       s_thr[i] = i < P.thr_cells ? reinterpret_cast<const float2 *>(P.thr)[i] : make_float2(2.0f, 2.0f);
     __syncthreads();
   }
@@ -125,7 +150,7 @@
   if (kUseGrid) build_top_grid<GL, TABLE>(s_nodes, P.lds_nodes, DEPTH, s_grid, &s_grid_ok, s_thr, P.thr_cells, P.thr_f0max, &s_band);
   __shared__ __attribute__((aligned(16))) uint32_t s_grid32[BRICK ? (1 << 15) : 4];
   if (BRICK) {
-    for (uint32_t i = threadIdx.x * 4u; i < (1u << 15); i += (uint32_t)TDT_BLOCK * 4u)
+    for (uint32_t i = threadIdx.x * 4u; i < (1u << 15); i += (uint32_t)BLOCK * 4u)
       *reinterpret_cast<uint4 *>(&s_grid32[i]) = *reinterpret_cast<const uint4 *>(&P.brick_grid[i]);
     __syncthreads();
   }
@@ -148,9 +173,10 @@
   MatSource ms_regs;
   if (!kColdArgs) ms_regs = material_source(P);
 #ifdef TDT_STATS
-  __shared__ uint32_t s_stats[(TDT_BLOCK / 64) * STAT_COUNT];
+  __shared__ uint32_t s_stats[(BLOCK / 64) * STAT_COUNT];
   uint32_t *const s_stat_row = &s_stats[(threadIdx.x >> 6) * STAT_COUNT];
   if ((threadIdx.x & 63) < STAT_COUNT) s_stat_row[threadIdx.x & 63] = 0u;
+  ns.stat_fallback = &s_stat_row[STAT_FALLBACK_PASS];
   const unsigned long long stat_t0 = __builtin_amdgcn_s_memrealtime();
   bool stat_drained = false;
 #endif
@@ -166,7 +192,7 @@
   if (COUNT && (threadIdx.x & 63) == 0) atomicCAS(&P.counters[23], 0ull, wave_t0);
   Counters cnt = {};
   uint32_t n_pixels = 0;
-  constexpr int kMemo = BRICK ? kBrickMemoLevels : kMemoLevels;
+  constexpr int kMemo = BRICK ? kBrickMemoLevels : (kCold ? 0 : kMemoLevels);
   NodeMemo<kMemo> memo;
 #pragma unroll
   for (int l = 0; l < kMemo; l++) { memo.key[l] = 0x3FFFFFFFu; memo.val[l] = 0u; }
@@ -237,7 +263,8 @@
         const float ipd_in = inv_pow_depth;
         CellPlanes cp;
         bool leaf;
-        if constexpr (kPlanes) leaf = tree_lookup_pow2<COUNT, kMemo, DEPTH, RESIDENT, SAFEV, FULL, BRICK, TABLE, UNIT>(P, ns, lx, ly, lz, inv_pow_depth, ugx, ugy, ugz, value, memo, cnt, &cp);
+        if constexpr (kCold) leaf = tree_lookup_pow2<COUNT, kMemo, DEPTH, false, SAFEV, FULL, BRICK, TABLE, UNIT, true>(P, ns, lx, ly, lz, inv_pow_depth, ugx, ugy, ugz, value, memo, cnt, &cp);
+        else if constexpr (kPlanes) leaf = tree_lookup_pow2<COUNT, kMemo, DEPTH, RESIDENT, SAFEV, FULL, BRICK, TABLE, UNIT>(P, ns, lx, ly, lz, inv_pow_depth, ugx, ugy, ugz, value, memo, cnt, &cp);
         else leaf = POW2 ? tree_lookup_pow2<COUNT, kMemo, DEPTH, RESIDENT, SAFEV, FULL, BRICK, TABLE>(P, ns, lx, ly, lz, inv_pow_depth, ugx, ugy, ugz, value, memo, cnt)
                          : tree_lookup<COUNT>(P, ns, lx, ly, lz, inv_pow_depth, ugx, ugy, ugz, value, cnt);
         TDT_MARK(traversal_b);
@@ -292,8 +319,10 @@
     TDT_MARK(hit_prologue);
     if (COUNT) evpass_no++;
     if (COUNT) { cnt.event_slots += slot64(); cnt.event_active += (state > ST_TRAVERSE); }
+    if constexpr (kCold) lane_work = cold.u(COLD_WORK);
     if (kSlim2) lane_work += (state == ST_HIT || state == ST_END) ? kCostEvent + kCostRayStep * ((uint32_t)it + 1u) : ((state > ST_TRAVERSE) ? kCostEvent : 0u);
     else lane_work += (state > ST_TRAVERSE) ? kCostEvent : 0u;
+    if constexpr (kCold) cold.u(COLD_WORK, lane_work);
     if (COUNT) lane_E += (state > ST_TRAVERSE) ? 1u : 0u;
     if (state == ST_HIT) {
       if (COUNT) { cnt.scatter_slots += slot64(); cnt.scatter_active++; }
@@ -305,9 +334,17 @@
       } else ms = ms_regs;
       const MatRef mat = material_fetch(ms, hit_index);
       TDT_ST(STAT_LAMB_PASS, __ballot(mat.type == 0u)); TDT_ST(STAT_METAL_PASS, __ballot(mat.type == 1u)); TDT_ST(STAT_DIEL_PASS, __ballot(mat.type == 2u));
-      if (owed.new_record()) { cube_hit_record(r, t_stride, leaf_box_x, leaf_box_y, leaf_box_z, inv_pow_depth, pc.leaf); if (COUNT) cnt.leaf_records++; }
+      if (owed.new_record()) {
+        cube_hit_record(r, t_stride, leaf_box_x, leaf_box_y, leaf_box_z, inv_pow_depth, pc.leaf); if (COUNT) cnt.leaf_records++;
+        if constexpr (kCold) cold.put(COLD_LEAF, pc.leaf);
+      }
       loop_count += 1;
-      const HitTmp &src = owed.leaf_site() ? pc.leaf : pc.root;
+      HitTmp cold_rec = {0.f, 0.f, 0.f, 0.f, 0.f, 0.f, false};
+      if constexpr (kCold) {
+        const ColdSlots<BLOCK> site = {cold.lane + (owed.leaf_site() ? COLD_LEAF * BLOCK : COLD_ROOT * BLOCK)};
+        cold_rec = site.get(0);
+      }
+      const HitTmp &src = kCold ? cold_rec : (owed.leaf_site() ? pc.leaf : pc.root);
       Hit h;
       h.px = src.px; h.py = src.py; h.pz = src.pz; h.nx = src.nx; h.ny = src.ny; h.nz = src.nz; h.ff = src.ff;
       h.index = hit_index;
@@ -327,6 +364,7 @@
     TDT_ST(STAT_END_PASS, __ballot(state == ST_END));
     if (state == ST_END) {
       float cr, cg, cb;
+      if constexpr (kCold) { sr = cold.f(COLD_SUM); sg = cold.f(COLD_SUM + 1); sb = cold.f(COLD_SUM + 2); }
       if (loop_count > 0) { cr = ar; cg = ag; cb = ab; }
       else {
         const float yp = r.dy + 1.0f;
@@ -335,14 +373,17 @@
       }
       sr = sr + cr; sg = sg + cg; sb = sb + cb;
       s++;
+      if constexpr (kCold) { cold.f(COLD_SUM, sr); cold.f(COLD_SUM + 1, sg); cold.f(COLD_SUM + 2, sb); }
       if (s < s_end) state = ST_PRIMARY;
       else {
         TDT_MARK(pixel_end);
         TDT_ST(STAT_PIXEL_END_PASS, __ballot(1));
+        if constexpr (kCold) { int x_, y_; bool in_; decode_pixel(P, (int)(pixel_slot >> 10), pixel_slot & 1023u, x_, y_, pix, in_); }
         float4 *dst = reinterpret_cast<float4 *>(P.image) + pix;
         if (P.accumulate) {
           *dst = make_float4(sr, sg, sb, 0.f);
           if (P.carry && !P.carry_final) {
+            if constexpr (kCold) { pc.root = cold.get(COLD_ROOT); pc.root_t = cold.f(COLD_ROOT_T); pc.leaf = cold.get(COLD_LEAF); }
             float4 *c = reinterpret_cast<float4 *>(P.carry) + pix * 4;
             c[0] = make_float4(pc.root.nx, pc.root.ny, pc.root.nz, pc.root.px);
             c[1] = make_float4(pc.root.py, pc.root.pz, pc.root.ff ? 1.f : 0.f, pc.root_t);
@@ -361,13 +402,13 @@
 #ifdef TDT_STATS
         if (P.stats && P.pixel_log) {
           uint32_t *L = P.pixel_log + (size_t)pixel_slot * 8;
-          L[0] = lane_work; L[3] = stat_pix_t0; L[4] = (uint32_t)__builtin_amdgcn_s_memrealtime(); L[5] = blockIdx.x * 16 + (threadIdx.x >> 6); L[7] = (uint32_t)threshold;
+          L[0] = lane_work; L[3] = stat_pix_t0; L[4] = (uint32_t)__builtin_amdgcn_s_memrealtime(); L[5] = blockIdx.x * (BLOCK / 64) + (threadIdx.x >> 6); L[7] = (uint32_t)threshold;
         }
 #endif
         if (COUNT && P.pixel_log) {
           uint32_t *L = P.pixel_log + (size_t)pixel_slot * 8;
           L[0] = lane_S; L[1] = lane_E; L[2] = pass_no - pixel_pass0; L[3] = (uint32_t)(pixel_rt0 - P.counters[23]);
-          L[4] = (uint32_t)(__builtin_amdgcn_s_memrealtime() - P.counters[23]); L[5] = blockIdx.x * 16 + (threadIdx.x >> 6); L[6] = evpass_no - pixel_evpass0; L[7] = (uint32_t)threshold;
+          L[4] = (uint32_t)(__builtin_amdgcn_s_memrealtime() - P.counters[23]); L[5] = blockIdx.x * (BLOCK / 64) + (threadIdx.x >> 6); L[6] = evpass_no - pixel_evpass0; L[7] = (uint32_t)threshold;
         }
         if (COUNT) {
           const unsigned long long d = (__builtin_amdgcn_s_memrealtime() - pixel_rt0) / 10000ull;
@@ -416,6 +457,7 @@
             pixel_slot = q;
             decode_pixel(P, (int)(pixel_slot >> 10), pixel_slot & 1023u, x, y, pix, inside);
             lane_work = 0u;
+            if constexpr (kCold) cold.u(COLD_WORK, 0u);
             if (inside) {
               n_pixels++;
               sr = 0.f; sg = 0.f; sb = 0.f; s = P.spp_begin;
@@ -430,6 +472,11 @@
                   pc.leaf = {c2.x, c2.y, c2.z, c2.w, c3.x, c3.y, c3.z != 0.f};
                 }
               }
+              if constexpr (kCold) {
+                cold.put(COLD_ROOT, pc.root); cold.f(COLD_ROOT_T, pc.root_t); cold.put(COLD_LEAF, pc.leaf);
+                cold.f(COLD_SUM, sr); cold.f(COLD_SUM + 1, sg); cold.f(COLD_SUM + 2, sb);
+                cold.u(COLD_X, (uint32_t)x); cold.u(COLD_Y, (uint32_t)y);
+              }
               if (s < s_end) state = ST_PRIMARY;
               else if (!P.accumulate) {
                 const float n = (float)P.samples_per_pixel;
@@ -445,6 +492,7 @@
     TDT_MARK(primary);
     TDT_ST(STAT_PRIMARY_PASS, __ballot(state == ST_PRIMARY));
     if (state == ST_PRIMARY) {
+      if constexpr (kCold) { x = (int)cold.u(COLD_X); y = (int)cold.u(COLD_Y); }
       r = primary_ray(P, x, y, s);
       loop_count = 0; ar = 1.f; ag = 1.f; ab = 1.f;
       state = ST_NEWRAY;
@@ -473,9 +521,11 @@
         const float t_enter = hw_max(hw_max(hw_max(mnx, 0.0003f), mny), mnz);
         const float t_exit = hw_min(hw_min(hw_min(mxx, inf), mxy), mxz);
         t_octree_max = inf;
+        if constexpr (kCold) pc.root_t = cold.f(COLD_ROOT_T);
         if (t_exit >= t_enter) {
           cube_hit_record(r, t_enter, P.min_x, P.min_y, P.min_z, P.scale, pc.root);
           pc.root_t = t_enter;
+          if constexpr (kCold) { cold.put(COLD_ROOT, pc.root); cold.f(COLD_ROOT_T, t_enter); }
           t_octree_max = t_exit;
         }
         t_stride = pc.root_t;
@@ -495,10 +545,10 @@
   if (P.stats) {
     const unsigned long long stat_t1 = __builtin_amdgcn_s_memrealtime();
     const uint32_t lane = threadIdx.x & 63u;
-    if (lane < (uint32_t)STAT_WAVE_TICKS) { const uint32_t v = s_stat_row[lane]; if (v) atomicAdd(&P.stats[lane], (unsigned long long)v); }
+    if (lane < (uint32_t)STAT_WAVE_TICKS || (lane >= (uint32_t)STAT_FALLBACK_PASS && lane < (uint32_t)STAT_COUNT)) { const uint32_t v = s_stat_row[lane]; if (v) atomicAdd(&P.stats[lane], (unsigned long long)v); }
     if (lane == 0) { atomicAdd(&P.stats[STAT_WAVE_TICKS], stat_t1 - stat_t0); atomicAdd(&P.stats[STAT_WAVES], 1ull);
                      atomicMin(&P.stats[STAT_T_FIRST], stat_t0); atomicMax(&P.stats[STAT_T_LAST], stat_t1);
-                     const uint32_t w = blockIdx.x * (TDT_BLOCK / 64) + (threadIdx.x >> 6);
+                     const uint32_t w = blockIdx.x * (BLOCK / 64) + (threadIdx.x >> 6);
                      if (w < 8192u) P.stats[STAT_COUNT + 1 + w] = stat_t1; }
   }
 #endif
@@ -508,7 +558,7 @@
       const unsigned long long t_end = __builtin_amdgcn_s_memrealtime();
       atomicMin(&P.counters[18], wave_t0); atomicMax(&P.counters[19], t_end);
       atomicAdd(&P.counters[20], t_end - wave_t0); atomicAdd(&P.counters[21], 1ull);
-      P.counters[32 + blockIdx.x * (TDT_BLOCK / 64) + (threadIdx.x >> 6)] = t_end;
+      P.counters[32 + blockIdx.x * (BLOCK / 64) + (threadIdx.x >> 6)] = t_end;
     }
     if ((threadIdx.x & 63) == 0) for (int i = 0; i < 7; i++) atomicAdd(&P.counters[24 + i], tacc[i]);
     uint32_t v[18] = {n_pixels, cnt.octree_hit_calls, cnt.iterations, cnt.node_loads,
@@ -1154,14 +1204,17 @@
 }
 
 using TraceFn = void (*)(const TraceParams);
-struct TraceVariant { int form, depth; bool resident, full, brick, unit; TraceFn fn; };
-#define TDT_V1(FORM, D, R, F, B, U) {tdt::FORM, D, R, F, B, U, tdt::trace_kernel<false, tdt::FORM, D, R, true, F, U, B>}
+struct TraceVariant { int form, depth; bool resident, full, brick, unit; TraceFn fn; int block, per_cu; };
+#define TDT_V1(FORM, D, R, F, B, U) {tdt::FORM, D, R, F, B, U, tdt::trace_kernel<false, tdt::FORM, D, R, true, F, U, B>, TDT_BLOCK, 1}
 #define TDT_V(FORM, D, R, F, B) TDT_V1(FORM, D, R, F, B, false), TDT_V1(FORM, D, R, F, B, true)
+#define TDT_V5_1(D, U) {tdt::FORM_POW2, D, true, true, false, U, tdt::trace_kernel<false, tdt::FORM_POW2, D, true, true, true, U, false, 256, 5>, 256, 5}
+#define TDT_V5(D) TDT_V5_1(D, false), TDT_V5_1(D, true)
 const TraceVariant kTraceVariants[] = {
   TDT_V(FORM_POW2, 6, false, false, true), TDT_V(FORM_POW2, 7, false, false, true), TDT_V(FORM_POW2, 8, false, false, true),
   TDT_V(FORM_POW2, 9, false, false, true), TDT_V(FORM_POW2, 10, false, false, true),
   TDT_V(FORM_POW2, 6, false, false, false), TDT_V(FORM_POW2, 7, false, false, false), TDT_V(FORM_POW2, 8, false, false, false),
   TDT_V(FORM_POW2, 9, false, false, false), TDT_V(FORM_POW2, 10, false, false, false),
+  TDT_V5(5), TDT_V5(6),
   TDT_V(FORM_POW2, 5, true, true, false), TDT_V(FORM_POW2, 6, true, true, false),
   TDT_V(FORM_POW2, 3, true, false, false), TDT_V(FORM_POW2, 4, true, false, false), TDT_V(FORM_POW2, 5, true, false, false),
   TDT_V(FORM_POW2, 6, true, false, false), TDT_V(FORM_POW2, 7, true, false, false), TDT_V(FORM_POW2, 8, true, false, false),
@@ -1172,11 +1225,14 @@
   TDT_V(FORM_TABLE, 6, false, false, false), TDT_V(FORM_TABLE, 7, false, false, false), TDT_V(FORM_TABLE, 8, false, false, false),
   TDT_V(FORM_TABLE, 9, false, false, false), TDT_V(FORM_TABLE, 10, false, false, false),
 };
+#undef TDT_V5
+#undef TDT_V5_1
 #undef TDT_V
 #undef TDT_V1
-TraceFn find_variant(int form, int depth, bool resident, bool full, bool brick, bool unit) {
+const TraceVariant *find_variant(int form, int depth, bool resident, bool full, bool brick, bool unit, bool four_waves) {
   for (const TraceVariant &v : kTraceVariants)
-    if (v.form == form && v.depth == depth && v.resident == resident && v.full == full && v.brick == brick && v.unit == unit) return v.fn;
+    if (v.form == form && v.depth == depth && v.resident == resident && v.full == full && v.brick == brick && v.unit == unit &&
+        !(four_waves && v.per_cu > 1)) return &v;
   return nullptr;
 }
 
@@ -1214,6 +1270,7 @@
     bool no_prepass = env_set("TDT_NO_PREPASS");
     bool no_order_reuse = env_set("TDT_NO_ORDER_REUSE");
     bool no_full = env_set("TDT_NO_FULL_GRID");
+    bool four_waves = env_one("TDT_FOUR_WAVES");
     bool no_table_form = env_set("TDT_NO_TABLE_FORM");
     bool no_bricks = env_set("TDT_NO_BRICKS");
     float max_share = env_float("TDT_MAX_SHARE", 1.0f);
@@ -1263,6 +1320,7 @@
   uint32_t *pixel_log = nullptr; size_t pixel_log_u32 = 0;
   unsigned long long *stats = nullptr;
   int last_variant[6] = {};
+  int last_geometry[2] = {};
 
   ~TraceState() { if (phase_timing) for (auto &e : phase_ev) (void)hipEventDestroy(e); }
   template <class T> hipError_t alloc(T *&p, size_t n) { p = mem.get<T>(n); return p ? hipSuccess : hipErrorOutOfMemory; }
@@ -1430,7 +1488,7 @@
 
 struct HandOut { const uint32_t *slot_order = nullptr, *plan = nullptr; uint32_t *slot_cost = nullptr; };
 
-int plan_order(tdt_ctx *ctx, TraceState &S, const CostSig &sig, const LaunchRequest &rq, int owned, HandOut &out) {
+int plan_order(tdt_ctx *ctx, TraceState &S, const CostSig &sig, const LaunchRequest &rq, int owned, uint32_t lanes, HandOut &out) {
   TraceState::CostOrder &O = S.order;
   const TraceState::Switches &env = S.env;
   const size_t n = (size_t)owned * 1024;
@@ -1461,7 +1519,6 @@
     const uint32_t n_slots = (uint32_t)owned * 1024u, n_chunks = (n_slots + tdt::kOrderChunk - 1) / tdt::kOrderChunk;
     const uint32_t og = tdt::kOrderBits;
     uint32_t *hist = O.hist + 1024u * O.parity, *hist_next = O.hist + 1024u * (O.parity ^ 1u), *plan = O.hist + 2048;
-    const uint32_t lanes = (uint32_t)ctx->num_cus * TDT_BLOCKS_PER_CU * TDT_BLOCK;
     hipLaunchKernelGGL(tdt::order_hist_kernel, dim3(n_chunks), dim3(1024), 0, ctx->stream, O.slot_cost, O.slot_acc, n_slots, hist, og, smooth, keep_costs ? 1 : 0, blend);
     hipLaunchKernelGGL(tdt::order_plan_kernel, dim3(1), dim3(512), 0, ctx->stream, hist, og, lanes, env.max_share, plan, smooth, hist_next, plan + 4);
     hipLaunchKernelGGL(tdt::order_scatter_kernel, dim3(n_chunks), dim3(1024), 0, ctx->stream, O.slot_cost, O.slot_acc, n_slots,
@@ -1595,25 +1652,34 @@
   return TDT_OK;
 }
 
-int launch_trace(tdt_ctx *ctx, TraceState &S, const LaunchRequest &rq, const TreeForm &f, int owned, const TraceParams &P) {
-  unsigned nblk = (unsigned)(((long)owned * 1024 + 1023) / 1024);
-  if (nblk > (unsigned)ctx->num_cus * TDT_BLOCKS_PER_CU) nblk = (unsigned)ctx->num_cus * TDT_BLOCKS_PER_CU;
-  const dim3 grid(nblk, 1, 1), block(TDT_BLOCK, 1, 1);
-  bool launched = false;
+struct TraceBuild { TraceFn fn = nullptr; int block = TDT_BLOCK, per_cu = 1; int v[6] = {}; };
+TraceBuild choose_build(const TraceState &S, const LaunchRequest &rq, const TreeForm &f, const TraceParams &P) {
+  TraceBuild b;
+  b.v[0] = f.pow2 ? tdt::FORM_POW2 : tdt::FORM_LITERAL;
   if (!rq.counts_out && (f.pow2 || f.table_form) && f.safev && !S.env.no_specialise) {
     const bool unit = P.scale == 1.0f && P.inv_scale == 1.0f && P.min_x != 0.0f && P.min_y != 0.0f && P.min_z != 0.0f && !rq.probe;
     const int form = f.pow2 ? tdt::FORM_POW2 : tdt::FORM_TABLE;
-    TraceFn fn = nullptr;
-    if (f.brick) fn = find_variant(form, P.max_depth, false, false, true, unit);
-    if (!fn && f.full) fn = find_variant(form, P.max_depth, true, true, false, unit);
-    if (!fn) fn = find_variant(form, P.max_depth, f.resident, false, false, unit);
-    if (fn) {
-      hipLaunchKernelGGL(fn, grid, block, 0, ctx->stream, P); launched = true;
+    const TraceVariant *tv = nullptr;
+    if (f.brick) tv = find_variant(form, P.max_depth, false, false, true, unit, S.env.four_waves);
+    if (!tv && f.full) tv = find_variant(form, P.max_depth, true, true, false, unit, S.env.four_waves);
+    if (!tv) tv = find_variant(form, P.max_depth, f.resident, false, false, unit, S.env.four_waves);
+    if (tv) {
+      b.fn = tv->fn; b.block = tv->block; b.per_cu = tv->per_cu;
       const int v[6] = {form, P.max_depth, (f.brick || !f.resident) ? 0 : 1, (!f.brick && f.full) ? 1 : 0, f.brick ? 1 : 0, unit ? 1 : 0};
-      std::memcpy(S.last_variant, v, sizeof v);
-    }
-  }
-  if (!launched) { const int v[6] = {f.pow2 ? tdt::FORM_POW2 : tdt::FORM_LITERAL, 0, 0, 0, 0, 0}; std::memcpy(S.last_variant, v, sizeof v); }
+      std::memcpy(b.v, v, sizeof v);
+    }
+  }
+  return b;
+}
+
+int launch_trace(tdt_ctx *ctx, TraceState &S, const LaunchRequest &rq, const TreeForm &f, const TraceBuild &b, int owned, const TraceParams &P) {
+  unsigned nblk = (unsigned)(((long)owned * 1024 + b.block - 1) / b.block);
+  if (nblk > (unsigned)ctx->num_cus * (unsigned)b.per_cu) nblk = (unsigned)ctx->num_cus * (unsigned)b.per_cu;
+  const dim3 grid(nblk, 1, 1), block((unsigned)b.block, 1, 1);
+  bool launched = false;
+  if (b.fn) { hipLaunchKernelGGL(b.fn, grid, block, 0, ctx->stream, P); launched = true; }
+  std::memcpy(S.last_variant, b.v, sizeof b.v);
+  S.last_geometry[0] = b.block; S.last_geometry[1] = b.per_cu;
 #define TDT_LAUNCH(C) do { if (f.pow2) hipLaunchKernelGGL((tdt::trace_kernel<C, tdt::FORM_POW2>), grid, block, 0, ctx->stream, P); \
                            else hipLaunchKernelGGL((tdt::trace_kernel<C, tdt::FORM_LITERAL>), grid, block, 0, ctx->stream, P); } while (0)
   if (!launched && rq.counts_out && getenv("TDT_COUNT_SPECIALISED") && f.pow2 && f.safev && f.resident && P.max_depth == 6) {
@@ -1640,21 +1706,22 @@
   if (t.owned > 0) {
     if (int rc = bind_queue(ctx, S.queue, S.mem, P)) return rc;
     if (int rc = refresh_packed(ctx, S, P)) return rc;
-    if (!S.env.no_cost_order) {
-      CostSig sig; HandOut h;
-      make_sig(ctx, c, k, ctx->image0, &sig);
-      if (int rc = plan_order(ctx, S, sig, rq, t.owned, h)) return rc;
-      P.slot_order = h.slot_order; P.plan = h.plan; P.slot_cost = h.slot_cost;
-    }
-    if (rq.prepass_ran && !rq.counts_out)
-      if (int rc = filter_done(ctx, S.miss, t.owned, P.slot_order)) return rc;
     TreeForm f = classify_tree(S, P);
     if (!rq.counts_out) {
       if (int rc = prepare_thresholds(ctx, S, f, P)) return rc;
       if (int rc = prepare_full_grid(ctx, S, f, P)) return rc;
       if (int rc = prepare_bricks(ctx, S, f, P)) return rc;
     }
-    if (int rc = launch_trace(ctx, S, rq, f, t.owned, P)) return rc;
+    const TraceBuild build = choose_build(S, rq, f, P);
+    if (!S.env.no_cost_order) {
+      CostSig sig; HandOut h;
+      make_sig(ctx, c, k, ctx->image0, &sig);
+      if (int rc = plan_order(ctx, S, sig, rq, t.owned, (uint32_t)ctx->num_cus * (uint32_t)(build.per_cu * build.block), h)) return rc;
+      P.slot_order = h.slot_order; P.plan = h.plan; P.slot_cost = h.slot_cost;
+    }
+    if (rq.prepass_ran && !rq.counts_out)
+      if (int rc = filter_done(ctx, S.miss, t.owned, P.slot_order)) return rc;
+    if (int rc = launch_trace(ctx, S, rq, f, build, t.owned, P)) return rc;
   }
   if (rq.counts_out) {
     TDT_HIP(ctx, hipMemcpyAsync(rq.counts_out, ctx->counters, 8 * sizeof(unsigned long long), hipMemcpyDeviceToHost, ctx->stream));
@@ -2164,10 +2231,18 @@
   return TDT_OK;
 }
 
+int tdt_debug_last_geometry(const tdt_ctx *ctx, int out[2]) {
+  if (!ctx || !out) return TDT_ERR_INVALID_VALUE;
+  if (ctx->multi) ctx = tdt::multi_first_member(const_cast<tdt_ctx *>(ctx));
+  std::memcpy(out, ctx->trace->last_geometry, 2 * sizeof(int));
+  return TDT_OK;
+}
+
 int tdt_debug_trace_variants(int *rows, int capacity, int *count) {
   if (!count || capacity < 0 || (capacity > 0 && !rows)) return TDT_ERR_INVALID_VALUE;
   int n = 0;
   for (const TraceVariant &v : kTraceVariants) {
+    if (v.per_cu == 1 && find_variant(v.form, v.depth, v.resident, v.full, v.brick, v.unit, false) != &v) continue;
     if (n < capacity) {
       const int r[6] = {v.form, v.depth, v.resident ? 1 : 0, v.full ? 1 : 0, v.brick ? 1 : 0, v.unit ? 1 : 0};
       std::memcpy(rows + 6 * n, r, sizeof r);
diff --git a/tdt4230_project_raytracing_amd/csrc/trace_device.hpp b/tdt4230_project_raytracing_amd/csrc/trace_device.hpp
--- a/tdt4230_project_raytracing_amd/csrc/trace_device.hpp
+++ b/tdt4230_project_raytracing_amd/csrc/trace_device.hpp
@@ -155,6 +155,9 @@
   const uint32_t *grid32; const void *bricks;
   const float2 *thr; float thr_f0max;
   __amdgpu_buffer_rsrc_t cells;
+#ifdef TDT_STATS
+  uint32_t *stat_fallback;
+#endif
 };
 
 TDT_DEV uint32_t fetch_node(const NodeSource &ns, uint32_t idx, uint32_t &code) {
@@ -316,6 +319,7 @@
 }
 template <int CL>
 struct NodeMemo { uint32_t key[CL]; uint32_t val[CL]; };
+template <> struct NodeMemo<0> { uint32_t key[1]; uint32_t val[1]; };
 constexpr int kNoProbeFrom = 6;
 TDT_DEV uint32_t grid_v_bound(int level) { return level < 3 ? 128u : (level == 3 ? 1024u : 8192u); }
 template <int GL> struct Grid;
@@ -489,10 +493,11 @@
   value = (g.w0 >> 5) & 0x7FFu;
   return (g.w0 & 3u) == 2u;
 }
-template <bool COUNT, int CL, int DEPTH, bool RESIDENT, bool SAFEV, bool FULL = false, bool BRICK = false, bool TABLE = false, bool UNIT = false>
+template <bool COUNT, int CL, int DEPTH, bool RESIDENT, bool SAFEV, bool FULL = false, bool BRICK = false, bool TABLE = false, bool UNIT = false, bool GLOBAL = false>
 TDT_DEV bool tree_lookup_pow2(const TraceParams &P, const NodeSource &ns, float fx, float fy, float fz, float &inv_pow_depth,
                               float &gx, float &gy, float &gz, uint32_t &value, NodeMemo<CL> &memo, Counters &cnt, CellPlanes *cp = nullptr) {
   static_assert(!TABLE || (SAFEV && !BRICK && !FULL), "per-cell thresholds: the resident walk, or (trees outside the LDS table) the jump table's bands only");
+  static_assert(!GLOBAL || (FULL && !RESIDENT && !COUNT), "the walk from global memory: behind the whole-depth table");
   constexpr bool PLANES = FULL && !COUNT && kFullEntryForm == kFullPlanes;
   const int depth = DEPTH > 0 ? DEPTH : P.max_depth;
   const float scale_d = __uint_as_float((uint32_t)(127 + depth) << 23);
@@ -517,6 +522,12 @@
       if constexpr (PLANES) return full_entry_planes<DEPTH>(g, ns.planes, *cp, inv_pow_depth, value);
       else return full_entry_decode<kFullEntryBits, DEPTH>(g, xg, Yi, Zi, gx, gy, gz, inv_pow_depth, value);
     }
+#ifdef TDT_STATS
+    {
+      const unsigned long long in_band = __ballot(!safe);
+      if ((threadIdx.x & 63) == (uint32_t)__builtin_ctzll(__ballot(1))) { ns.stat_fallback[0] += 1u; ns.stat_fallback[1] += (uint32_t)__popcll(in_band); }
+    }
+#endif
   } else if constexpr (BRICK && !COUNT) {
     static_assert(!BRICK || (DEPTH >= 6 && DEPTH <= 10 && !RESIDENT && SAFEV), "the 32-bit table: trees of depth 6-10 outside the LDS table");
     constexpr int BL = (int)brick_levels(DEPTH);
@@ -631,7 +642,7 @@
     qx = qx + qx + bitx;
     const uint32_t idx = ((ix << 2) + (((Yi >> sh) & 1u) << 1) + ((Zi >> sh) & 1u)) & 0x1FFFFFFFu;
     bool resident = false;
-    if (RESIDENT || l < kNoProbeFrom) {
+    if (!GLOBAL && (RESIDENT || l < kNoProbeFrom)) {
       const uint32_t li = idx < ns.lds_nodes ? idx : ns.lds_nodes;
       const uint32_t n = ns.lds[li];
       resident = RESIDENT || (n != kPackedEscape);
diff --git a/tdt4230_project_raytracing_amd/rt.py b/tdt4230_project_raytracing_amd/rt.py
--- a/tdt4230_project_raytracing_amd/rt.py
+++ b/tdt4230_project_raytracing_amd/rt.py
@@ -224,6 +224,7 @@
     ("tdt_debug_edit_mode", _I, [_P, _I]),
     ("tdt_debug_last_edit_path", _I, [_P]),
     ("tdt_debug_last_variant", _I, [_P, ctypes.POINTER(ctypes.c_int)]),
+    ("tdt_debug_last_geometry", _I, [_P, ctypes.POINTER(ctypes.c_int)]),
     ("tdt_debug_trace_variants", _I, [ctypes.POINTER(ctypes.c_int), _I, ctypes.POINTER(ctypes.c_int)]),
     ("tdt_debug_counters", _I, [_P, ctypes.POINTER(ctypes.c_uint64)]),
     ("tdt_debug_stats", _I, [_P, ctypes.POINTER(ctypes.c_uint64), _I, _I]),
@@ -682,22 +683,24 @@
         return n.value
 
     def last_variant(self):
-        v = (ctypes.c_int * 6)()
+        v, g = (ctypes.c_int * 6)(), (ctypes.c_int * 2)()
         self.check(lib().tdt_debug_last_variant(self.h, v))
-        return dict(zip(("form", "depth", "resident", "full", "brick", "unit"), [int(x) for x in v]))
+        self.check(lib().tdt_debug_last_geometry(self.h, g))
+        return dict(zip(("form", "depth", "resident", "full", "brick", "unit", "block", "per_cu"), [int(x) for x in v] + [int(x) for x in g]))
 
     STAT_NAMES = ("trav_pass", "trav_lanes", "inside_lanes", "alive_lanes", "event_pass", "event_lanes", "hit_pass", "hit_lanes", "lamb_pass", "lamb_lanes",
                   "metal_pass", "metal_lanes", "diel_pass", "diel_lanes", "end_pass", "end_lanes", "pixel_end_pass", "pixel_end_lanes", "fetch_pass", "fetch_lanes",
                   "primary_pass", "primary_lanes", "newray_pass", "newray_lanes", "gate_wait_lanes", "drained_trav_pass", "drained_event_pass", "loop_pass",
-                  "wave_ticks", "waves", "t_first", "t_last")
+                  "wave_ticks", "waves", "t_first", "t_last", "fallback_pass", "fallback_lanes")
 
     def stats(self, reset=True):
-        n = 32 + 1 + 8192
+        rows = len(self.STAT_NAMES)
+        n = rows + 1 + 8192
         v = (ctypes.c_uint64 * n)()
         self.check(lib().tdt_debug_stats(self.h, v, n, 1 if reset else 0))
-        d = dict(zip(self.STAT_NAMES, [int(x) for x in v[:32]]))
-        d["t_queue_dry"] = int(v[32])
-        d["wave_ends"] = [int(x) for x in v[33:33 + min(int(v[29]), 8192)]]
+        d = dict(zip(self.STAT_NAMES, [int(x) for x in v[:rows]]))
+        d["t_queue_dry"] = int(v[rows])
+        d["wave_ends"] = [int(x) for x in v[rows + 1:rows + 1 + min(d["waves"], 8192)]]
         return d
 
     def selftest_index(self, cell_count, inv_cell_count, n_cells, shift=0):
```

Measured after the change: 7963 Mray-samples/s (median of 6 runs). 3.6% higher.
